# igd-geo/schwarzwald

Measured on AMD Instinct MI355X. Metric: Mpoints/s end-to-end tile (Morton+sort+sample), higher is better.
Workload: dtype u64 keys / f64 positions

## Files before the change

schwarzwald_amd/csrc/swz_api.hip:

```cpp
#include <algorithm>
#include <cstring>

#include "swz_device.h"
#include "swz_internal.h"

int swz_ctx::get(const char* name, size_t bytes, void** out) {
  swz::DevBuf& b = bufs[name];
  if (bytes == 0) bytes = 16;
  if (b.cap < bytes) {
    const size_t old_cap = b.cap;
    if (b.ptr) {
      SWZ_HIP(this, hipStreamSynchronize(stream));
      free_buf(b);
    }
    size_t want = bytes + bytes / 16;
    const size_t minimal = (want + 255) & ~size_t(255);
    if (old_cap) {
      if (strncmp(name, "tl_", 3) == 0 || strncmp(name, "tiler_store", 11) == 0) want = std::max(want, 2 * old_cap);
      else want = std::max(want, std::min(2 * old_cap, bytes + (size_t(1) << 30)));
    }
    want = (want + 255) & ~size_t(255);
    hipError_t e = hipMalloc(&b.ptr, want);
    if (const char* fa = opt("SWZ_FAIL_ALLOC")) {
      const size_t fl = strlen(fa);
      const bool hit = fl && fa[fl - 1] == '*' ? strncmp(fa, name, fl - 1) == 0 : strcmp(fa, name) == 0;
      if (e == hipSuccess && hit) {
        (void)hipFree(b.ptr);
        b.ptr = nullptr;
        e = hipErrorOutOfMemory;
      }
    }
    if (e == hipErrorOutOfMemory) {
      (void)hipGetLastError();
      SWZ_HIP(this, hipStreamSynchronize(stream));
      for (auto& kv : bufs) {
        const std::string& nm = kv.first;
        const bool level_scratch = nm.compare(0, 3, "md_") == 0 || nm.compare(0, 3, "sp_") == 0 || nm.compare(0, 3, "pm_") == 0;
        const bool shared_root = md_shard_root_published && nm.size() >= 3 && nm.compare(nm.size() - 3, 3, "_sr") == 0;
        const bool tiler_scratch = tiler_scratch_dead && nm.compare(0, 3, "tl_") == 0;
        if ((level_scratch || tiler_scratch) && !shared_root && kv.second.ptr && kv.second.epoch < scratch_epoch && &kv.second != &b)
          free_buf(kv.second);
      }
      e = hipMalloc(&b.ptr, want);
      if (e == hipErrorOutOfMemory && want > minimal) {
        (void)hipGetLastError();
        want = minimal;
        e = hipMalloc(&b.ptr, want);
      }
    }
    if (e != hipSuccess) {
      b.ptr = nullptr;
      std::vector<std::pair<size_t, std::string>> held;
      size_t total = 0;
      for (const auto& kv : bufs) {
        if (kv.second.host) continue;
        total += kv.second.cap;
        if (kv.second.cap) held.emplace_back(kv.second.cap, kv.first);
      }
      std::sort(held.rbegin(), held.rend());
      size_t free_b = 0, total_b = 0;
      (void)hipMemGetInfo(&free_b, &total_b);
      std::string top;
      for (size_t i = 0; i < held.size() && i < 14; ++i)
        top += " " + held[i].second + "=" + std::to_string(held[i].first >> 20) + "M";
      return fail(SWZ_ERR_HIP, std::string("hipMalloc(") + name + ", " + std::to_string(want) + " bytes): " + hipGetErrorString(e) +
                                 "; workspace holds " + std::to_string(total >> 20) + " MiB, device free " +
                                 std::to_string(free_b >> 20) + " of " + std::to_string(total_b >> 20) + " MiB; largest:" + top);
    }
    b.cap = want;
    if (const char* e = opt("SWZ_POISON")) {
      const char* only = opt("SWZ_POISON_ONLY");
      if (!only || strstr(name, only)) SWZ_HIP(this, hipMemsetAsync(b.ptr, atoi(e), want, stream));
    }
  }
  b.epoch = scratch_epoch;
  *out = b.ptr;
  return SWZ_OK;
}

void swz_ctx::release_all() {
  if (stream) (void)hipStreamSynchronize(stream);
  for (auto& kv : bufs) free_buf(kv.second);
  bufs.clear();
}

void swz_ctx::free_buf(swz::DevBuf& b) {
  if (b.ptr && b.ptr == sbi_clean_ptr) sbi_clean_ptr = nullptr;
  if (b.ptr) (void)(b.host ? hipHostFree(b.ptr) : hipFree(b.ptr));
  b.ptr = nullptr;
  b.cap = 0;
  b.host = false;
}

uint64_t swz_ctx::held_bytes() const {
  uint64_t s = 0;
  for (const auto& kv : bufs)
    if (!kv.second.host) s += kv.second.cap;
  return s;
}

uint64_t swz_ctx::held_host_bytes() const {
  uint64_t s = 0;
  for (const auto& kv : bufs)
    if (kv.second.host) s += kv.second.cap;
  return s;
}

hipEvent_t swz_ctx::take_event() {
  if (!event_pool.empty()) {
    hipEvent_t e = event_pool.back();
    event_pool.pop_back();
    return e;
  }
  hipEvent_t e = nullptr;
  (void)hipEventCreate(&e);
  return e;
}

void swz_ctx::prof_begin(const char*) {
  if (!profile) return;
  cur_e0_ = take_event();
  (void)hipEventRecord(cur_e0_, stream);
}

void swz_ctx::prof_end(const char* name, uint64_t launches, uint64_t bytes) {
  if (!profile || !cur_e0_) return;
  hipEvent_t e1 = take_event();
  (void)hipEventRecord(e1, stream);
  pending.push_back({name, cur_e0_, e1, launches, bytes});
  cur_e0_ = nullptr;
}

void swz_ctx::prof_collect() {
  for (auto& p : pending) {
    float ms = 0.f;
    if (hipEventSynchronize(p.e1) == hipSuccess && hipEventElapsedTime(&ms, p.e0, p.e1) == hipSuccess) {
      swz::KernelStat& k = kstats[p.name];
      k.launches += p.launches;
      k.total_ms += ms;
      k.bytes += p.bytes;
    }
    event_pool.push_back(p.e0);
    event_pool.push_back(p.e1);
  }
  pending.clear();
}

int swz::read_u32(swz_ctx* c, const uint32_t* d, uint32_t* h) {
  SWZ_HIP(c, hipMemcpyAsync(h, d, 4, hipMemcpyDeviceToHost, c->stream));
  SWZ_HIP(c, hipStreamSynchronize(c->stream));
  return SWZ_OK;
}

int swz::check_params(swz_ctx* c, const swz_tile_params* p) {
  if (!p) return c->fail(SWZ_ERR_BAD_ARG, "params must not be NULL");
  if (p->sampler < SWZ_RANDOM_GRID || p->sampler > SWZ_MIN_DISTANCE_FAST) return c->fail(SWZ_ERR_BAD_ARG, "unknown sampler");
  if (p->sampler == SWZ_MIN_DISTANCE_FAST && (p->flags & SWZ_FLAG_MIN_DISTANCE_PROPERTY))
    return c->fail(SWZ_ERR_BAD_ARG, "SWZ_FLAG_MIN_DISTANCE_PROPERTY with MIN_DISTANCE_FAST: the property mode's order is not defined for "
                                    "a sampler that offers only every n-th point of a node");
  if (p->strategy != SWZ_ACCURATE && p->strategy != SWZ_FAST) return c->fail(SWZ_ERR_BAD_ARG, "unknown strategy");
  if (!(p->spacing_at_root > 0.f)) return c->fail(SWZ_ERR_BAD_ARG, "spacing_at_root must be > 0");
  if (p->strategy == SWZ_FAST && p->fast_concurrency == 0)
    return c->fail(SWZ_ERR_BAD_ARG, "FAST needs fast_concurrency >= 1");
  return SWZ_OK;
}

const char* swz::sharded_sampler_refusal(int sampler) {
  if (sampler != SWZ_MIN_DISTANCE_FAST) return nullptr;
  return "MIN_DISTANCE_FAST cannot be sharded: the root offers every fourth point of ITS Morton-ordered range, counted across the "
         "shards' octants, and a shard does not know how many points the lower shards hold in front of its own";
}

static std::string g_create_error;

namespace {

int upload(swz_ctx* c, void* dst, const void* src, size_t bytes) {
  if (bytes == 0) return SWZ_OK;
  SWZ_HIP(c, hipMemcpyAsync(dst, src, bytes, hipMemcpyHostToDevice, c->stream));
  return SWZ_OK;
}
int download(swz_ctx* c, void* dst, const void* src, size_t bytes) {
  if (bytes == 0) return SWZ_OK;
  SWZ_HIP(c, hipMemcpyAsync(dst, src, bytes, hipMemcpyDeviceToHost, c->stream));
  return SWZ_OK;
}
int sync(swz_ctx* c) {
  SWZ_HIP(c, hipStreamSynchronize(c->stream));
  c->prof_collect();
  return SWZ_OK;
}
int check_n(swz_ctx* c, uint64_t n) {
  if (n > 0xFFFF0000ull) return c->fail(SWZ_ERR_TOO_MANY_POINTS, "more than 2^32-65536 points in one batch");
  return SWZ_OK;
}
int check_bounds(swz_ctx* c, const double mn[3], const double mx[3]) {
  if (!mn || !mx) return c->fail(SWZ_ERR_BAD_ARG, "bounds must not be NULL");
  for (int a = 0; a < 3; ++a)
    if (!(mx[a] > mn[a])) return c->fail(SWZ_ERR_BAD_ARG, "bounds must have positive extent on every axis");
  return SWZ_OK;
}

}

extern "C" {

int swz_abi_version(void) { return SWZ_ABI_VERSION; }

int swz_create(swz_ctx** ctx_out, int device) {
  if (!ctx_out) return SWZ_ERR_BAD_ARG;
  *ctx_out = nullptr;
  int count = 0;
  hipError_t e = hipGetDeviceCount(&count);
  if (e != hipSuccess || count <= 0) {
    g_create_error = std::string("swz_create: no usable HIP device (") +
                     (e != hipSuccess ? hipGetErrorString(e) : "device count is 0") +
                     "); this library has no CPU fallback";
    return SWZ_ERR_HIP;
  }
  if (device < 0 || device >= count) {
    g_create_error = "swz_create: device ordinal out of range";
    return SWZ_ERR_BAD_ARG;
  }
  e = hipSetDevice(device);
  if (e != hipSuccess) {
    g_create_error = std::string("swz_create: hipSetDevice: ") + hipGetErrorString(e);
    return SWZ_ERR_HIP;
  }
  swz_ctx* c = new swz_ctx();
  c->device = device;
  e = hipStreamCreateWithFlags(&c->own_stream, hipStreamNonBlocking);
  if (e != hipSuccess) {
    g_create_error = std::string("swz_create: hipStreamCreate: ") + hipGetErrorString(e);
    delete c;
    return SWZ_ERR_HIP;
  }
  c->stream = c->own_stream;
  extern char** environ;
  for (char** e = environ; e && *e; ++e) {
    if (std::strncmp(*e, "SWZ_", 4) != 0) continue;
    const char* eq = std::strchr(*e, '=');
    if (eq) c->options[std::string(*e, (size_t)(eq - *e))] = std::string(eq + 1);
  }
  *ctx_out = c;
  return SWZ_OK;
}

int swz_set_option(swz_ctx* c, const char* name, const char* value) {
  if (!c || !name) return SWZ_ERR_BAD_ARG;
  if (value) c->options[name] = value; else c->options.erase(name);
  return SWZ_OK;
}

int swz_destroy(swz_ctx* c) {
  if (!c) return SWZ_OK;
  (void)hipSetDevice(c->device);
  if (c->nodes_tiler) {
    (void)swz_tiler_destroy(c->nodes_tiler);
    c->nodes_tiler = nullptr;
  }
  swz::shard_free(c);
  c->release_all();
  c->prof_collect();
  for (hipEvent_t e : c->event_pool) (void)hipEventDestroy(e);
  for (hipStream_t st : c->aux_streams) (void)hipStreamDestroy(st);
  if (c->own_stream) (void)hipStreamDestroy(c->own_stream);
  delete c;
  return SWZ_OK;
}

const char* swz_last_error(const swz_ctx* c) { return c ? c->err.c_str() : g_create_error.c_str(); }

int swz_set_stream(swz_ctx* c, void* hip_stream) {
  if (!c) return SWZ_ERR_BAD_ARG;
  SWZ_HIP(c, hipStreamSynchronize(c->stream));
  c->stream = hip_stream == SWZ_OWN_STREAM ? c->own_stream : reinterpret_cast<hipStream_t>(hip_stream);
  return SWZ_OK;
}

int swz_release_workspace(swz_ctx* c) {
  if (!c) return SWZ_ERR_BAD_ARG;
  SWZ_HIP(c, hipSetDevice(c->device));
  if (c->tiler_active) return c->fail(SWZ_ERR_BAD_ARG, "swz_release_workspace: a tiler of this context keeps its node store in the workspace");
  swz::shard_free(c);
  c->release_all();
  return SWZ_OK;
}

uint64_t swz_workspace_bytes(const swz_ctx* c) { return c ? c->held_bytes() : 0; }

int swz_host_alloc_pinned(uint64_t bytes, void** out) {
  if (!out) return SWZ_ERR_BAD_ARG;
  *out = nullptr;
  return hipHostMalloc(out, bytes ? bytes : 1, hipHostMallocDefault) == hipSuccess ? SWZ_OK : SWZ_ERR_HIP;
}
int swz_host_free_pinned(void* p) { return (!p || hipHostFree(p) == hipSuccess) ? SWZ_OK : SWZ_ERR_HIP; }

int swz_device_alloc(uint64_t bytes, void** d_out) {
  if (!d_out) return SWZ_ERR_BAD_ARG;
  *d_out = nullptr;
  return hipMalloc(d_out, bytes ? bytes : 1) == hipSuccess ? SWZ_OK : SWZ_ERR_HIP;
}
int swz_device_alloc_on(swz_ctx* c, uint64_t bytes, void** d_out) {
  if (!c || !d_out) return SWZ_ERR_BAD_ARG;
  *d_out = nullptr;
  SWZ_HIP(c, hipSetDevice(c->device));
  SWZ_HIP(c, hipMalloc(d_out, bytes ? bytes : 1));
  return SWZ_OK;
}
int swz_device_free(void* d_ptr) { return (!d_ptr || hipFree(d_ptr) == hipSuccess) ? SWZ_OK : SWZ_ERR_HIP; }
static bool is_mapped_host_memory(const void* p) {
  hipPointerAttribute_t at{};
  if (hipPointerGetAttributes(&at, p) != hipSuccess) {
    (void)hipGetLastError();
    return false;
  }
  return at.type == hipMemoryTypeHost;
}
int swz_copy_to_host(swz_ctx* c, void* dst_host, const void* d_src, uint64_t bytes) {
  if (!c) return SWZ_ERR_BAD_ARG;
  SWZ_HIP(c, hipSetDevice(c->device));
  if (bytes && is_mapped_host_memory(d_src)) {
    SWZ_HIP(c, hipStreamSynchronize(c->stream));
    std::memcpy(dst_host, d_src, bytes);
    return SWZ_OK;
  }
  if (bytes) SWZ_HIP(c, hipMemcpyAsync(dst_host, d_src, bytes, hipMemcpyDeviceToHost, c->stream));
  SWZ_HIP(c, hipStreamSynchronize(c->stream));
  return SWZ_OK;
}
int swz_copy_to_device(swz_ctx* c, void* d_dst, const void* src_host, uint64_t bytes) {
  if (!c) return SWZ_ERR_BAD_ARG;
  SWZ_HIP(c, hipSetDevice(c->device));
  if (bytes && is_mapped_host_memory(d_dst)) {
    SWZ_HIP(c, hipStreamSynchronize(c->stream));
    std::memcpy(d_dst, src_host, bytes);
    return SWZ_OK;
  }
  if (bytes) SWZ_HIP(c, hipMemcpyAsync(d_dst, src_host, bytes, hipMemcpyHostToDevice, c->stream));
  SWZ_HIP(c, hipStreamSynchronize(c->stream));
  return SWZ_OK;
}

int swz_profile_enable(swz_ctx* c, int enabled) {
  if (!c) return SWZ_ERR_BAD_ARG;
  c->profile = enabled != 0;
  return SWZ_OK;
}
int swz_profile_reset(swz_ctx* c) {
  if (!c) return SWZ_ERR_BAD_ARG;
  SWZ_TRY(sync(c));
  c->kstats.clear();
  return SWZ_OK;
}
int swz_profile_get(swz_ctx* c, swz_kernel_stat* out, uint32_t max_stats, uint32_t* num_out) {
  if (!c || !num_out) return SWZ_ERR_BAD_ARG;
  SWZ_TRY(sync(c));
  uint32_t k = 0;
  for (const auto& kv : c->kstats) {
    if (k < max_stats && out) {
      std::memset(&out[k], 0, sizeof(out[k]));
      std::strncpy(out[k].name, kv.first.c_str(), sizeof(out[k].name) - 1);
      out[k].launches = kv.second.launches;
      out[k].total_ms = kv.second.total_ms;
      out[k].algorithmic_bytes = kv.second.bytes;
    }
    ++k;
  }
  *num_out = k;
  return SWZ_OK;
}

int swz_morton_encode_device(swz_ctx* c, double* d_xyz, uint64_t n, const double bmin[3], const double bmax[3],
                             uint64_t* d_keys_out) {
  if (!c) return SWZ_ERR_BAD_ARG;
  SWZ_HIP(c, hipSetDevice(c->device));
  SWZ_TRY(check_n(c, n));
  SWZ_TRY(check_bounds(c, bmin, bmax));
  if (n && (!d_xyz || !d_keys_out)) return c->fail(SWZ_ERR_BAD_ARG, "swz_morton_encode_device: NULL buffer");
  SWZ_TRY(swz::encode_device(c, d_xyz, (uint32_t)n, bmin, bmax, d_keys_out));
  return sync(c);
}

int swz_morton_encode(swz_ctx* c, double* xyz, uint64_t n, const double bmin[3], const double bmax[3],
                      uint64_t* keys_out) {
  if (!c) return SWZ_ERR_BAD_ARG;
  SWZ_HIP(c, hipSetDevice(c->device));
  SWZ_TRY(check_n(c, n));
  SWZ_TRY(check_bounds(c, bmin, bmax));
  if (n == 0) return SWZ_OK;
  if (!xyz || !keys_out) return c->fail(SWZ_ERR_BAD_ARG, "swz_morton_encode: NULL buffer");
  double* d_xyz = nullptr;
  uint64_t* d_keys = nullptr;
  SWZ_TRY(c->get("h_xyz", (size_t)n * 3, &d_xyz));
  SWZ_TRY(c->get("h_keys", (size_t)n, &d_keys));
  SWZ_TRY(upload(c, d_xyz, xyz, (size_t)n * 24));
  SWZ_TRY(swz::encode_device(c, d_xyz, (uint32_t)n, bmin, bmax, d_keys));
  SWZ_TRY(download(c, keys_out, d_keys, (size_t)n * 8));
  SWZ_TRY(download(c, xyz, d_xyz, (size_t)n * 24));
  return sync(c);
}

int swz_sort_by_key_device(swz_ctx* c, const uint64_t* d_keys, uint64_t n, uint32_t* d_perm_out,
                           uint64_t* d_keys_sorted_out) {
  if (!c) return SWZ_ERR_BAD_ARG;
  SWZ_HIP(c, hipSetDevice(c->device));
  SWZ_TRY(check_n(c, n));
  if (n == 0) return SWZ_OK;
  if (!d_keys || !d_perm_out) return c->fail(SWZ_ERR_BAD_ARG, "swz_sort_by_key_device: NULL buffer");
  uint64_t *kin = nullptr, *kout = d_keys_sorted_out;
  uint32_t* vtmp = nullptr;
  SWZ_TRY(c->get("sort_keys_b", (size_t)n, &kin));
  SWZ_TRY(c->get("sort_vals_b", (size_t)n, &vtmp));
  if (!kout) SWZ_TRY(c->get("sort_keys_a", (size_t)n, &kout));
  SWZ_HIP(c, hipMemcpyAsync(kin, d_keys, (size_t)n * 8, hipMemcpyDeviceToDevice, c->stream));
  SWZ_TRY(swz::radix_sort_pairs(c, kin, vtmp, kout, d_perm_out, (uint32_t)n, true));
  return sync(c);
}

int swz_sort_by_key(swz_ctx* c, const uint64_t* keys, uint64_t n, uint32_t* perm_out, uint64_t* keys_sorted_out) {
  if (!c) return SWZ_ERR_BAD_ARG;
  SWZ_HIP(c, hipSetDevice(c->device));
  SWZ_TRY(check_n(c, n));
  if (n == 0) return SWZ_OK;
  if (!keys || !perm_out) return c->fail(SWZ_ERR_BAD_ARG, "swz_sort_by_key: NULL buffer");
  uint64_t *ka = nullptr, *kb = nullptr;
  uint32_t *va = nullptr, *vb = nullptr;
  SWZ_TRY(c->get("sort_keys_a", (size_t)n, &ka));
  SWZ_TRY(c->get("sort_keys_b", (size_t)n, &kb));
  SWZ_TRY(c->get("sort_vals_a", (size_t)n, &va));
  SWZ_TRY(c->get("sort_vals_b", (size_t)n, &vb));
  SWZ_TRY(upload(c, kb, keys, (size_t)n * 8));
  SWZ_TRY(swz::radix_sort_pairs(c, kb, vb, ka, va, (uint32_t)n, true));
  SWZ_TRY(download(c, perm_out, va, (size_t)n * 4));
  if (keys_sorted_out) SWZ_TRY(download(c, keys_sorted_out, ka, (size_t)n * 8));
  return sync(c);
}

int swz_generate_uniform_device(swz_ctx* c, uint64_t seed, uint64_t first_point, uint64_t n, double* d_xyz_out) {
  if (!c) return SWZ_ERR_BAD_ARG;
  SWZ_HIP(c, hipSetDevice(c->device));
  if (n && !d_xyz_out) return c->fail(SWZ_ERR_BAD_ARG, "swz_generate_uniform_device: NULL buffer");
  SWZ_TRY(swz::generate_uniform_device(c, seed, first_point, n, d_xyz_out));
  return sync(c);
}

int swz_tile_device(swz_ctx* c, double* d_xyz, uint64_t n, const double bmin[3], const double bmax[3],
                    const swz_tile_params* params, uint64_t* d_keys_out, uint32_t* d_perm_out, int8_t* d_level_out,
                    uint32_t* d_dup_mask_out, swz_tile_stats* stats) {
  if (!c) return SWZ_ERR_BAD_ARG;
  SWZ_HIP(c, hipSetDevice(c->device));
  if (c->opt("SWZ_SYNC_ENTRY")) SWZ_HIP(c, hipDeviceSynchronize());
  SWZ_TRY(check_n(c, n));
  SWZ_TRY(check_bounds(c, bmin, bmax));
  SWZ_TRY(swz::check_params(c, params));
  if (stats) std::memset(stats, 0, sizeof(*stats));
  if (stats) {
    stats->max_level = -1;
    stats->fast_start_levels = -1;
  }
  if (n == 0) return SWZ_OK;
  if (!d_xyz || !d_keys_out || !d_perm_out || !d_level_out)
    return c->fail(SWZ_ERR_BAD_ARG, "swz_tile_device: NULL buffer");
  swz::TileDeviceOut out{d_keys_out, d_perm_out, d_level_out, d_dup_mask_out};
  int st = swz::tile_device(c, d_xyz, (uint32_t)n, bmin, bmax, *params, out, stats);
  int st2 = sync(c);
  return st != SWZ_OK ? st : st2;
}

int swz_tile(swz_ctx* c, double* xyz, uint64_t n, const double bmin[3], const double bmax[3],
             const swz_tile_params* params, uint64_t* keys_out, uint32_t* perm_out, int8_t* level_out,
             uint32_t* dup_mask_out, swz_tile_stats* stats) {
  if (!c) return SWZ_ERR_BAD_ARG;
  SWZ_HIP(c, hipSetDevice(c->device));
  SWZ_TRY(check_n(c, n));
  SWZ_TRY(check_bounds(c, bmin, bmax));
  SWZ_TRY(swz::check_params(c, params));
  if (stats) {
    std::memset(stats, 0, sizeof(*stats));
    stats->max_level = -1;
    stats->fast_start_levels = -1;
  }
  if (n == 0) return SWZ_OK;
  if (!xyz || !keys_out || !perm_out || !level_out) return c->fail(SWZ_ERR_BAD_ARG, "swz_tile: NULL buffer");
  double* d_xyz = nullptr;
  uint64_t* d_keys = nullptr;
  uint32_t *d_perm = nullptr, *d_dup = nullptr;
  int8_t* d_level = nullptr;
  SWZ_TRY(c->get("h_xyz", (size_t)n * 3, &d_xyz));
  SWZ_TRY(c->get("h_keys", (size_t)n, &d_keys));
  SWZ_TRY(c->get("h_perm", (size_t)n, &d_perm));
  SWZ_TRY(c->get("h_level", (size_t)n, &d_level));
  if (dup_mask_out) SWZ_TRY(c->get("h_dup", (size_t)n, &d_dup));
  SWZ_TRY(upload(c, d_xyz, xyz, (size_t)n * 24));
  swz::TileDeviceOut out{d_keys, d_perm, d_level, d_dup};
  int st = swz::tile_device(c, d_xyz, (uint32_t)n, bmin, bmax, *params, out, stats);
  if (st != SWZ_OK) {
    (void)sync(c);
    return st;
  }
  SWZ_TRY(download(c, keys_out, d_keys, (size_t)n * 8));
  SWZ_TRY(download(c, perm_out, d_perm, (size_t)n * 4));
  SWZ_TRY(download(c, level_out, d_level, (size_t)n));
  if (dup_mask_out) SWZ_TRY(download(c, dup_mask_out, d_dup, (size_t)n * 4));
  SWZ_TRY(download(c, xyz, d_xyz, (size_t)n * 24));
  return sync(c);
}

int swz_partition_by_octant_device(swz_ctx* c, const uint64_t* d_keys, uint64_t n, uint32_t* d_perm_out,
                                   uint64_t counts_out[8]) {
  if (!c || !counts_out) return SWZ_ERR_BAD_ARG;
  SWZ_HIP(c, hipSetDevice(c->device));
  SWZ_TRY(check_n(c, n));
  for (int o = 0; o < 8; ++o) counts_out[o] = 0;
  if (n == 0) return SWZ_OK;
  if (!d_keys || !d_perm_out) return c->fail(SWZ_ERR_BAD_ARG, "swz_partition_by_octant_device: NULL buffer");
  SWZ_TRY(swz::partition_top_digit(c, d_keys, (uint32_t)n, d_perm_out, counts_out));
  return sync(c);
}

int swz_shard_presort_device(swz_ctx* c, const double* d_xyz_local, uint64_t n, const double bmin[3],
                             const double bmax[3], const swz_tile_params* params, uint64_t ghost_capacity) {
  if (!c) return SWZ_ERR_BAD_ARG;
  SWZ_HIP(c, hipSetDevice(c->device));
  SWZ_TRY(check_n(c, n + ghost_capacity));
  SWZ_TRY(check_bounds(c, bmin, bmax));
  SWZ_TRY(swz::check_params(c, params));
  if (const char* why = swz::sharded_sampler_refusal(params->sampler)) return c->fail(SWZ_ERR_BAD_ARG, why);
  if (n && !d_xyz_local) return c->fail(SWZ_ERR_BAD_ARG, "swz_shard_presort_device: NULL buffer");
  if (n == 0) return SWZ_OK;
  int st = swz::shard_presort_device(c, d_xyz_local, (uint32_t)n, bmin, bmax, *params, (uint32_t)ghost_capacity);
  int st2 = sync(c);
  return st != SWZ_OK ? st : st2;
}

int swz_shard_begin_device(swz_ctx* c, const double* d_xyz_local, uint64_t n, const double bmin[3],
                           const double bmax[3], const swz_tile_params* params, const swz_shard_info* shard,
                           uint64_t* num_root_taken_out) {
  if (!c) return SWZ_ERR_BAD_ARG;
  SWZ_HIP(c, hipSetDevice(c->device));
  if (!shard) return c->fail(SWZ_ERR_BAD_ARG, "shard info must not be NULL");
  SWZ_TRY(check_n(c, n + shard->num_ghosts));
  SWZ_TRY(check_bounds(c, bmin, bmax));
  SWZ_TRY(swz::check_params(c, params));
  if (const char* why = swz::sharded_sampler_refusal(params->sampler)) return c->fail(SWZ_ERR_BAD_ARG, why);
  if ((n && !d_xyz_local) || (shard->num_ghosts && !shard->d_ghost_xyz))
    return c->fail(SWZ_ERR_BAD_ARG, "swz_shard_begin_device: NULL buffer");
  if (num_root_taken_out) *num_root_taken_out = 0;
  if (n == 0) {
    return swz::shard_begin_empty(c);
  }
  int st = swz::shard_begin_device(c, d_xyz_local, (uint32_t)n, bmin, bmax, *params, shard->global_points,
                                   shard->d_ghost_xyz, (uint32_t)shard->num_ghosts, num_root_taken_out);
  int st2 = sync(c);
  return st != SWZ_OK ? st : st2;
}

int swz_shard_root_taken_device(swz_ctx* c, double* d_xyz_out) {
  if (!c) return SWZ_ERR_BAD_ARG;
  SWZ_HIP(c, hipSetDevice(c->device));
  SWZ_TRY(swz::shard_root_taken_device(c, d_xyz_out));
  return sync(c);
}

int swz_shard_finish_device(swz_ctx* c, uint64_t* d_keys_out, uint32_t* d_perm_out, int8_t* d_level_out,
                            swz_tile_stats* stats) {
  if (!c) return SWZ_ERR_BAD_ARG;
  SWZ_HIP(c, hipSetDevice(c->device));
  if (stats) {
    std::memset(stats, 0, sizeof(*stats));
    stats->max_level = -1;
    stats->fast_start_levels = -1;
  }
  int st = swz::shard_finish_device(c, d_keys_out, d_perm_out, d_level_out, stats);
  int st2 = sync(c);
  return st != SWZ_OK ? st : st2;
}

int swz_shard_fast_begin_device(swz_ctx* c, const double* d_xyz_local, uint64_t n, const double bmin[3], const double bmax[3],
                                const swz_tile_params* params, uint32_t* prefix_counts_out) {
  if (!c) return SWZ_ERR_BAD_ARG;
  SWZ_HIP(c, hipSetDevice(c->device));
  SWZ_TRY(check_n(c, n));
  SWZ_TRY(check_bounds(c, bmin, bmax));
  SWZ_TRY(swz::check_params(c, params));
  if (const char* why = swz::sharded_sampler_refusal(params->sampler)) return c->fail(SWZ_ERR_BAD_ARG, why);
  if ((n && !d_xyz_local) || !prefix_counts_out) return c->fail(SWZ_ERR_BAD_ARG, "swz_shard_fast_begin_device: NULL buffer");
  int st = swz::shard_fast_begin_device(c, d_xyz_local, (uint32_t)n, bmin, bmax, *params, prefix_counts_out);
  int st2 = sync(c);
  return st != SWZ_OK ? st : st2;
}
int swz_shard_fast_run(swz_ctx* c, int32_t start_level, uint64_t* num_root_candidates_out) {
  if (!c || !num_root_candidates_out) return SWZ_ERR_BAD_ARG;
  SWZ_HIP(c, hipSetDevice(c->device));
  int st = swz::shard_fast_run_device(c, start_level, num_root_candidates_out);
  int st2 = sync(c);
  return st != SWZ_OK ? st : st2;
}
int swz_shard_fast_root_candidates_device(swz_ctx* c, uint64_t* d_keys_out, double* d_xyz_out) {
  if (!c) return SWZ_ERR_BAD_ARG;
  SWZ_HIP(c, hipSetDevice(c->device));
  SWZ_TRY(swz::shard_fast_root_candidates_device(c, d_keys_out, d_xyz_out));
  return sync(c);
}
int swz_shard_fast_set_root_device(swz_ctx* c, const uint8_t* d_taken) {
  if (!c) return SWZ_ERR_BAD_ARG;
  SWZ_HIP(c, hipSetDevice(c->device));
  SWZ_TRY(swz::shard_fast_set_root_device(c, d_taken));
  return sync(c);
}
int swz_shard_fast_finish_device(swz_ctx* c, uint64_t* d_keys_out, uint32_t* d_perm_out, int8_t* d_level_out, uint32_t* d_dup_out,
                                 swz_tile_stats* stats) {
  if (!c) return SWZ_ERR_BAD_ARG;
  SWZ_HIP(c, hipSetDevice(c->device));
  if (stats) {
    std::memset(stats, 0, sizeof(*stats));
    stats->max_level = -1;
    stats->fast_start_levels = -1;
  }
  int st = swz::shard_fast_finish_device(c, d_keys_out, d_perm_out, d_level_out, d_dup_out, stats);
  int st2 = sync(c);
  return st != SWZ_OK ? st : st2;
}

int swz_sample_points(swz_ctx* c, int sampler, uint64_t max_points_per_node, const uint64_t* keys,
                      const uint32_t* idx, uint64_t n, const double* xyz, uint64_t num_points, uint64_t node_key,
                      int32_t node_level, const double root_min[3], const double root_max[3], float spacing_at_root,
                      int behaviour, uint8_t* taken_out, uint64_t* num_taken_out) {
  if (!c) return SWZ_ERR_BAD_ARG;
  SWZ_HIP(c, hipSetDevice(c->device));
  SWZ_TRY(check_n(c, n));
  SWZ_TRY(check_n(c, num_points));
  SWZ_TRY(check_bounds(c, root_min, root_max));
  if (sampler < SWZ_RANDOM_GRID || sampler > SWZ_MIN_DISTANCE_FAST) return c->fail(SWZ_ERR_BAD_ARG, "unknown sampler");
  if (node_level < -1 || node_level > 20) return c->fail(SWZ_ERR_BAD_ARG, "node_level out of range");
  if (num_taken_out) *num_taken_out = 0;
  if (n == 0) return SWZ_OK;
  if (!keys || !idx || !xyz || !taken_out) return c->fail(SWZ_ERR_BAD_ARG, "swz_sample_points: NULL buffer");
  double* d_xyz = nullptr;
  uint64_t* d_keys = nullptr;
  uint32_t* d_idx = nullptr;
  uint8_t* d_taken = nullptr;
  SWZ_TRY(c->get("h_xyz", (size_t)num_points * 3, &d_xyz));
  SWZ_TRY(c->get("h_keys", (size_t)n, &d_keys));
  SWZ_TRY(c->get("h_perm", (size_t)n, &d_idx));
  SWZ_TRY(c->get("h_taken", (size_t)n, &d_taken));
  SWZ_TRY(upload(c, d_xyz, xyz, (size_t)num_points * 24));
  SWZ_TRY(upload(c, d_keys, keys, (size_t)n * 8));
  SWZ_TRY(upload(c, d_idx, idx, (size_t)n * 4));
  int st = swz::sample_points_device(c, sampler, max_points_per_node, d_keys, d_idx, (uint32_t)n, d_xyz, node_key,
                                     node_level, root_min, root_max, spacing_at_root, behaviour, d_taken,
                                     num_taken_out);
  if (st != SWZ_OK) {
    (void)sync(c);
    return st;
  }
  SWZ_TRY(download(c, taken_out, d_taken, (size_t)n));
  return sync(c);
}

int swz_sample_points_device(swz_ctx* c, int sampler, uint64_t max_points_per_node, const uint64_t* d_keys, const uint32_t* d_idx,
                             uint64_t n, const double* d_xyz, uint64_t num_points, uint64_t node_key, int32_t node_level,
                             const double root_min[3], const double root_max[3], float spacing_at_root, int behaviour,
                             uint8_t* d_taken_out, uint64_t* num_taken_out) {
  if (!c) return SWZ_ERR_BAD_ARG;
  SWZ_HIP(c, hipSetDevice(c->device));
  SWZ_TRY(check_n(c, n));
  SWZ_TRY(check_n(c, num_points));
  SWZ_TRY(check_bounds(c, root_min, root_max));
  if (sampler < SWZ_RANDOM_GRID || sampler > SWZ_MIN_DISTANCE_FAST) return c->fail(SWZ_ERR_BAD_ARG, "unknown sampler");
  if (node_level < -1 || node_level > 20) return c->fail(SWZ_ERR_BAD_ARG, "node_level out of range");
  if (num_taken_out) *num_taken_out = 0;
  if (n == 0) return SWZ_OK;
  if (!d_keys || !d_idx || !d_xyz || !d_taken_out) return c->fail(SWZ_ERR_BAD_ARG, "swz_sample_points_device: NULL buffer");
  int st = swz::sample_points_device(c, sampler, max_points_per_node, d_keys, d_idx, (uint32_t)n, d_xyz, node_key, node_level, root_min,
                                     root_max, spacing_at_root, behaviour, d_taken_out, num_taken_out);
  int st2 = sync(c);
  return st != SWZ_OK ? st : st2;
}

int swz_build_node_lists(swz_ctx* c, const uint64_t* keys_sorted, const int8_t* level, uint64_t n,
                         uint32_t* order_out, uint64_t max_nodes, int8_t* node_level_out, uint64_t* node_key_out,
                         uint64_t* node_offset_out, uint64_t* node_count_out, uint64_t* num_nodes_out) {
  if (!c || !num_nodes_out) return SWZ_ERR_BAD_ARG;
  *num_nodes_out = 0;
  if (n == 0) return SWZ_OK;
  if (!keys_sorted || !level || !order_out) return c->fail(SWZ_ERR_BAD_ARG, "swz_build_node_lists: NULL buffer");
  uint64_t hist[23] = {0};
  for (uint64_t i = 0; i < n; ++i) {
    const int l = level[i];
    if (l < -1 || l > 20) return c->fail(SWZ_ERR_BAD_ARG, "level out of range");
    hist[l + 2]++;
  }
  for (int l = 1; l < 23; ++l) hist[l] += hist[l - 1];
  for (uint64_t i = 0; i < n; ++i) order_out[hist[level[i] + 1]++] = (uint32_t)i;
  uint64_t nn = 0;
  uint64_t i = 0;
  while (i < n) {
    const uint64_t p = order_out[i];
    const int l = level[p];
    const uint32_t sh = (l < 0) ? 63u : swz::level_shift(l);
    const uint64_t prefix = keys_sorted[p] >> sh;
    uint64_t j = i + 1;
    while (j < n && level[order_out[j]] == l && (keys_sorted[order_out[j]] >> sh) == prefix) ++j;
    if (nn < max_nodes && node_level_out && node_key_out && node_offset_out && node_count_out) {
      node_level_out[nn] = (int8_t)l;
      node_key_out[nn] = (l < 0) ? 0 : (prefix << sh);
      node_offset_out[nn] = i;
      node_count_out[nn] = j - i;
    }
    ++nn;
    i = j;
  }
  *num_nodes_out = nn;
  if (nn > max_nodes) return c->fail(SWZ_ERR_BAD_ARG, "max_nodes too small");
  return SWZ_OK;
}

}
```

schwarzwald_amd/csrc/swz_internal.h:

```cpp
#pragma once

#include <hip/hip_runtime.h>
#include <stdint.h>

#include <map>
#include <cstdio>
#include <cstdlib>
#include <string>
#include <vector>

#include "../../include/swz_gpu.h"

namespace swz {

constexpr uint32_t MAX_LEVELS = 21;

struct DevBuf {
  void* ptr = nullptr;
  size_t cap = 0;
  uint64_t epoch = 0;
  bool host = false;
};

struct KernelStat {
  uint64_t launches = 0;
  double total_ms = 0.0;
  uint64_t bytes = 0;
};

struct PendingEvent {
  std::string name;
  hipEvent_t e0, e1;
  uint64_t launches;
  uint64_t bytes;
};

}

struct swz_ctx {
  int device = 0;
  hipStream_t own_stream = nullptr;
  hipStream_t stream = nullptr;
  std::string err;
  std::map<std::string, swz::DevBuf> bufs;
  bool profile = false;
  std::map<std::string, swz::KernelStat> kstats;
  std::vector<swz::PendingEvent> pending;
  std::vector<hipEvent_t> event_pool;
  std::vector<hipStream_t> aux_streams;

  int fail(int code, const std::string& msg) {
    err = msg;
    return code;
  }
  int hip_fail(hipError_t e, const char* what, const char* file, int line) {
    err = std::string(what) + ": " + hipGetErrorString(e) + " (" + file + ":" + std::to_string(line) + ")";
    return SWZ_ERR_HIP;
  }

  uint64_t scratch_epoch = 1;
  void next_scratch_epoch() { ++scratch_epoch; }
  int get(const char* name, size_t bytes, void** out);
  template <typename T>
  int get(const char* name, size_t count, T** out) {
    return get(name, count * sizeof(T), reinterpret_cast<void**>(out));
  }
  void release_all();
  void free_buf(swz::DevBuf& b);
  uint64_t held_bytes() const;
  uint64_t held_host_bytes() const;

  hipEvent_t take_event();
  void prof_begin(const char* name);
  void prof_end(const char* name, uint64_t launches, uint64_t bytes);
  void prof_collect();
  hipEvent_t cur_e0_ = nullptr;
  void* shard = nullptr;
  const void* md_shard_root = nullptr;
  bool md_shard_root_published = false;
  const void* sbi_clean_ptr = nullptr;
  size_t sbi_clean_bytes = 0;
  bool tiler_active = false;
  swz_tiler* nodes_tiler = nullptr;
  bool tiler_scratch_dead = false;
  std::map<std::string, std::string> options;
  const char* opt(const char* name) const {
    const auto it = options.find(name);
    return it == options.end() ? nullptr : it->second.c_str();
  }
  long opt_int(const char* name, long def) const {
    const char* v = opt(name);
    return v ? (long)atoll(v) : def;
  }
  double opt_num(const char* name, double def) const {
    const char* v = opt(name);
    return v ? atof(v) : def;
  }
  bool opt_on(const char* name, bool def) const {
    const char* v = opt(name);
    return v ? atoi(v) != 0 : def;
  }
};

#define SWZ_HIP(ctx, expr)                                                \
  do {                                                                    \
    hipError_t _e = (expr);                                               \
    if (_e != hipSuccess) return (ctx)->hip_fail(_e, #expr, __FILE__, __LINE__); \
  } while (0)

#define SWZ_TRY(expr)            \
  do {                           \
    int _s = (expr);             \
    if (_s != SWZ_OK) return _s; \
  } while (0)

#define SWZ_LAUNCH_CHECK(ctx) SWZ_HIP(ctx, hipGetLastError())

namespace swz {

inline uint32_t div_up(uint64_t a, uint64_t b) { return (uint32_t)((a + b - 1) / b); }

struct ProfScope {
  swz_ctx* c;
  const char* name;
  uint64_t launches, bytes;
  ProfScope(swz_ctx* ctx, const char* n, uint64_t b, uint64_t l = 1) : c(ctx), name(n), launches(l), bytes(b) {
    c->prof_begin(name);
  }
  ~ProfScope() { c->prof_end(name, launches, bytes); }
};

#define SWZ_STAGE(ctx, what)                                                              \
  do {                                                                                    \
    if ((ctx)->opt("SWZ_TRACE")) {                                                            \
      const hipError_t _e = hipStreamSynchronize((ctx)->stream);                          \
      fprintf(stderr, "[swz trace] %s:%d %s -> %s\n", __FILE__, __LINE__, what, hipGetErrorString(_e)); \
      fflush(stderr);                                                                     \
    }                                                                                     \
  } while (0)

inline hipError_t memset_large(void* p, int value, size_t bytes, hipStream_t stream) {
  const size_t piece = size_t(1) << 30;
  for (size_t at = 0; at < bytes; at += piece) {
    const hipError_t e = hipMemsetAsync(static_cast<char*>(p) + at, value, bytes - at < piece ? bytes - at : piece, stream);
    if (e != hipSuccess) return e;
  }
  return hipSuccess;
}

int read_u32(swz_ctx* c, const uint32_t* d, uint32_t* h);

int encode_device(swz_ctx* c, double* d_xyz, uint32_t n, const double bmin[3], const double bmax[3],
                  uint64_t* d_keys);
int generate_uniform_device(swz_ctx* c, uint64_t seed, uint64_t first, uint64_t n, double* d_xyz);
int check_params(swz_ctx* c, const swz_tile_params* p);
const char* sharded_sampler_refusal(int sampler);

int radix_sort_pairs(swz_ctx* c, uint64_t* d_keys_in, uint32_t* d_vals_tmp, uint64_t* d_keys_out,
                     uint32_t* d_vals_out, uint32_t n, bool vals_identity);

int scan_exclusive_u32(swz_ctx* c, const uint32_t* d_in, uint32_t* d_out, uint64_t n, uint32_t* d_total,
                       const char* tag);

int gather_positions(swz_ctx* c, const double* d_xyz, const uint32_t* d_perm, uint32_t n, double* d_x,
                     double* d_y, double* d_z);

struct TileDeviceOut {
  uint64_t* keys;
  uint32_t* perm;
  int8_t* level;
  uint32_t* dup;
};

int tile_device(swz_ctx* c, double* d_xyz, uint32_t n, const double bmin[3], const double bmax[3],
                const swz_tile_params& p, const TileDeviceOut& out, swz_tile_stats* stats);

int shard_begin_device(swz_ctx* c, const double* d_xyz_local, uint32_t n, const double bmin[3],
                       const double bmax[3], const swz_tile_params& p, uint64_t global_points,
                       const double* d_ghost_xyz, uint32_t ghosts, uint64_t* num_root_taken);
int shard_presort_device(swz_ctx* c, const double* d_xyz_local, uint32_t n, const double bmin[3], const double bmax[3],
                         const swz_tile_params& p, uint32_t ghost_capacity);
int shard_root_taken_device(swz_ctx* c, double* d_xyz_out);
int shard_finish_device(swz_ctx* c, uint64_t* d_keys_out, uint32_t* d_perm_out, int8_t* d_level_out,
                        swz_tile_stats* stats);
int shard_begin_empty(swz_ctx* c);
void shard_free(swz_ctx* c);
int shard_fast_begin_device(swz_ctx* c, const double* d_xyz_local, uint32_t n, const double bmin[3], const double bmax[3],
                            const swz_tile_params& p, uint32_t* counts_host);
int shard_fast_run_device(swz_ctx* c, int start_level, uint64_t* num_root_candidates);
int shard_fast_root_candidates_device(swz_ctx* c, uint64_t* d_keys_out, double* d_xyz_out);
int shard_fast_set_root_device(swz_ctx* c, const uint8_t* d_taken);
int shard_fast_finish_device(swz_ctx* c, uint64_t* d_keys_out, uint32_t* d_perm_out, int8_t* d_level_out, uint32_t* d_dup_out,
                             swz_tile_stats* stats);
int partition_top_digit(swz_ctx* c, const uint64_t* d_keys, uint32_t n, uint32_t* d_perm_out, uint64_t octants[8]);
int partition_by_top_byte(swz_ctx* c, const uint64_t* d_keys, uint32_t n, uint32_t* d_perm_out, uint32_t starts[256]);

int sample_points_device(swz_ctx* c, int sampler, uint64_t max_points, const uint64_t* d_keys,
                         const uint32_t* d_idx, uint32_t n, const double* d_xyz, uint64_t node_key,
                         int32_t node_level, const double rmin[3], const double rmax[3], float spacing,
                         int behaviour, uint8_t* d_taken, uint64_t* num_taken);

}
```

schwarzwald_amd/csrc/swz_level.h:

```cpp
#pragma once
#include "swz_device.h"
#include "swz_internal.h"

namespace swz {

enum : uint8_t { MODE_TAKE_ALL = 0, MODE_SAMPLE = 1 };

inline bool greedy_sampler(int sampler) { return sampler == SWZ_MIN_DISTANCE || sampler == SWZ_MIN_DISTANCE_FAST; }

enum {
  CTR_NUM_NODES = 0,
  CTR_SAMPLE_NODES = 1,
  CTR_SAMPLE_POINTS = 2,
  CTR_ERROR = 3,
  CTR_REMAINING = 4,
  CTR_NUM_CELLS = 5,
  CTR_DONE_CELLS = 6,
  CTR_Q0 = 8,
  CTR_DBG_TIME = 20,
  CTR_DBG_TMAX = 21,
  CTR_DBG_HIST = 22,
  CTR_COUNT = 40
};

struct ActiveSet {
  const uint64_t* akey = nullptr;
  const uint32_t* aidx = nullptr;
  uint32_t m = 0;
  const uint64_t* ckey = nullptr;
  uint32_t nc = 0;
  uint32_t old_lo = 0, old_hi = 0;
  const uint64_t* new_key = nullptr;
  uint32_t new_m = 0;
  const uint64_t* child_nkey = nullptr;
  uint32_t child_nn = 0;
  const uint64_t* parent_prefix = nullptr;
  uint32_t parents = 0;
};

struct SortedPoints {
  const double* X = nullptr;
  const double* Y = nullptr;
  const double* Z = nullptr;
  const double* xyz = nullptr;
  const uint32_t* perm = nullptr;
  const double* ghost_xyz = nullptr;
  uint32_t ghosts = 0;
};
__host__ __device__ inline const double* sorted_point_xyz(const double* xyz, const uint32_t* perm, const double* ghost_xyz, uint32_t ghosts,
                                                          uint32_t s) {
  return (s < ghosts ? ghost_xyz : xyz) + (size_t)perm[s] * 3;
}
__device__ __forceinline__ void store_sorted_point(const SortedPoints& sp, uint32_t i, double* __restrict__ out_xyz, uint64_t o) {
  if (sp.X) {
    out_xyz[3 * o] = sp.X[i];
    out_xyz[3 * o + 1] = sp.Y[i];
    out_xyz[3 * o + 2] = sp.Z[i];
  } else {
    const double* p = sorted_point_xyz(sp.xyz, sp.perm, sp.ghost_xyz, sp.ghosts, i);
    out_xyz[3 * o] = p[0];
    out_xyz[3 * o + 1] = p[1];
    out_xyz[3 * o + 2] = p[2];
  }
}

struct LevelPlan {
  int level = -1;
  uint32_t node_shift = 63;
  int sampler = 0;
  uint64_t max_points = 0;
  bool force_sample = false;
  bool terminal = false;
  bool reroot = false;
  bool md_property = false;
  Box root;
  int cand = -1;
  double spacing_node = 0.0;
  uint32_t jitter_start = 0;
  double sq_spacing = 0.0;
  int cell_levels_geo = 0;
};

struct LevelBuffers {
  uint32_t* flags = nullptr;
  uint32_t* nid = nullptr;
  uint32_t* nstart = nullptr;
  uint8_t* nmode = nullptr;
  uint8_t* taken = nullptr;
  uint32_t* counters = nullptr;
};

struct LevelResult {
  uint32_t remaining = 0;
  uint32_t num_nodes = 0;
  uint32_t md_rounds = 0;
  const uint64_t* node_prefix = nullptr;
};

LevelPlan make_plan(int level, int sampler, uint64_t max_points, float spacing_at_root, uint32_t max_depth,
                    const double bmin[3], const double bmax[3], bool force_sample, bool tiler_rules);
int alloc_level_buffers(swz_ctx* c, uint32_t m, LevelBuffers* lb);
int required_depth_host(int sampler, int node_level, double root_extent_x, float root_max_spacing);
int level_step(swz_ctx* c, const LevelPlan& plan, const ActiveSet& as, const SortedPoints& sp, const LevelBuffers& lb,
               int8_t* level_out, uint64_t* okey, uint32_t* oidx, LevelResult* res);
const char* level_error_message(int code);
int fast_start_level(swz_ctx* c, const uint64_t* d_keys_sorted, uint32_t n, uint32_t concurrency, int* start_level);
int fast_prefix_counts(swz_ctx* c, const uint64_t* d_keys_sorted, uint32_t n, uint32_t* counts_host);
int fast_start_level_from_counts(const uint64_t* counts, uint32_t concurrency);

int random_grid_level(swz_ctx* c, const LevelPlan& plan, const ActiveSet& as, const LevelBuffers& lb);
int grid_level(swz_ctx* c, const LevelPlan& plan, const ActiveSet& as, const SortedPoints& sp, const LevelBuffers& lb);
bool grid_level_uses_keys(const swz_ctx* c, const LevelPlan& plan, const SortedPoints& sp);
int min_distance_level(swz_ctx* c, const LevelPlan& plan, const ActiveSet& as, const SortedPoints& sp,
                       const LevelBuffers& lb, uint32_t num_nodes, uint32_t sample_nodes,
                       uint32_t sample_points, uint32_t* rounds_out);
int min_distance_fast_level(swz_ctx* c, const LevelPlan& plan, const ActiveSet& as, const SortedPoints& sp, const LevelBuffers& lb,
                            uint32_t stride, uint32_t num_nodes, uint32_t sample_nodes, uint32_t* rounds_out);

}
```

schwarzwald_amd/csrc/swz_level.hip:

```cpp
#include <algorithm>
#include <cmath>

#include "swz_md.h"
#include "swz_scan.h"

namespace swz {

struct NodeHeadF {
  const uint64_t* akey;
  uint32_t nsh;
  __device__ uint32_t operator()(uint32_t i) const {
    return (i == 0) ? 1u : (uint32_t)((akey[i] >> nsh) != (akey[i - 1] >> nsh));
  }
};
struct NodeAssignG {
  uint32_t* nid;
  uint32_t* nstart;
  uint32_t m;
  __device__ void operator()(uint32_t i, uint32_t excl, uint32_t head) const {
    const uint32_t id = excl + head - 1u;
    nid[i] = id;
    if (head) nstart[id] = i;
    if (i == m - 1) nstart[id + 1] = m;
  }
};
__global__ __launch_bounds__(256) void node_child_bounds_kernel(const uint64_t* __restrict__ akey, uint32_t m, uint32_t nsh,
                                                                const uint64_t* __restrict__ pprefix, uint32_t parents,
                                                                uint32_t* __restrict__ cb) {
  const uint32_t t = blockIdx.x * 256 + threadIdx.x;
  const uint32_t j = t >> 4, o = t & 15u;
  if (j >= parents || o > 8u) return;
  const uint64_t target = (pprefix[j] >> nsh) + o;
  uint32_t lo = 0, hi = m;
  while (lo < hi) {
    const uint32_t mid = lo + (hi - lo) / 2;
    if ((akey[mid] >> nsh) < target) lo = mid + 1; else hi = mid;
  }
  cb[j * 9u + o] = lo;
}
struct ChildExistsF {
  const uint32_t* cb;
  uint32_t parents, m;
  uint32_t* counters;
  __device__ uint32_t operator()(uint32_t e) const {
    const uint32_t j = e >> 3, o = e & 7u;
    if (o == 0) {
      const uint32_t b = cb[j * 9u], en = cb[j * 9u + 8u];
      const bool ok = (j == 0 ? b == 0u : b == cb[(j - 1u) * 9u + 8u]) && (j + 1u < parents || en == m);
      if (!ok) atomicMax(&counters[CTR_ERROR], (uint32_t)SWZ_ERR_INTERNAL);
    }
    return cb[j * 9u + o + 1u] > cb[j * 9u + o] ? 1u : 0u;
  }
};
struct ChildStartG {
  const uint32_t* cb;
  uint32_t* nstart;
  __device__ void operator()(uint32_t e, uint32_t excl, uint32_t exists) const {
    if (!exists) return;
    const uint32_t j = e >> 3, o = e & 7u;
    nstart[excl] = cb[j * 9u + o];
    nstart[excl + 1u] = cb[j * 9u + o + 1u];
  }
};
constexpr uint32_t NF_TILE = 1024;
__global__ __launch_bounds__(256) void node_fill_kernel(const uint32_t* __restrict__ nstart, const uint32_t* __restrict__ counters,
                                                        uint32_t m, uint32_t* __restrict__ nid, int lazy) {
  __shared__ uint32_t s_lo, s_hi;
  __shared__ uint32_t ss[NF_TILE + 1];
  const uint32_t nn = counters[CTR_NUM_NODES];
  if (lazy && counters[CTR_SAMPLE_NODES] == nn) return;
  if (counters[CTR_ERROR] != 0u || nn == 0u) return;
  const uint32_t tid = threadIdx.x;
  const uint32_t i0 = blockIdx.x * NF_TILE;
  const uint32_t last = (m - i0) > NF_TILE ? i0 + NF_TILE - 1u : m - 1u;
  auto node_of = [&](uint32_t i) {
    uint32_t lo = 0, hi = nn;
    while (lo < hi) {
      const uint32_t mid = lo + (hi - lo) / 2;
      if (nstart[mid] <= i) lo = mid + 1; else hi = mid;
    }
    return lo - 1u;
  };
  if (tid < 2) {
    const uint32_t r = node_of(tid ? last : i0);
    if (tid) s_hi = r; else s_lo = r;
  }
  __syncthreads();
  const uint32_t lo = s_lo, span = min(s_hi - s_lo + 1u, (uint32_t)NF_TILE);
  for (uint32_t k = tid; k <= span; k += 256u) ss[k] = (lo + k < nn) ? nstart[lo + k] : 0xFFFFFFFFu;
  __syncthreads();
  const uint32_t i = i0 + tid * 4u;
  if (i >= m) return;
  uint32_t a = 0, b = span;
  while (a < b) {
    const uint32_t mid = a + (b - a) / 2;
    if (ss[mid] <= i) a = mid + 1; else b = mid;
  }
  uint32_t k = a - 1u;
  uint32_t v[4];
#pragma unroll
  for (uint32_t q = 0; q < 4u; ++q) {
    while (k + 1u <= span && ss[k + 1u] <= i + q) ++k;
    v[q] = lo + k;
  }
  if (i + 4u <= m) {
    *reinterpret_cast<uint4*>(nid + i) = make_uint4(v[0], v[1], v[2], v[3]);
  } else {
    for (uint32_t q = 0; i + q < m; ++q) nid[i + q] = v[q];
  }
}
__global__ __launch_bounds__(256) void node_prefix_kernel(const uint32_t* __restrict__ nstart, const uint64_t* __restrict__ akey,
                                                          uint32_t nsh, uint32_t nn, uint64_t* __restrict__ out) {
  const uint32_t j = blockIdx.x * 256 + threadIdx.x;
  if (j < nn) out[j] = nsh >= 63u ? 0ull : ((akey[nstart[j]] >> nsh) << nsh);
}
__global__ void single_node_kernel(uint32_t* __restrict__ nstart, uint32_t* __restrict__ num_nodes, uint32_t m) {
  nstart[0] = 0;
  nstart[1] = m;
  *num_nodes = 1;
}
struct KeepF {
  const uint8_t* taken;
  __device__ uint32_t operator()(uint32_t i) const { return taken[i] ? 0u : 1u; }
};
template <>
struct FsCountsZeroBytes<KeepF> {
  static constexpr bool value = true;
};
struct CompactG {
  const uint64_t* akey;
  const uint32_t* aidx;
  int8_t level;
  int8_t* level_out;
  uint64_t* okey;
  uint32_t* oidx;
  __device__ void operator()(uint32_t i, uint32_t excl, uint32_t keep) const {
    const uint32_t p = aidx ? aidx[i] : i;
    if (keep) {
      okey[excl] = akey[i];
      oidx[excl] = p;
    } else {
      level_out[p] = level;
    }
  }
};

__global__ __launch_bounds__(256) void node_head_kernel(const uint64_t* __restrict__ akey, uint32_t m,
                                                        uint32_t nsh, uint32_t* __restrict__ flags) {
  const uint32_t i = blockIdx.x * 256 + threadIdx.x;
  if (i >= m) return;
  flags[i] = (i == 0) ? 1u : (uint32_t)((akey[i] >> nsh) != (akey[i - 1] >> nsh));
}

__global__ __launch_bounds__(256) void node_finish_kernel(const uint32_t* __restrict__ flags,
                                                          uint32_t* __restrict__ nid, uint32_t m,
                                                          uint32_t* __restrict__ nstart) {
  const uint32_t i = blockIdx.x * 256 + threadIdx.x;
  if (i >= m) return;
  const uint32_t f = flags[i];
  const uint32_t id = nid[i] + f - 1u;
  nid[i] = id;
  if (f) nstart[id] = i;
  if (i == m - 1) nstart[id + 1] = m;
}

__global__ __launch_bounds__(256) void node_mode_kernel(const uint32_t* __restrict__ nstart,
                                                        uint8_t* __restrict__ nmode, uint32_t* __restrict__ counters,
                                                        uint64_t max_points, int force_sample, int terminal,
                                                        int reroot, const uint64_t* __restrict__ akey, uint32_t nsh,
                                                        const uint64_t* __restrict__ ckey, uint32_t nc) {
  const uint32_t nnodes = counters[CTR_NUM_NODES];
  for (uint32_t j = blockIdx.x * 256 + threadIdx.x; j < nnodes; j += gridDim.x * 256u) {
    const uint32_t cnt = nstart[j + 1] - nstart[j];
    bool cached = false;
    if (nc) {
      const uint64_t prefix = akey[nstart[j]] >> nsh;
      uint32_t lo = 0, hi = nc;
      while (lo < hi) {
        const uint32_t mid = lo + (hi - lo) / 2;
        if ((ckey[mid] >> nsh) < prefix) lo = mid + 1; else hi = mid;
      }
      cached = lo < nc && (ckey[lo] >> nsh) == prefix;
    }
    const bool sample = !terminal && (force_sample || cached || (uint64_t)cnt > max_points);
    nmode[j] = sample ? MODE_SAMPLE : MODE_TAKE_ALL;
    if (sample) {
      if (reroot) atomicMax(&counters[CTR_ERROR], (uint32_t)SWZ_ERR_REROOT_UNSUPPORTED);
      atomicAdd(&counters[CTR_SAMPLE_NODES], 1u);
      atomicAdd(&counters[CTR_SAMPLE_POINTS], cnt);
    }
  }
}

__global__ __launch_bounds__(256) void take_all_kernel(uint32_t m, const uint32_t* __restrict__ nid,
                                                       const uint8_t* __restrict__ nmode,
                                                       uint8_t* __restrict__ taken) {
  const uint32_t i = blockIdx.x * 256 + threadIdx.x;
  if (i >= m) return;
  if (nmode[nid[i]] == MODE_TAKE_ALL) taken[i] = 1;
}

static int candidate_level_host(double root_extent_x, float spacing_at_root, int node_level) {
  const auto spacing_at_this_node = spacing_at_root / std::pow(2, node_level + 1);
  return std::max(-1, (int)std::floor(std::log2f(root_extent_x / spacing_at_this_node)) - 1);
}
static int node_level_to_sample_from_host(double root_extent_x, float root_max_spacing, int node_level) {
  const auto spacing_at_target_node = root_max_spacing / std::pow(2, node_level + 1);
  const float target_spacing = (float)spacing_at_target_node;
  return std::max(-1, (int)std::floor(std::log2f(root_extent_x / target_spacing)) - 1);
}
static uint32_t prev_pow2_host(uint32_t x) {
  x = x | (x >> 1);
  x = x | (x >> 2);
  x = x | (x >> 4);
  x = x | (x >> 8);
  x = x | (x >> 16);
  return x - (x >> 1);
}
int required_depth_host(int sampler, int node_level, double root_extent_x, float root_max_spacing) {
  switch (sampler) {
    case SWZ_RANDOM_GRID:
    case SWZ_GRID_CENTER:
      return node_level_to_sample_from_host(root_extent_x, root_max_spacing, node_level);
    case SWZ_MIN_DISTANCE:
    case SWZ_MIN_DISTANCE_FAST:
      return node_level;
    default: {
      const auto spacing_at_this_node = root_max_spacing / std::pow(2, node_level + 1);
      const auto perfect_cell_count = (root_extent_x / std::pow(2, node_level + 1)) / spacing_at_this_node;
      const double clamped = perfect_cell_count >= 4294967295.0 ? 4294967295.0 : perfect_cell_count;
      const auto actual_cell_count = prev_pow2_host(static_cast<uint32_t>(clamped));
      const uint32_t levels = static_cast<uint32_t>(std::log2(actual_cell_count));
      return static_cast<int32_t>(static_cast<uint32_t>(node_level + levels));
    }
  }
}

}
extern "C" int32_t swz_required_morton_index_depth(int sampler, int32_t node_level, const double root_min[3],
                                                   const double root_max[3], float spacing_at_root) {
  if (!root_min || !root_max) return INT32_MIN;
  return swz::required_depth_host(sampler, node_level, root_max[0] - root_min[0], spacing_at_root);
}
namespace swz {

LevelPlan make_plan(int level, int sampler, uint64_t max_points, float spacing_at_root, uint32_t max_depth,
                           const double bmin[3], const double bmax[3], bool force_sample, bool tiler_rules) {
  LevelPlan p;
  p.level = level;
  p.node_shift = level < 0 ? 63u : level_shift(level);
  p.sampler = sampler;
  p.max_points = max_points;
  p.force_sample = force_sample;
  p.root = Box{bmin[0], bmin[1], bmin[2], bmax[0], bmax[1], bmax[2]};
  const double ext_x = bmax[0] - bmin[0];
  if (tiler_rules) {
    const int req = required_depth_host(sampler, level, ext_x, spacing_at_root);
    const bool deeper = req > level;
    const int max_level = (int)std::min<uint32_t>(MAX_LEVELS - 1, max_depth);
    if (!deeper) {
      p.terminal = req >= max_level;
    } else {
      p.terminal = level >= max_level;
      p.reroot = !p.terminal && req >= (int)MAX_LEVELS;
    }
  }
  p.cand = candidate_level_host(ext_x, spacing_at_root, level);
  p.spacing_node = spacing_at_root / std::pow(2, level + 1);
  p.jitter_start = (3u * static_cast<uint32_t>(level + 1)) % 16u;
  const float sf = static_cast<float>(p.spacing_node);
  const float sq = sf * sf;
  p.sq_spacing = (double)sq;
  double min_ext = std::min(bmax[0] - bmin[0], std::min(bmax[1] - bmin[1], bmax[2] - bmin[2]));
  const double need = (double)spacing_at_root * (1.0 + 0x1.0p-20);
  int mg = 0;
  while (mg < 20 && min_ext / 2 >= need) {
    min_ext /= 2;
    ++mg;
  }
  p.cell_levels_geo = std::min(mg, 20 - level);
  return p;
}

bool level_decides_on_keys(const swz_ctx* c, const LevelPlan& plan, const SortedPoints& sp) {
  if (plan.sampler == SWZ_RANDOM_GRID) return true;
  if (greedy_sampler(plan.sampler)) return min_distance_level_uses_keys(c, plan, sp);
  return grid_level_uses_keys(c, plan, sp);
}

const char* level_error_message(int code) {
  switch (code) {
    case SWZ_ERR_JITTER_GRID_TOO_SMALL: return "Grids smaller than 16x16 are not supported currently!";
    case SWZ_ERR_JITTER_NODE_TOO_DEEP: return "node is too small to be sampled with JITTERED";
    case SWZ_ERR_REROOT_UNSUPPORTED: return "a node needs Morton re-rooting, which this call's per-point outputs cannot express: use swz_tile_nodes_begin_device / _end_device (one batch as node files) or a swz_tiler";
    case SWZ_ERR_INTERNAL: return "level segmentation inconsistent, or a MIN_DISTANCE sweep / a peer shard failed";
    default: return "a kernel of the level raised an error";
  }
}

int level_step(swz_ctx* c, const LevelPlan& plan, const ActiveSet& as, const SortedPoints& sp,
                      const LevelBuffers& lb, int8_t* level_out, uint64_t* okey, uint32_t* oidx,
                      LevelResult* res) {
  const uint32_t m = as.m;
  const uint32_t nb = div_up(m, 256);
  SWZ_HIP(c, hipMemsetAsync(lb.counters, 0, CTR_COUNT * sizeof(uint32_t), c->stream));
  {
    ProfScope ps(c, "level_nodes", (uint64_t)m * 8ull, 3);
    bool fill_after_modes = false;
    if (plan.node_shift >= 63u && m > 0) {
      const bool sampled_for_sure = !plan.terminal && (plan.force_sample || (uint64_t)m > plan.max_points);
      if (greedy_sampler(plan.sampler) || !sampled_for_sure)
        SWZ_HIP(c, hipMemsetAsync(lb.nid, 0, (size_t)m * sizeof(uint32_t), c->stream));
      hipLaunchKernelGGL(single_node_kernel, dim3(1), dim3(1), 0, c->stream, lb.nstart, lb.counters + CTR_NUM_NODES, m);
      SWZ_LAUNCH_CHECK(c);
    } else if (as.parent_prefix && as.parents && m > 0 && !c->opt("SWZ_LEVEL_NODES_SCAN")) {
      uint32_t* cb = nullptr;
      SWZ_TRY(c->get("lvl_child_bounds", (size_t)as.parents * 9u, &cb));
      hipLaunchKernelGGL(node_child_bounds_kernel, dim3(div_up(as.parents * 16u, 256u)), dim3(256), 0, c->stream, as.akey, m,
                         plan.node_shift, as.parent_prefix, as.parents, cb);
      SWZ_LAUNCH_CHECK(c);
      SWZ_TRY(fused_scan(c, ChildExistsF{cb, as.parents, m, lb.counters}, ChildStartG{cb, lb.nstart}, as.parents * 8u,
                         lb.counters + CTR_NUM_NODES, "lvl"));
      fill_after_modes = true;
    } else {
      SWZ_TRY(fused_scan(c, NodeHeadF{as.akey, plan.node_shift}, NodeAssignG{lb.nid, lb.nstart, m}, m,
                         lb.counters + CTR_NUM_NODES, "lvl"));
    }
    hipLaunchKernelGGL(node_mode_kernel, dim3(std::min(nb, 2048u)), dim3(256), 0, c->stream, lb.nstart, lb.nmode, lb.counters,
                       plan.max_points, plan.force_sample ? 1 : 0, plan.terminal ? 1 : 0, plan.reroot ? 1 : 0, as.akey,
                       plan.node_shift, as.ckey, as.nc);
    SWZ_LAUNCH_CHECK(c);
    if (fill_after_modes) {
      hipLaunchKernelGGL(node_fill_kernel, dim3(div_up(m, NF_TILE)), dim3(256), 0, c->stream, lb.nstart, lb.counters, m, lb.nid,
                         greedy_sampler(plan.sampler) ? 0 : 1);
      SWZ_LAUNCH_CHECK(c);
    }
  }

  if (plan.sampler == SWZ_RANDOM_GRID) {
    SWZ_TRY(random_grid_level(c, plan, as, lb));
  } else if (plan.sampler == SWZ_GRID_CENTER || plan.sampler == SWZ_JITTERED) {
    SWZ_TRY(grid_level(c, plan, as, sp, lb));
  } else if (plan.sampler == SWZ_MIN_DISTANCE_FAST && plan.cand < 0) {
    SWZ_TRY(random_grid_level(c, plan, as, lb));
  } else {
    SWZ_HIP(c, hipMemsetAsync(lb.taken, 0, m, c->stream));
    uint32_t h[CTR_COUNT];
    SWZ_HIP(c, hipMemcpyAsync(h, lb.counters, sizeof(h), hipMemcpyDeviceToHost, c->stream));
    SWZ_HIP(c, hipStreamSynchronize(c->stream));
    if (h[CTR_ERROR]) return c->fail((int)h[CTR_ERROR], level_error_message((int)h[CTR_ERROR]));
    if (h[CTR_SAMPLE_NODES] < h[CTR_NUM_NODES]) {
      hipLaunchKernelGGL(take_all_kernel, dim3(nb), dim3(256), 0, c->stream, m, lb.nid, lb.nmode, lb.taken);
      SWZ_LAUNCH_CHECK(c);
    }
    const uint32_t stride = plan.sampler == SWZ_MIN_DISTANCE_FAST ? (uint32_t)swz_min_distance_fast_stride(plan.level) : 1u;
    if (h[CTR_SAMPLE_NODES] > 0 && stride > 1u) {
      SWZ_TRY(min_distance_fast_level(c, plan, as, sp, lb, stride, h[CTR_NUM_NODES], h[CTR_SAMPLE_NODES], &res->md_rounds));
    } else if (h[CTR_SAMPLE_NODES] > 0) {
      SWZ_TRY(min_distance_level(c, plan, as, sp, lb, h[CTR_NUM_NODES], h[CTR_SAMPLE_NODES], h[CTR_SAMPLE_POINTS],
                                 &res->md_rounds));
    }
  }

  if (okey) {
    ProfScope ps(c, "level_compact", (uint64_t)m * 14ull, 2);
    SWZ_TRY(fused_scan(c, KeepF{lb.taken}, CompactG{as.akey, as.aidx, (int8_t)plan.level, level_out, okey, oidx}, m,
                       lb.counters + CTR_REMAINING, "lvl"));
  }
  uint32_t h[CTR_COUNT];
  SWZ_HIP(c, hipMemcpyAsync(h, lb.counters, sizeof(h), hipMemcpyDeviceToHost, c->stream));
  SWZ_HIP(c, hipStreamSynchronize(c->stream));
  c->prof_collect();
  if (h[CTR_ERROR]) {
    const int code = (int)h[CTR_ERROR];
    return c->fail(code, level_error_message(code));
  }
  res->remaining = h[CTR_REMAINING];
  res->num_nodes = h[CTR_NUM_NODES];
  res->node_prefix = nullptr;
  if (okey && res->remaining && res->num_nodes) {
    uint64_t* np = nullptr;
    SWZ_TRY(c->get((plan.level & 1) ? "lvl_node_prefix_1" : "lvl_node_prefix_0", (size_t)res->num_nodes, &np));
    hipLaunchKernelGGL(node_prefix_kernel, dim3(div_up(res->num_nodes, 256)), dim3(256), 0, c->stream, lb.nstart, as.akey,
                       plan.node_shift, res->num_nodes, np);
    SWZ_LAUNCH_CHECK(c);
    res->node_prefix = np;
  }
  return SWZ_OK;
}

int alloc_level_buffers(swz_ctx* c, uint32_t m, LevelBuffers* lb) {
  SWZ_TRY(c->get("lvl_flags", (size_t)m, &lb->flags));
  SWZ_TRY(c->get("lvl_nid", (size_t)m, &lb->nid));
  SWZ_TRY(c->get("lvl_nstart", (size_t)m + 1, &lb->nstart));
  SWZ_TRY(c->get("lvl_nmode", (size_t)m, &lb->nmode));
  SWZ_TRY(c->get("lvl_taken", (size_t)m, &lb->taken));
  SWZ_TRY(c->get("lvl_counters", (size_t)CTR_COUNT, &lb->counters));
  return SWZ_OK;
}

}
```

schwarzwald_amd/csrc/swz_md.h:

```cpp
#pragma once
#include "swz_level.h"

namespace swz {

struct MdPeerView {
  const uint4* rec = nullptr;
  const uint64_t* qpos = nullptr;
  const uint8_t* state = nullptr;
  const float4* ovf = nullptr;
  const uint32_t* gridmap = nullptr;
  const uint32_t* round_word = nullptr;
  const uint32_t* perm = nullptr;
  const double* xyz = nullptr;
  const uint32_t* aidx = nullptr;
  uint32_t ncells = 0, rg = 0, cell_shift = 0;
  uint32_t npoints = 0;
  int status = 0;
  int entered = 0;
};
struct MdShardRoot {
  int shard = 0, shards = 1;
  MdPeerView* views = nullptr;
  void (*barrier)(void*) = nullptr;
  void* barrier_arg = nullptr;
};

struct KeyMetric {
  bool ok = false;
  double T = 0.0;
  float f_lo = 0.f;
  float f_hi = 0.f;
};
KeyMetric key_metric(const swz_ctx* c, const LevelPlan& plan, const SortedPoints& sp);
int key_point_ids(swz_ctx* c, const ActiveSet& as, const SortedPoints& sp, const uint32_t** ids);
bool min_distance_level_uses_keys(const swz_ctx* c, const LevelPlan& plan, const SortedPoints& sp);
bool level_decides_on_keys(const swz_ctx* c, const LevelPlan& plan, const SortedPoints& sp);
struct MdLevel {
  const LevelPlan& plan;
  const ActiveSet& as;
  const SortedPoints& sp;
  const LevelBuffers& lb;
  uint32_t num_nodes, sample_nodes, sample_points;
  bool all_sampled;
  const uint32_t* snode_of = nullptr;
  KeyMetric km;
  uint32_t occupied[12] = {0};
  bool sampled_hist = false;
  double pop[4] = {0, 0, 0, 0};
  bool have_pop = false;
};
int md_clamp_cell_levels(uint32_t sample_nodes, int cl);
int md_count_cells_exact(swz_ctx* c, const MdLevel& L, uint32_t occupied[12]);
int md_active_positions(swz_ctx* c, const MdLevel& L, size_t per_point, const double** X, const double** Y, const double** Z);

int min_distance_keys_level(swz_ctx* c, const MdLevel& L, int cl, uint32_t* rounds_out, bool* used,
                            const MdShardRoot* shard_root = nullptr);
int min_distance_block_level(swz_ctx* c, const MdLevel& L, bool* done);
int min_distance_sparse_level(swz_ctx* c, const MdLevel& L, int cl, uint32_t* rounds_out, bool* used);
int min_distance_rounds_level(swz_ctx* c, const MdLevel& L, uint32_t* rounds_out, bool* used);
int min_distance_sweep_level(swz_ctx* c, const MdLevel& L, int cl, uint32_t* rounds_out);
int min_distance_phases_level(swz_ctx* c, const MdLevel& L, int cl, uint32_t* phases_out);

}
```

schwarzwald_amd/csrc/swz_md.hip:

```cpp
#include <algorithm>
#include <cmath>

#include "swz_md.h"
#include "swz_scan.h"

namespace swz {

__global__ __launch_bounds__(256) void md_node_flag_kernel(const uint8_t* __restrict__ nmode, uint32_t nnodes,
                                                           uint32_t* __restrict__ out) {
  const uint32_t j = blockIdx.x * 256 + threadIdx.x;
  if (j < nnodes) out[j] = nmode[j] == MODE_SAMPLE ? 1u : 0u;
}

__global__ __launch_bounds__(256) void md_cell_hist_kernel(const uint64_t* __restrict__ akey, const uint32_t* __restrict__ nid,
                                                           const uint8_t* __restrict__ nmode, uint32_t m, uint32_t node_shift,
                                                           uint32_t cl_geo, uint32_t skip, uint32_t* __restrict__ hist) {
  __shared__ uint32_t lh[16];
  if (threadIdx.x < 16) lh[threadIdx.x] = 0;
  __syncthreads();
  uint32_t mine = 0;
  for (uint64_t i0 = (uint64_t)blockIdx.x * skip * 256u; i0 < m; i0 += (uint64_t)gridDim.x * skip * 256u) {
    const uint32_t i = (uint32_t)i0 + threadIdx.x;
    uint32_t bin = 0xFFu;
    if (i0 + threadIdx.x < m && nmode[nid[i]] == MODE_SAMPLE) {
      if (i == 0 || nid[i - 1] != nid[i]) {
        bin = 0;
      } else if (cl_geo) {
        const uint64_t diff = ((akey[i] ^ akey[i - 1]) >> (node_shift - 3u * cl_geo)) & ((1ull << (3u * cl_geo)) - 1ull);
        if (diff) bin = cl_geo - (uint32_t)(63 - __clzll((unsigned long long)diff)) / 3u;
      }
    }
    for (uint32_t b = 0; b <= cl_geo; ++b) {
      const uint32_t cnt = (uint32_t)__popcll(__ballot(bin == b));
      if (lane_id() == b) mine += cnt;
    }
  }
  if (lane_id() <= cl_geo && mine) atomicAdd(&lh[lane_id()], mine);
  __syncthreads();
  if (threadIdx.x < 16 && lh[threadIdx.x]) atomicAdd(&hist[threadIdx.x], lh[threadIdx.x]);
}

constexpr uint32_t MD_POP_SAMPLES = 1u << 16;
__global__ __launch_bounds__(256) void md_cell_pop_kernel(const uint64_t* __restrict__ akey, const uint32_t* __restrict__ nid,
                                                          const uint8_t* __restrict__ nmode, uint32_t m, uint32_t node_shift,
                                                          uint32_t cl_geo, unsigned long long* __restrict__ out) {
  const uint32_t t = blockIdx.x * 256 + threadIdx.x;
  if (t >= MD_POP_SAMPLES) return;
  const uint32_t i = (uint32_t)(((uint64_t)t * m) / MD_POP_SAMPLES);
  if (i >= m || nmode[nid[i]] != MODE_SAMPLE) return;
  const uint64_t key = akey[i];
  for (uint32_t k = 0; k <= 3u && k <= cl_geo; ++k) {
    const uint32_t sh = node_shift - 3u * (cl_geo - k);
    const uint64_t pre = key >> sh;
    uint32_t lo = 0, hi = i;
    while (lo < hi) {
      const uint32_t mid = lo + (hi - lo) / 2u;
      if ((akey[mid] >> sh) < pre) lo = mid + 1u; else hi = mid;
    }
    const uint32_t first = lo;
    lo = i;
    hi = m;
    while (lo < hi) {
      const uint32_t mid = lo + (hi - lo) / 2u;
      if ((akey[mid] >> sh) <= pre) lo = mid + 1u; else hi = mid;
    }
    atomicAdd(&out[k], (unsigned long long)(lo - first));
  }
  atomicAdd(&out[4], 1ull);
}

__global__ __launch_bounds__(256) void md_gather_active_kernel(const uint32_t* __restrict__ aidx, uint32_t m,
                                                               const double* __restrict__ X,
                                                               const double* __restrict__ Y,
                                                               const double* __restrict__ Z, double* __restrict__ ax,
                                                               double* __restrict__ ay, double* __restrict__ az) {
  const uint32_t i = blockIdx.x * 256 + threadIdx.x;
  if (i >= m) return;
  const uint32_t s = aidx[i];
  ax[i] = X[s];
  ay[i] = Y[s];
  az[i] = Z[s];
}

__global__ __launch_bounds__(256) void pm_clear_taken_kernel(const uint32_t* __restrict__ nid, const uint8_t* __restrict__ nmode,
                                                             uint32_t m, uint8_t* __restrict__ taken) {
  const uint32_t i = blockIdx.x * 256 + threadIdx.x;
  if (i < m && nmode[nid[i]] == MODE_SAMPLE) taken[i] = 0;
}

int md_clamp_cell_levels(uint32_t sample_nodes, int cl) {
  while (cl > 0 && (double)sample_nodes * std::pow(8.0, cl) > 2147483648.0) --cl;
  return cl;
}

static int count_cells(swz_ctx* c, const MdLevel& L, uint32_t skip, uint32_t occupied[12]) {
  const uint32_t m = L.as.m;
  uint32_t* d_hist = nullptr;
  SWZ_TRY(c->get("md_hist", (size_t)16, &d_hist));
  SWZ_HIP(c, hipMemsetAsync(d_hist, 0, 64, c->stream));
  const uint32_t tiles = div_up(m, 256);
  const uint32_t sampled_tiles = div_up(tiles, skip);
  hipLaunchKernelGGL(md_cell_hist_kernel, dim3(std::min<uint32_t>(sampled_tiles, 4096u)), dim3(256), 0, c->stream, L.as.akey,
                     L.lb.nid, L.lb.nmode, m, L.plan.node_shift, (uint32_t)L.plan.cell_levels_geo, skip, d_hist);
  SWZ_LAUNCH_CHECK(c);
  SWZ_STAGE(c, "md cell hist");
  uint32_t h[16];
  SWZ_HIP(c, hipMemcpyAsync(h, d_hist, 64, hipMemcpyDeviceToHost, c->stream));
  SWZ_HIP(c, hipStreamSynchronize(c->stream));
  const double scale = skip == 1 ? 1.0 : (double)m / (double)std::min<uint64_t>(m, (uint64_t)sampled_tiles * 256u);
  double run = 0;
  for (int b = 0; b < 12; ++b) {
    run += h[b];
    occupied[b] = (uint32_t)std::min<double>(run * scale, (double)m);
  }
  return SWZ_OK;
}
int md_count_cells_exact(swz_ctx* c, const MdLevel& L, uint32_t occupied[12]) { return count_cells(c, L, 1u, occupied); }

static int md_populations(swz_ctx* c, MdLevel& L) {
  if (L.have_pop) return SWZ_OK;
  unsigned long long* d_pop = nullptr;
  SWZ_TRY(c->get("md_pop", (size_t)8, &d_pop));
  SWZ_HIP(c, hipMemsetAsync(d_pop, 0, 64, c->stream));
  hipLaunchKernelGGL(md_cell_pop_kernel, dim3(MD_POP_SAMPLES / 256), dim3(256), 0, c->stream, L.as.akey, L.lb.nid, L.lb.nmode, L.as.m,
                     L.plan.node_shift, (uint32_t)L.plan.cell_levels_geo, d_pop);
  SWZ_LAUNCH_CHECK(c);
  SWZ_STAGE(c, "md cell pop");
  unsigned long long h[5];
  SWZ_HIP(c, hipMemcpyAsync(h, d_pop, 40, hipMemcpyDeviceToHost, c->stream));
  SWZ_HIP(c, hipStreamSynchronize(c->stream));
  for (int k = 0; k < 4; ++k) L.pop[k] = h[4] ? (double)h[k] / (double)h[4] : 1e30;
  L.have_pop = true;
  return SWZ_OK;
}

static int survey(swz_ctx* c, MdLevel& L) {
  const uint32_t skip = std::max(1u, L.as.m >> 23);
  L.sampled_hist = skip > 1u;
  SWZ_TRY(count_cells(c, L, skip, L.occupied));
  if (!L.plan.md_property) SWZ_TRY(md_populations(c, L));
  uint32_t* snode = nullptr;
  SWZ_TRY(c->get("md_snode", (size_t)L.num_nodes, &snode));
  hipLaunchKernelGGL(md_node_flag_kernel, dim3(div_up(L.num_nodes, 256)), dim3(256), 0, c->stream, L.lb.nmode, L.num_nodes, snode);
  SWZ_LAUNCH_CHECK(c);
  SWZ_TRY(scan_exclusive_u32(c, snode, snode, L.num_nodes, nullptr, "mdn"));
  L.snode_of = snode;
  L.km = key_metric(c, L.plan, L.sp);
  return SWZ_OK;
}

int md_active_positions(swz_ctx* c, const MdLevel& L, size_t per_point, const double** X, const double** Y, const double** Z) {
  *X = L.sp.X;
  *Y = L.sp.Y;
  *Z = L.sp.Z;
  if (!L.as.aidx) return SWZ_OK;
  const uint32_t m = L.as.m;
  double* ax = nullptr;
  SWZ_TRY(c->get("md_pos", (size_t)m * per_point, &ax));
  hipLaunchKernelGGL(md_gather_active_kernel, dim3(div_up(m, 256)), dim3(256), 0, c->stream, L.as.aidx, m, L.sp.X, L.sp.Y, L.sp.Z, ax,
                     ax + m, ax + 2 * (size_t)m);
  SWZ_LAUNCH_CHECK(c);
  *X = ax;
  *Y = ax + m;
  *Z = ax + 2 * (size_t)m;
  return SWZ_OK;
}

static int sweep_cell_levels(const swz_ctx* c, const MdLevel& L) {
  const LevelPlan& plan = L.plan;
  int cl = plan.cell_levels_geo;
  const double avg = (double)L.sample_points / (double)L.sample_nodes;
  const double per_cell = 8.0;
  const double max_pop = 160.0;
  while (cl > 0 && plan.cell_levels_geo - cl < 3 && (double)L.sample_points / (double)std::max(1u, L.occupied[cl]) < per_cell &&
         L.pop[plan.cell_levels_geo - cl + 1] <= max_pop)
    --cl;
  cl = md_clamp_cell_levels(L.sample_nodes, cl);
  if (const long coarsen = c->opt_int("SWZ_MD_COARSEN", 0))
    if (avg / std::pow(8.0, cl) >= c->opt_num("SWZ_MD_COARSEN_MIN", 32.0)) cl = std::max(0, cl - (int)coarsen);
  return cl;
}

static int phases_cell_levels(swz_ctx* c, MdLevel& L, int* cl_out) {
  const LevelPlan& plan = L.plan;
  const double node_ext = (plan.root.maxx - plan.root.minx) / std::pow(2.0, plan.level + 1);
  const double r0 = node_ext / std::pow(2.0, plan.cell_levels_geo) / plan.spacing_node;
  int cl = plan.cell_levels_geo;
  if (cl > 0 && (double)L.sample_points / (double)std::max(1u, L.occupied[cl]) < 24.0 && 0.75 * 8.0 * r0 * r0 * r0 <= 48.0) {
    SWZ_TRY(md_populations(c, L));
    if (L.pop[1] <= 1024.0) --cl;
  }
  *cl_out = md_clamp_cell_levels(L.sample_nodes, cl);
  return SWZ_OK;
}

int min_distance_level(swz_ctx* c, const LevelPlan& plan, const ActiveSet& as, const SortedPoints& sp, const LevelBuffers& lb,
                       uint32_t num_nodes, uint32_t sample_nodes, uint32_t sample_points, uint32_t* rounds_out) {
  c->next_scratch_epoch();
  MdLevel L{plan, as, sp, lb, num_nodes, sample_nodes, sample_points, sample_nodes == num_nodes};
  SWZ_TRY(survey(c, L));
  bool used = false;

  if (c->md_shard_root && plan.level == -1) {
    SWZ_TRY(min_distance_keys_level(c, L, plan.cell_levels_geo, rounds_out, &used, static_cast<const MdShardRoot*>(c->md_shard_root)));
    if (!used) return c->fail(SWZ_ERR_INTERNAL, "MIN_DISTANCE root of a sharded batch: the joint sweep needs a level that can be decided on keys");
    return SWZ_OK;
  }

  const int cl_sparse = md_clamp_cell_levels(sample_nodes, plan.cell_levels_geo);
  const bool sparse = (double)sample_points / (double)std::max(1u, L.occupied[cl_sparse]) < c->opt_num("SWZ_MD_SPARSE_LIMIT", 2.0);
  if (sparse && !(sp.ghosts && plan.level == -1 && !sp.X)) {
    SWZ_TRY(min_distance_block_level(c, L, &used));
    if (used) {
      if (rounds_out) *rounds_out += 1;
      return SWZ_OK;
    }
    SWZ_TRY(min_distance_sparse_level(c, L, cl_sparse, rounds_out, &used));
    if (used) return SWZ_OK;
    if (plan.md_property) {
      hipLaunchKernelGGL(pm_clear_taken_kernel, dim3(div_up(as.m, 256)), dim3(256), 0, c->stream, lb.nid, lb.nmode, as.m, lb.taken);
      SWZ_LAUNCH_CHECK(c);
    }
  }

  if (plan.md_property && L.km.ok) {
    SWZ_TRY(min_distance_rounds_level(c, L, rounds_out, &used));
    if (used) return SWZ_OK;
  }

  int cl = 0;
  if (!plan.md_property || !sp.X) {
    SWZ_TRY(md_populations(c, L));
    cl = sweep_cell_levels(c, L);
    SWZ_TRY(min_distance_keys_level(c, L, cl, rounds_out, &used));
    if (used) return SWZ_OK;
  }

  if (!sp.X) return c->fail(SWZ_ERR_INTERNAL, "MIN_DISTANCE: this level needs the positions in Morton order and they were not gathered");
  if (!plan.md_property) return min_distance_sweep_level(c, L, cl, rounds_out);
  SWZ_TRY(phases_cell_levels(c, L, &cl));
  return min_distance_phases_level(c, L, cl, rounds_out);
}

}
```

schwarzwald_amd/csrc/swz_mdkeys.hip:

```cpp
#include <algorithm>
#include <chrono>
#include <cmath>
#include <cstdio>
#include <cstdlib>
#include <cstring>
#include <string>
#include <vector>

#include "swz_md.h"
#include "swz_scan.h"

namespace swz {

constexpr uint32_t QNONE = 0xFFFFFFFFu;
constexpr unsigned long long QEMPTY = ~0ull;
constexpr uint32_t MQ_WOKEN = 0x80000000u;
constexpr int MQ_LIST_CAP = 128;
constexpr int MQ_FRESH_CAP = 32;
#ifndef MQ_MINW4
#define MQ_MINW4 4
#endif
#ifndef MQ_MINW1
#define MQ_MINW1 6
#endif
constexpr uint32_t MQ_FIRST_ROUND = 2;
constexpr uint32_t MQ_ROUND_DONE = 0xFFFFFFF0u;
constexpr uint32_t MQ_ROUND_FAILED = 0xFFFFFFF1u;

enum : uint8_t { QS_OPEN = 0, QS_TAKEN = 1, QS_DEAD = 2 };

KeyMetric key_metric(const swz_ctx* c, const LevelPlan& plan, const SortedPoints& sp) {
  KeyMetric k;
  if (!sp.xyz || !sp.perm) return k;
  if (!c->opt_on("SWZ_MD_KEYS", true)) return k;
  const double ex = plan.root.maxx - plan.root.minx, ey = plan.root.maxy - plan.root.miny, ez = plan.root.maxz - plan.root.minz;
  if (!(ex > 0.0) || ex != ey || ey != ez) return k;
  const double cell = ex / 2097152.0;
  const double T = std::sqrt(plan.sq_spacing) / cell;
  const double tmin = c->opt_num("SWZ_MD_KEYS_MIN_CELLS", 64.0);
  if (!(T >= tmin) || !(T < 4.0e6)) return k;
  double band = 1.75 + T * 0x1.0p-20;
  band += c->opt_num("SWZ_MD_KEYS_BAND", 0.0);
  const double lo = T - band, hi = T + band;
  float f_lo = 0.f;
  if (lo > 0.0) {
    f_lo = (float)(lo * lo);
    while ((double)f_lo > lo * lo) f_lo = std::nextafterf(f_lo, 0.f);
    f_lo = std::nextafterf(f_lo, 0.f);
  }
  float f_hi = (float)(hi * hi);
  while ((double)f_hi < hi * hi) f_hi = std::nextafterf(f_hi, INFINITY);
  f_hi = std::nextafterf(f_hi, INFINITY);
  k.T = T;
  k.f_lo = f_lo;
  k.f_hi = f_hi;
  k.ok = true;
  return k;
}

__global__ __launch_bounds__(256) void mq_point_ids_kernel(const uint32_t* __restrict__ aidx, const uint32_t* __restrict__ perm, uint32_t m,
                                                           uint32_t ghosts, uint32_t* __restrict__ ids) {
  const uint32_t i = blockIdx.x * 256 + threadIdx.x;
  if (i >= m) return;
  const uint32_t s = aidx ? aidx[i] : i;
  ids[i] = s < ghosts ? perm[s] : ghosts + perm[s];
}
int key_point_ids(swz_ctx* c, const ActiveSet& as, const SortedPoints& sp, const uint32_t** ids) {
  if (!as.aidx && !sp.ghosts) {
    *ids = sp.perm;
    return SWZ_OK;
  }
  uint32_t* d = nullptr;
  SWZ_TRY(c->get("md_qids", (size_t)as.m, &d));
  hipLaunchKernelGGL(mq_point_ids_kernel, dim3(div_up(as.m, 256)), dim3(256), 0, c->stream, as.aidx, sp.perm, as.m, sp.ghosts, d);
  SWZ_LAUNCH_CHECK(c);
  *ids = d;
  return SWZ_OK;
}

constexpr uint32_t MQ_PEER_SHIFT = 28;
constexpr uint32_t MQ_ID_MASK = (1u << MQ_PEER_SHIFT) - 1u;
struct MqPeers {
  const uint4* rec[8];
  const uint64_t* qpos[8];
  const uint8_t* state[8];
  const float4* ovf[8];
  const uint32_t* gridmap[8];
  const uint32_t* round_word[8];
  const uint32_t* perm[8];
  const double* xyz[8];
  const uint32_t* aidx[8];
  uint32_t shard, shards;
};

struct MqArgs {
  const uint64_t* akey;
  const uint32_t* aidx;
  uint32_t m;
  const uint32_t* nid;
  const uint8_t* nmode;
  const uint32_t* nstart;
  const double* xyz;
  const uint32_t* perm;
  const double* gxyz;
  uint32_t ng;
  uint8_t* taken;
  uint32_t* counters;
  uint64_t* qpos;
  uint8_t* state;
  uint32_t direct;
  uint32_t cpn_shift;
  uint2* cinfo;
  uint32_t* crel;
  uint32_t* csnode;
  uint32_t* gridmap;
  uint32_t* qnbr;
  uint4* rec;
  float4* ovf;
  unsigned long long* slot;
  uint4* qst;
  uint32_t* queue[2];
  uint32_t* qctr;
  uint32_t* qtotal;
  uint32_t* qhead;
  uint32_t nseg, nseg_shift, segcap;
  const uint32_t* snode_of;
  uint32_t cell_shift;
  uint64_t cells_per_node;
  uint32_t cell_bits;
  uint32_t cell_levels;
  uint32_t rg, rg2_shift;
  float f_lo, f_hi;
  double sq_spacing;
  uint32_t patient;
  float lazy_frac;
  uint32_t all_sampled;
  uint32_t group, groups;
  uint32_t no_dead_test;
  uint32_t stats;
  uint32_t chain;
  uint32_t dense_min;
  uint8_t* dirty;
  uint32_t* bulk_round;
  const uint32_t* dlist;
  uint32_t* round_word;
  MqPeers peers;
};

__device__ __forceinline__ uint32_t uni(uint32_t v) { return (uint32_t)__builtin_amdgcn_readfirstlane((int)v); }
__device__ __forceinline__ uint32_t qb_u32(uint32_t v, int src) { return (uint32_t)__builtin_amdgcn_readlane((int)v, src); }
__device__ __forceinline__ float qb_f32(float v, int src) {
  return __int_as_float(__builtin_amdgcn_readlane(__float_as_int(v), src));
}
__device__ __forceinline__ unsigned long long qb_u64(unsigned long long v, int src) {
  const uint32_t lo = qb_u32((uint32_t)v, src), hi = qb_u32((uint32_t)(v >> 32), src);
  return ((unsigned long long)hi << 32) | lo;
}
template <typename Op>
__device__ __forceinline__ uint32_t mq_wave_scan(uint32_t v, Op op, uint32_t identity) {
  v = op(v, (uint32_t)__builtin_amdgcn_update_dpp((int)identity, (int)v, 0x111, 0xF, 0xF, false));
  v = op(v, (uint32_t)__builtin_amdgcn_update_dpp((int)identity, (int)v, 0x112, 0xF, 0xF, false));
  v = op(v, (uint32_t)__builtin_amdgcn_update_dpp((int)identity, (int)v, 0x114, 0xF, 0xF, false));
  v = op(v, (uint32_t)__builtin_amdgcn_update_dpp((int)identity, (int)v, 0x118, 0xF, 0xF, false));
  v = op(v, (uint32_t)__builtin_amdgcn_update_dpp((int)identity, (int)v, 0x142, 0xA, 0xF, false));
  v = op(v, (uint32_t)__builtin_amdgcn_update_dpp((int)identity, (int)v, 0x143, 0xC, 0xF, false));
  return v;
}
struct MqAdd {
  __device__ uint32_t operator()(uint32_t a, uint32_t b) const { return a + b; }
};
struct MqMax {
  __device__ uint32_t operator()(uint32_t a, uint32_t b) const { return a > b ? a : b; }
};
struct MqMin {
  __device__ uint32_t operator()(uint32_t a, uint32_t b) const { return a < b ? a : b; }
};

__device__ __forceinline__ uint64_t mq_pack(uint64_t key) {
  uint32_t x, y, z;
  key_coords_u32(key, x, y, z);
  return (uint64_t)x | ((uint64_t)y << 21) | ((uint64_t)z << 42);
}
__device__ __forceinline__ void mq_unpack(uint64_t v, float& x, float& y, float& z) {
  const uint32_t lo = (uint32_t)v, hi = (uint32_t)(v >> 32);
  x = (float)(lo & 0x1FFFFFu);
  y = (float)(((lo >> 21) | (hi << 11)) & 0x1FFFFFu);
  z = (float)(hi >> 10);
}
__device__ __forceinline__ float mq_d2(float ax, float ay, float az, float bx, float by, float bz) {
  const float dx = ax - bx, dy = ay - by, dz = az - bz;
  return __builtin_fmaf(dz, dz, __builtin_fmaf(dy, dy, dx * dx));
}
__device__ __forceinline__ bool mq_exact_near(const MqArgs& a, uint32_t i, uint32_t j) {
  const double* p = sorted_point_xyz(a.xyz, a.perm, a.gxyz, a.ng, a.aidx ? a.aidx[i] : i);
  const double* q = sorted_point_xyz(a.xyz, a.perm, a.gxyz, a.ng, a.aidx ? a.aidx[j] : j);
  return sq_dist(p[0], p[1], p[2], q[0], q[1], q[2]) < a.sq_spacing;
}

#ifdef SWZ_MQ_STATS
#define MQ_T(var) const uint64_t var = wall_clock64()
#define MQ_TACC(idx, t0, t1) do { if (l == 0 && (c & 31u) == 0u) atomicAdd(&a.counters[CTR_DBG_HIST + 8 + (idx)], (uint32_t)((t1) - (t0))); } while (0)
#else
#define MQ_T(var) do { } while (0)
#define MQ_TACC(idx, t0, t1) do { } while (0)
#endif
#define MQ_STAT(idx) do { if (a.stats && l == 0) atomicAdd(&a.counters[CTR_DBG_HIST + (idx)], 1u); } while (0)

__device__ __forceinline__ uint4 mq_ld_sys(const uint4* p) {
  const unsigned long long* q = reinterpret_cast<const unsigned long long*>(p);
  const unsigned long long lo = __hip_atomic_load(q, __ATOMIC_RELAXED, __HIP_MEMORY_SCOPE_SYSTEM);
  const unsigned long long hi = __hip_atomic_load(q + 1, __ATOMIC_RELAXED, __HIP_MEMORY_SCOPE_SYSTEM);
  return make_uint4((uint32_t)lo, (uint32_t)(lo >> 32), (uint32_t)hi, (uint32_t)(hi >> 32));
}
__device__ __forceinline__ uint4 mq_ld_agent(const uint4* p) {
  const unsigned long long* q = reinterpret_cast<const unsigned long long*>(p);
  const unsigned long long lo = __hip_atomic_load(q, __ATOMIC_RELAXED, __HIP_MEMORY_SCOPE_AGENT);
  const unsigned long long hi = __hip_atomic_load(q + 1, __ATOMIC_RELAXED, __HIP_MEMORY_SCOPE_AGENT);
  return make_uint4((uint32_t)lo, (uint32_t)(lo >> 32), (uint32_t)hi, (uint32_t)(hi >> 32));
}
__device__ __forceinline__ uint32_t mq_ld_sys(const uint32_t* p) { return __hip_atomic_load(p, __ATOMIC_RELAXED, __HIP_MEMORY_SCOPE_SYSTEM); }

__device__ __forceinline__ bool mq_exact_near_peer(const MqArgs& a, uint32_t i, uint32_t j, uint32_t tag) {
  const double* p = sorted_point_xyz(a.xyz, a.perm, a.gxyz, a.ng, a.aidx ? a.aidx[i] : i);
  const double* q = tag ? a.peers.xyz[tag - 1u] + (size_t)a.peers.perm[tag - 1u][a.peers.aidx[tag - 1u] ? a.peers.aidx[tag - 1u][j] : j] * 3
                        : sorted_point_xyz(a.xyz, a.perm, a.gxyz, a.ng, a.aidx ? a.aidx[j] : j);
  return sq_dist(p[0], p[1], p[2], q[0], q[1], q[2]) < a.sq_spacing;
}

struct MqLds {
  uint4* stage;
  float4* list;
  float4* fresh;
  uint8_t* tag;
  uint32_t* trust;
  uint32_t* sid;
};
constexpr uint32_t MQ_CHAIN = 8;
__host__ __device__ constexpr uint32_t mq_staged(bool peers) { return peers ? 27u : 20u; }
static inline size_t mq_lds_bytes(uint32_t rg, bool peers) {
  return (size_t)(mq_staged(peers) * 2u * rg + MQ_LIST_CAP + MQ_FRESH_CAP) * 16u + MQ_LIST_CAP + MQ_CHAIN * 4u + 128u;
}

__device__ __forceinline__ bool mq_is_head(const MqArgs& a, uint32_t i) {
  if (!a.all_sampled && a.nmode[a.nid[i]] != MODE_SAMPLE) return false;
  return i == 0 || ((a.akey[i] >> a.cell_shift) != (a.akey[i - 1] >> a.cell_shift));
}

__global__ __launch_bounds__(256) void mq_pack_kernel(const uint64_t* __restrict__ akey, uint32_t m, uint64_t* __restrict__ qpos,
                                                      uint8_t* __restrict__ state) {
  const uint32_t i = blockIdx.x * 256 + threadIdx.x;
  if (i >= m) return;
  qpos[i] = mq_pack(akey[i]);
  state[i] = QS_OPEN;
}

struct MqHeadF {
  MqArgs a;
  __device__ uint32_t operator()(uint32_t i) const { return mq_is_head(a, i) ? 1u : 0u; }
};
struct MqCellBuildG {
  MqArgs a;
  __device__ void operator()(uint32_t i, uint32_t c, uint32_t head) const {
    const uint64_t key = a.akey[i];
    a.qpos[i] = mq_pack(key);
    a.state[i] = QS_OPEN;
    if (!head) return;
    a.cinfo[c].x = i;
    a.crel[c] = (uint32_t)((key >> a.cell_shift) & (a.cells_per_node - 1ull));
    a.csnode[c] = a.all_sampled ? a.nid[i] : a.snode_of[a.nid[i]];
  }
};

__global__ __launch_bounds__(256) void mq_direct_build_kernel(MqArgs a, uint32_t vec) {
  const uint64_t i0 = ((uint64_t)blockIdx.x * 256u + threadIdx.x) * 4u;
  if (i0 >= a.m) return;
  const uint32_t n = a.m - i0 < 4u ? (uint32_t)(a.m - i0) : 4u;
  uint64_t key[6];
  uint64_t q[4];
  if (vec && n == 4u) {
    const ulonglong2 v0 = *reinterpret_cast<const ulonglong2*>(a.akey + i0), v1 = *reinterpret_cast<const ulonglong2*>(a.akey + i0 + 2);
    key[1] = v0.x, key[2] = v0.y, key[3] = v1.x, key[4] = v1.y;
  } else {
#pragma unroll
    for (uint32_t j = 0; j < 4u; ++j) key[1 + j] = j < n ? a.akey[i0 + j] : 0ull;
  }
  key[0] = i0 ? a.akey[i0 - 1u] : 0ull;
  key[5] = i0 + 4u < a.m ? a.akey[i0 + 4u] : 0ull;
#pragma unroll
  for (int j = 0; j < 4; ++j) q[j] = mq_pack(key[1 + j]);
  if (n == 4u) {
    ulonglong2 w0, w1;
    w0.x = q[0], w0.y = q[1], w1.x = q[2], w1.y = q[3];
    *reinterpret_cast<ulonglong2*>(a.qpos + i0) = w0;
    *reinterpret_cast<ulonglong2*>(a.qpos + i0 + 2) = w1;
    *reinterpret_cast<uint32_t*>(a.state + i0) = 0x01010101u * (uint32_t)QS_OPEN;
  } else {
    for (uint32_t j = 0; j < n; ++j) {
      a.qpos[i0 + j] = q[j];
      a.state[i0 + j] = QS_OPEN;
    }
  }
#pragma unroll
  for (uint32_t j = 0; j < 4u; ++j) {
    if (j >= n) break;
    const uint32_t i = (uint32_t)i0 + j;
    const uint64_t pre = key[1 + j] >> a.cell_shift;
    const bool first = i == 0u || (key[j] >> a.cell_shift) != pre;
    const bool last = i + 1u == a.m || (key[2 + j] >> a.cell_shift) != pre;
    if (!first && !last) continue;
    const uint32_t node = a.nid[i];
    if (!a.all_sampled && a.nmode[node] != MODE_SAMPLE) continue;
    const uint64_t g = ((uint64_t)(a.all_sampled ? node : a.snode_of[node]) << a.cpn_shift) | (pre & (a.cells_per_node - 1ull));
    if (first) a.cinfo[g].x = i;
    if (last) a.cinfo[g].y = i + 1u;
  }
}

__global__ __launch_bounds__(256) void mq_cell_end_kernel(MqArgs a, uint32_t ncells) {
  const uint32_t c = blockIdx.x * 256 + threadIdx.x;
  if (c >= ncells) return;
  const uint32_t s = a.cinfo[c].x;
  const uint32_t node_end = a.nstart[a.nid[s] + 1];
  const uint32_t next = (c + 1 < ncells) ? a.cinfo[c + 1].x : a.m;
  const uint32_t e = next < node_end ? next : node_end;
  a.cinfo[c].y = e;
  a.gridmap[(uint64_t)a.csnode[c] * a.cells_per_node + a.crel[c]] = c;
  uint4* r = a.rec + ((size_t)c << a.rg2_shift);
  r[0] = make_uint4(s, 0u, 0u, e);
  r[a.rg] = make_uint4(s, 0u, 1u, e);
  a.qst[c] = make_uint4(QNONE, 0u, 0u, 0u);
}

__device__ __forceinline__ void mq_wave_push(bool want, uint32_t value, uint32_t* qout, uint32_t* cout) {
  const uint64_t m = __ballot(want);
  if (!m) return;
  const int leader = __ffsll((unsigned long long)m) - 1;
  uint32_t base = 0;
  if ((int)lane_id() == leader) base = atomicAdd(cout, (uint32_t)__popcll(m));
  base = __shfl(base, leader, WAVE);
  if (want) qout[base + (uint32_t)__popcll(m & lanemask_lt())] = value;
}

struct MqStart {
  uint32_t* queue[8];
  uint32_t* qctr[8];
  uint32_t groups;
  uint32_t lazy;
};

__global__ __launch_bounds__(256) void mq_nbr_build_kernel(MqArgs a, uint32_t ncells, MqStart st) {
  for (uint64_t cbase = (uint64_t)blockIdx.x * 8u; cbase < ncells; cbase += (uint64_t)gridDim.x * 8u) {
    const uint32_t c = (uint32_t)cbase + threadIdx.x / 32u;
    const uint32_t k = threadIdx.x & 31u;
    const bool in_grid = c < ncells;
    bool in = in_grid;
    if (a.direct && in_grid) {
      const uint2 ci = a.cinfo[c];
      if (k < 2u) a.rec[((size_t)c << a.rg2_shift) + k * a.rg] = make_uint4(ci.x, 0u, k, ci.y);
      in = ci.x != ci.y;
    }
    uint32_t nb = QNONE;
    if (in && k == 13u) {
      nb = c;
    } else if (in && k < 27u) {
      const uint32_t rel = a.direct ? (c & (uint32_t)(a.cells_per_node - 1ull)) : a.crel[c];
      const uint32_t all = (uint32_t)(a.cells_per_node - 1ull);
      const uint32_t mz = all & 0x09249249u, my = mz << 1, mx = mz << 2;
      const uint32_t v[3] = {rel & mx, rel & my, rel & mz};
      const uint32_t mk[3] = {mx, my, mz};
      const uint32_t d[3] = {k / 9u, (k / 3u) % 3u, k % 3u};
      bool inside = true;
      uint32_t nrel = 0;
#pragma unroll
      for (int ax = 0; ax < 3; ++ax) {
        uint32_t w = v[ax];
        if (d[ax] == 0u) {
          inside &= w != 0u;
          w = (w - 1u) & mk[ax];
        } else if (d[ax] == 2u) {
          inside &= w != mk[ax];
          w = ((w | ~mk[ax]) + 1u) & mk[ax];
        }
        nrel |= w;
      }
      if (inside) {
        if (a.peers.shards > 1u) {
          const uint32_t owner = (nrel >> (3u * (a.cell_levels - 1u))) * a.peers.shards / 8u;
          if (owner == a.peers.shard) {
            nb = a.gridmap[nrel];
          } else if (owner < a.peers.shard && a.peers.gridmap[owner]) {
            const uint32_t id = a.peers.gridmap[owner][nrel];
            if (id != QNONE) nb = ((owner + 1u) << MQ_PEER_SHIFT) | id;
          }
        } else if (a.direct) {
          const uint32_t g = (c - rel) | nrel;
          const uint2 cn = a.cinfo[g];
          if (cn.x != cn.y) nb = g;
        } else {
          nb = a.gridmap[(uint64_t)a.csnode[c] * a.cells_per_node + nrel];
        }
      }
    }
    if (in) a.qnbr[(size_t)c * 32 + k] = nb;
    uint32_t best = 0;
    if (st.lazy && in && k < 27u && nb != QNONE && (a.peers.shards <= 1u || (nb >> MQ_PEER_SHIFT) == 0u) && nb < c) best = nb + 1u;
    if (st.lazy) {
#pragma unroll
      for (int off = 16; off >= 1; off >>= 1) best = max(best, (uint32_t)__shfl_xor((int)best, off, 32));
      if (in && best && nb + 1u == best) {
        const uint2 o = a.cinfo[best - 1u];
        const uint32_t bq = o.x + (uint32_t)((float)(o.y - 1u - o.x) * a.lazy_frac);
        a.slot[(size_t)(best - 1u) * 32 + (26u - k)] = (unsigned long long)bq;
        a.qst[c] = make_uint4(a.cinfo[c].x, k, bq, 0u);
      }
    }
    if (a.direct && in_grid && k == 2u && best == 0u) a.qst[c] = make_uint4(QNONE, 0u, 0u, 0u);
    const bool push = in && k == 13u && best == 0u;
    const uint32_t seg = (uint32_t)(cbase >> 3) & (a.nseg - 1u);
    if (st.groups == 1u) {
      mq_wave_push(push, c | MQ_WOKEN, st.queue[0] + (size_t)seg * a.segcap, st.qctr[0] + (size_t)seg * 32u);
    } else {
      const uint32_t g = push ? (a.direct ? c >> a.cpn_shift : a.csnode[c]) % st.groups : 0u;
      for (uint32_t gg = 0; gg < st.groups; ++gg)
        mq_wave_push(push && g == gg, c | MQ_WOKEN, st.queue[gg] + (size_t)seg * a.segcap, st.qctr[gg] + (size_t)seg * 32u);
    }
  }
}

template <int SU>
__device__ __forceinline__ uint32_t mq_scan(const MqArgs& a, const uint64_t* __restrict__ qpos, const uint8_t* __restrict__ state,
                                            const MqLds& lds, uint32_t live_wn, uint32_t qs, uint32_t qe, float cx, float cy, float cz) {
  const uint32_t l = lane_id();
  for (uint32_t q0 = qs; q0 < qe; q0 += (uint32_t)SU * WAVE) {
    uint64_t v[SU];
    uint8_t s[SU];
#pragma unroll
    for (int u = 0; u < SU; ++u) {
      const uint32_t q = q0 + (uint32_t)u * WAVE + l;
      const bool inb = q < qe;
      v[u] = inb ? qpos[q] : 0ull;
      s[u] = inb ? state[q] : (uint8_t)QS_DEAD;
    }
#pragma unroll
    for (int u = 0; u < SU; ++u) {
      float x, y, z;
      mq_unpack(v[u], x, y, z);
      bool hit = s[u] != QS_DEAD && mq_d2(x, y, z, cx, cy, cz) < a.f_hi;
      uint64_t hb = __ballot(hit);
      if (hb && live_wn) {
        if (hit) {
          for (uint32_t i = 0; i < live_wn; ++i) {
            const float4 e = lds.list[i];
            if (mq_d2(x, y, z, e.x, e.y, e.z) < a.f_lo) {
              hit = false;
              break;
            }
          }
        }
        hb = __ballot(hit);
      }
      if (hb) return q0 + (uint32_t)u * WAVE + (uint32_t)__ffsll((unsigned long long)hb) - 1u;
    }
  }
  return QNONE;
}

__device__ __forceinline__ uint32_t mq_first_open(const uint8_t* __restrict__ state, uint32_t q0, uint32_t qe) {
  const uint32_t l = lane_id();
  while (q0 < qe) {
    const uint32_t base = q0 & ~15u;
    const uint32_t at = base + l * 16u;
    uint4 sb = make_uint4(0x02020202u, 0x02020202u, 0x02020202u, 0x02020202u);
    if (at < qe) sb = *reinterpret_cast<const uint4*>(state + at);
    const uint32_t w[4] = {sb.x, sb.y, sb.z, sb.w};
    uint32_t first = 16u;
#pragma unroll
    for (int q = 3; q >= 0; --q)
#pragma unroll
      for (int bt = 3; bt >= 0; --bt) {
        const uint32_t idx = at + (uint32_t)q * 4u + (uint32_t)bt;
        if (((w[q] >> (8 * bt)) & 0xFFu) != (uint32_t)QS_DEAD && idx >= q0 && idx < qe) first = (uint32_t)q * 4u + (uint32_t)bt;
      }
    const uint64_t hit = __ballot(first < 16u);
    if (hit) {
      const int hl = __ffsll((unsigned long long)hit) - 1;
      return base + (uint32_t)hl * 16u + qb_u32(first, hl);
    }
    q0 = base + 1024u;
  }
  return qe;
}

template <int SU>
__device__ __forceinline__ uint32_t mq_scan_dense(const MqArgs& a, const uint64_t* __restrict__ qpos, const uint8_t* __restrict__ state,
                                                  const MqLds& lds, uint32_t live_wn, uint32_t qs, uint32_t qe, float cx, float cy, float cz) {
  for (uint32_t q0 = mq_first_open(state, qs, qe); q0 < qe;) {
    const uint32_t wend = (qe - q0) > (uint32_t)SU * WAVE ? q0 + (uint32_t)SU * WAVE : qe;
    const uint32_t hq = mq_scan<SU>(a, qpos, state, lds, live_wn, q0, wend, cx, cy, cz);
    if (hq != QNONE) return hq;
    q0 = mq_first_open(state, wend, qe);
  }
  return QNONE;
}

enum : uint32_t { QO_FINISHED = 0, QO_STALLED = 1, QO_YIELD = 2 };

template <int U, bool PEERS>
__device__ void mq_activate(const MqArgs& a, uint32_t round, uint32_t qentry, const MqLds& lds, uint32_t* qout, uint32_t* cout, uint32_t seg0,
                            uint32_t ntrust, bool may_chain, uint32_t& chain_next) {
  chain_next = QNONE;
  const uint32_t l = lane_id();
  const bool woken = (qentry & MQ_WOKEN) != 0u;
  const uint32_t c = qentry & ~MQ_WOKEN;
  const uint32_t rg = a.rg, rg2s = a.rg2_shift, cap = rg - 1u;
  const float f_lo = a.f_lo, f_hi = a.f_hi;

  MQ_T(t_begin);
  const uint32_t nbv = a.qnbr[(size_t)c * 32 + (l & 31u)];
  const unsigned long long myslot = a.slot[(size_t)c * 32 + (l & 31u)];
  const uint2 ci = a.cinfo[c];
  const uint4 st = a.qst[c];
  uint4* myrec = a.rec + ((size_t)c << rg2s);
  const uint4 h0 = myrec[0], h1 = myrec[rg];
  const uint32_t sbuf = h1.z > h0.z ? 1u : 0u;
  const uint32_t e = ci.y, P = sbuf ? h1.x : h0.x, CNT = sbuf ? h1.y : h0.y;
  if (P >= e) return;
  const bool nb_have = nbv != QNONE;
  const uint32_t nb_peer = (PEERS && nb_have) ? (nbv >> MQ_PEER_SHIFT) : 0u;
  const uint32_t nb_id = PEERS ? (nbv & MQ_ID_MASK) : nbv;
  auto push_again = [&](uint32_t entry) {
    uint32_t base = 0, seg = (seg0 + c * 0x9E3779B1u + (c >> 7)) & (a.nseg - 1u);
    if (l == 0) {
      uint32_t tries = 0;
      for (; tries < a.nseg; ++tries) {
        base = atomicAdd(cout + (size_t)seg * 32u, 1u);
        if (base + 1u <= a.segcap) break;
        seg = (seg + 1u) & (a.nseg - 1u);
      }
      if (tries == a.nseg) atomicMax(&a.counters[CTR_ERROR], (uint32_t)SWZ_ERR_INTERNAL);
      else qout[(size_t)seg * a.segcap + base] = entry;
    }
  };
  bool claimed = woken;

  if (!woken) {
    if (st.x == QNONE || st.w == round) return;
    const uint32_t bk = uni(st.y);
    const uint32_t Bv = qb_u32(nbv, (int)bk);
    const uint32_t Bp = PEERS ? (Bv >> MQ_PEER_SHIFT) : 0u, B = PEERS ? (Bv & MQ_ID_MASK) : Bv;
    if (PEERS && Bp) {
      const uint32_t rb = mq_ld_sys(a.peers.round_word[Bp - 1u]);
      if (rb == MQ_ROUND_FAILED) {
        if (l == 0) atomicMax(&a.counters[CTR_ERROR], (uint32_t)SWZ_ERR_INTERNAL);
        return;
      }
      const uint4* brec = a.peers.rec[Bp - 1u] + ((size_t)B << rg2s);
      const uint4 b0 = mq_ld_sys(brec), b1 = mq_ld_sys(brec + rg);
      const uint32_t ra = mq_ld_sys(a.peers.round_word[Bp - 1u]);
      const bool use1 = b1.z < rb && (b0.z >= rb || b1.z > b0.z);
      const uint4 hb = use1 ? b1 : b0;
      const bool seen = ra == rb && (use1 || b0.z < rb);
      if (!seen || !(hb.x > st.z || hb.x >= hb.w)) {
        push_again(c);
        return;
      }
      claimed = true;
    } else {
    const uint4* brec = a.rec + ((size_t)B << rg2s);
    const uint4 b0 = brec[0], b1 = brec[rg];
    const bool use1 = b1.z < round && (b0.z >= round || b1.z > b0.z);
    const uint4 hb = use1 ? b1 : b0;
    const bool passed = hb.x > st.z || hb.x >= hb.w;
    if (!passed) {
      MQ_STAT(1);
      return;
    }
    const unsigned long long expect = ((unsigned long long)st.w << 32) | st.z;
    unsigned long long old = expect;
    if (l == 0) old = atomicCAS(&a.slot[(size_t)B * 32 + (26u - bk)], expect, QEMPTY);
    old = qb_u64(old, 0);
    if (old != expect) {
      MQ_STAT(2);
      return;
    }
    claimed = true;
    }
  }

  MQ_STAT(0);
  MQ_T(t_rt1);
  MQ_TACC(0, t_begin, t_rt1);
  uint64_t pv[U];
  uint8_t ps[U];
#pragma unroll
  for (int u = 0; u < U; ++u) {
    const uint32_t p = P + (uint32_t)u * WAVE + l;
    const bool inb = p < e;
    pv[u] = inb ? a.qpos[p] : 0ull;
    ps[u] = inb ? a.state[p] : (uint8_t)QS_DEAD;
  }
  const bool valid = l < 27u && nb_have && (nb_peer != 0u || nb_id <= c);
  const uint32_t vmask = (uint32_t)__ballot(valid);
  const uint32_t srank = (uint32_t)__popc(vmask & ((1u << (l & 31u)) - 1u));
  const uint32_t rank13 = (uint32_t)__popc(vmask & ((1u << 13) - 1u));
  if (valid) lds.sid[srank] = nbv;
  __builtin_amdgcn_wave_barrier();
  uint32_t r_before = round;
  if (PEERS && nb_peer && l < 27u) r_before = mq_ld_sys(a.peers.round_word[nb_peer - 1u]);
  {
    const uint32_t ngran = (uint32_t)__popc(vmask) << rg2s;
    constexpr int NT = (int)(mq_staged(PEERS) * 16u + WAVE - 1u) / (int)WAVE;
    uint4 tmp[NT];
#pragma unroll
    for (int j = 0; j < NT; ++j) {
      const uint32_t g = (uint32_t)j * WAVE + l;
      tmp[j] = make_uint4(0u, 0u, 0u, 0u);
      if (g < ngran) {
        const uint32_t nb = lds.sid[g >> rg2s], part = g & ((1u << rg2s) - 1u);
        if (PEERS) {
          const uint32_t np = nb >> MQ_PEER_SHIFT, ni = nb & MQ_ID_MASK;
          if (np) tmp[j] = mq_ld_sys(a.peers.rec[np - 1u] + ((size_t)ni << rg2s) + part);
          else tmp[j] = ntrust ? mq_ld_agent(a.rec + ((size_t)ni << rg2s) + part) : a.rec[((size_t)ni << rg2s) + part];
        } else {
          tmp[j] = ntrust ? mq_ld_agent(a.rec + ((size_t)nb << rg2s) + part) : a.rec[((size_t)nb << rg2s) + part];
        }
      }
    }
#pragma unroll
    for (int j = 0; j < NT; ++j) {
      const uint32_t g = (uint32_t)j * WAVE + l;
      if (g < ngran) lds.stage[g] = tmp[j];
    }
  }
  __builtin_amdgcn_wave_barrier();
  if (PEERS) {
    bool late = false;
    if (nb_peer && l < 27u) late = mq_ld_sys(a.peers.round_word[nb_peer - 1u]) != r_before;
    if (__ballot(PEERS && nb_peer && l < 27u && r_before == MQ_ROUND_FAILED)) {
      if (l == 0) atomicMax(&a.counters[CTR_ERROR], (uint32_t)SWZ_ERR_INTERNAL);
      return;
    }
    if (__ballot(late)) {
      push_again(claimed ? (c | MQ_WOKEN) : c);
      return;
    }
  }

  MQ_T(t_rt2);
  MQ_TACC(1, t_rt1, t_rt2);
  const bool earlier = valid && l != 13u;
  uint32_t n_pos = 0, n_cnt = 0, n_end = 0, pick = 0;
  if (valid) {
    const uint4 a0 = lds.stage[srank << rg2s], a1 = lds.stage[(srank << rg2s) + rg];
    uint32_t rr = (PEERS && nb_peer) ? r_before : round;
    if (ntrust && !(PEERS && nb_peer)) {
      bool mine = false;
      for (uint32_t j = 0; j < ntrust; ++j) mine |= lds.trust[j] == nb_id;
      if (mine) rr = round + 1u;
    }
    pick = (a1.z < rr && (a0.z >= rr || a1.z > a0.z)) ? 1u : 0u;
    const uint4 hd = pick ? a1 : a0;
    n_pos = hd.x;
    n_cnt = hd.y;
    n_end = hd.w;
  }
  const uint32_t my_last = sbuf ? h1.z : h0.z;
  const bool k_new = valid && l != 13u && (nb_peer != 0u || (pick ? lds.stage[(srank << rg2s) + rg].z : lds.stage[srank << rg2s].z) >= my_last);
  const uint32_t incl_new = mq_wave_scan(k_new ? n_cnt : 0u, MqAdd{}, 0u);
  const uint32_t incl_old = mq_wave_scan(k_new ? 0u : n_cnt, MqAdd{}, 0u);
  const uint32_t Tnew = qb_u32(incl_new, WAVE - 1);
  const uint32_t T = Tnew + qb_u32(incl_old, WAVE - 1);
  const uint32_t off = k_new ? incl_new - n_cnt : Tnew + incl_old - n_cnt;
  const uint32_t maxcnt = qb_u32(mq_wave_scan(n_cnt, MqMax{}, 0u), WAVE - 1);
  const uint32_t tested = (st.x != QNONE && my_last >= MQ_FIRST_ROUND) ? st.x : P;
  auto fill = [&](uint32_t base) -> uint32_t {
    __builtin_amdgcn_wave_barrier();
    for (uint32_t j = 0; j < maxcnt && j < cap; ++j) {
      const uint32_t ti = off + j;
      if (j < n_cnt && ti >= base && ti < base + (uint32_t)MQ_LIST_CAP) {
        *reinterpret_cast<uint4*>(&lds.list[ti - base]) = lds.stage[(srank << rg2s) + pick * rg + 1u + j];
        if (PEERS) lds.tag[ti - base] = (uint8_t)nb_peer;
      }
    }
    const float4* ovf = a.ovf;
    if (PEERS) {
      if (nb_peer) ovf = a.peers.ovf[(nb_peer - 1u) & 7u];
    }
    for (uint32_t j0 = cap; j0 < maxcnt; j0 += 2u) {
      const uint32_t ja = j0, jb = j0 + 1u, ta = off + ja, tb = off + jb;
      const bool ma = ja < n_cnt && ta >= base && ta < base + (uint32_t)MQ_LIST_CAP;
      const bool mb = jb < n_cnt && tb >= base && tb < base + (uint32_t)MQ_LIST_CAP;
      uint4 sa = make_uint4(0u, 0u, 0u, 0u), sb = sa;
      if (PEERS && nb_peer) {
        if (ma) sa = mq_ld_sys(reinterpret_cast<const uint4*>(ovf + (n_end - 1u - (ja - cap))));
        if (mb) sb = mq_ld_sys(reinterpret_cast<const uint4*>(ovf + (n_end - 1u - (jb - cap))));
      } else if (ntrust) {
        if (ma) sa = mq_ld_agent(reinterpret_cast<const uint4*>(ovf + (n_end - 1u - (ja - cap))));
        if (mb) sb = mq_ld_agent(reinterpret_cast<const uint4*>(ovf + (n_end - 1u - (jb - cap))));
      } else {
        if (ma) sa = *reinterpret_cast<const uint4*>(ovf + (n_end - 1u - (ja - cap)));
        if (mb) sb = *reinterpret_cast<const uint4*>(ovf + (n_end - 1u - (jb - cap)));
      }
      if (ma) *reinterpret_cast<uint4*>(&lds.list[ta - base]) = sa;
      if (mb) *reinterpret_cast<uint4*>(&lds.list[tb - base]) = sb;
      if (PEERS) {
        if (ma) lds.tag[ta - base] = (uint8_t)nb_peer;
        if (mb) lds.tag[tb - base] = (uint8_t)nb_peer;
      }
    }
    __builtin_amdgcn_wave_barrier();
    return (T - base) < (uint32_t)MQ_LIST_CAP ? (T - base) : (uint32_t)MQ_LIST_CAP;
  };
  const uint32_t wn0 = T ? fill(0u) : 0u;
  uint32_t resident = 0;
  const uint32_t live_wn = (T <= (uint32_t)MQ_LIST_CAP && !a.no_dead_test) ? wn0 : 0u;

  MQ_T(t_fill);
  MQ_TACC(2, t_rt2, t_fill);
  uint32_t fresh = 0;
  uint32_t out_pos = e, out_status = QO_FINISHED, b_k = 0, b_q = 0;
  uint32_t tested_now = P;
  const uint32_t S = 1u << a.cell_bits;

  for (uint32_t W0 = P; W0 < e; W0 += (uint32_t)U * WAVE) {
    float fx[U], fy[U], fz[U];
    uint32_t alive = 0;
    if (W0 != P) {
      while (W0 < e) {
        const uint32_t base = W0 & ~15u;
        const uint32_t at = base + l * 16u;
        uint4 sb = make_uint4(0x02020202u, 0x02020202u, 0x02020202u, 0x02020202u);
        if (at < e) sb = *reinterpret_cast<const uint4*>(a.state + at);
        const uint32_t w[4] = {sb.x, sb.y, sb.z, sb.w};
        uint32_t first = 16u;
#pragma unroll
        for (int q = 3; q >= 0; --q)
#pragma unroll
          for (int bt = 3; bt >= 0; --bt) {
            const uint32_t idx = at + (uint32_t)q * 4u + (uint32_t)bt;
            if (((w[q] >> (8 * bt)) & 0xFFu) == (uint32_t)QS_OPEN && idx >= W0 && idx < e) first = (uint32_t)q * 4u + (uint32_t)bt;
          }
        const uint64_t hit = __ballot(first < 16u);
        if (hit) {
          const int hl = __ffsll((unsigned long long)hit) - 1;
          W0 = base + (uint32_t)hl * 16u + qb_u32(first, hl);
          break;
        }
        W0 = base + 1024u;
      }
      if (W0 >= e) break;
#pragma unroll
      for (int u = 0; u < U; ++u) {
        const uint32_t p = W0 + (uint32_t)u * WAVE + l;
        const bool inb = p < e;
        pv[u] = inb ? a.qpos[p] : 0ull;
        ps[u] = inb ? a.state[p] : (uint8_t)QS_DEAD;
      }
    }
#pragma unroll
    for (int u = 0; u < U; ++u) {
      mq_unpack(pv[u], fx[u], fy[u], fz[u]);
      alive |= (ps[u] == QS_OPEN ? 1u : 0u) << u;
    }
    tested_now = W0 + (uint32_t)U * WAVE;
    if (!__ballot(alive != 0u)) continue;

    {
      float bx0 = 0.f, bx1 = 0.f, by0 = 0.f, by1 = 0.f, bz0 = 0.f, bz1 = 0.f;
      if (U == 1) {
        const bool al = alive & 1u;
        const uint32_t hi_id = 0xFFFFFFFFu;
        bx0 = __uint_as_float(qb_u32(mq_wave_scan(al ? __float_as_uint(fx[0]) : hi_id, MqMin{}, hi_id), WAVE - 1));
        by0 = __uint_as_float(qb_u32(mq_wave_scan(al ? __float_as_uint(fy[0]) : hi_id, MqMin{}, hi_id), WAVE - 1));
        bz0 = __uint_as_float(qb_u32(mq_wave_scan(al ? __float_as_uint(fz[0]) : hi_id, MqMin{}, hi_id), WAVE - 1));
        bx1 = __uint_as_float(qb_u32(mq_wave_scan(al ? __float_as_uint(fx[0]) : 0u, MqMax{}, 0u), WAVE - 1));
        by1 = __uint_as_float(qb_u32(mq_wave_scan(al ? __float_as_uint(fy[0]) : 0u, MqMax{}, 0u), WAVE - 1));
        bz1 = __uint_as_float(qb_u32(mq_wave_scan(al ? __float_as_uint(fz[0]) : 0u, MqMax{}, 0u), WAVE - 1));
      }
      uint32_t oldc = 0;
#pragma unroll
      for (int u = 0; u < U; ++u)
        if (W0 + (uint32_t)(u + 1) * WAVE <= tested) oldc |= 1u << u;
      uint32_t nearb = 0;
      for (uint32_t base = 0;; base += (uint32_t)MQ_LIST_CAP) {
        const bool last = base >= T;
        uint32_t wn = fresh;
        if (!last) {
          if (oldc == (1u << U) - 1u && base >= Tnew) {
            base = T;
            continue;
          }
          if (resident != base) {
            (void)fill(base);
            resident = base;
          }
          wn = (T - base) < (uint32_t)MQ_LIST_CAP ? (T - base) : (uint32_t)MQ_LIST_CAP;
        }
        const float4* lst = last ? lds.fresh : lds.list;
        float dmin[U];
#pragma unroll
        for (int u = 0; u < U; ++u) dmin[u] = __builtin_inff();
        if (U == 1) {
          const uint32_t lim = (last || !(oldc & 1u)) ? wn : (Tnew > base ? ((Tnew - base) < wn ? (Tnew - base) : wn) : 0u);
          for (uint32_t b0 = 0; b0 < lim; b0 += WAVE) {
            bool rel = false;
            if (b0 + l < lim) {
              const float4 en = lst[b0 + l];
              const float gx = fmaxf(fmaxf(bx0 - en.x, en.x - bx1), 0.f);
              const float gy = fmaxf(fmaxf(by0 - en.y, en.y - by1), 0.f);
              const float gz = fmaxf(fmaxf(bz0 - en.z, en.z - bz1), 0.f);
              rel = __builtin_fmaf(gz, gz, __builtin_fmaf(gy, gy, gx * gx)) < f_hi;
            }
            uint64_t rm = __ballot(rel);
            while (rm) {
              const int bit = __ffsll((unsigned long long)rm) - 1;
              rm &= rm - 1ull;
              const float4 en = lst[b0 + (uint32_t)bit];
              dmin[0] = fminf(dmin[0], mq_d2(fx[0], fy[0], fz[0], en.x, en.y, en.z));
            }
          }
        } else {
          const uint32_t nnew = last ? wn : (Tnew > base ? ((Tnew - base) < wn ? (Tnew - base) : wn) : 0u);
          const uint32_t lim = oldc == (1u << U) - 1u ? nnew : wn;
          for (uint32_t i = 0; i < lim; ++i) {
            const float4 en = lst[i];
#pragma unroll
            for (int u = 0; u < U; ++u) dmin[u] = fminf(dmin[u], mq_d2(fx[u], fy[u], fz[u], en.x, en.y, en.z));
          }
        }
        uint32_t pend = 0;
#pragma unroll
        for (int u = 0; u < U; ++u) {
          nearb |= (dmin[u] < f_lo ? 1u : 0u) << u;
          pend |= (dmin[u] >= f_lo && dmin[u] < f_hi ? 1u : 0u) << u;
        }
        pend &= alive & ~nearb;
        if (__ballot(pend != 0u)) {
          for (uint32_t i = 0; i < wn; ++i) {
            const float4 en = lst[i];
#pragma unroll
            for (int u = 0; u < U; ++u) {
              if ((pend >> u) & 1u) {
                const float d2 = mq_d2(fx[u], fy[u], fz[u], en.x, en.y, en.z);
                if (d2 >= f_lo && d2 < f_hi &&
                    ((PEERS && !last) ? mq_exact_near_peer(a, W0 + (uint32_t)u * WAVE + l, __float_as_uint(en.w), lds.tag[i])
                                      : mq_exact_near(a, W0 + (uint32_t)u * WAVE + l, __float_as_uint(en.w)))) {
                  nearb |= 1u << u;
                  pend &= ~(1u << u);
                }
              }
            }
          }
        }
        if (last) break;
      }
      const uint32_t died = alive & nearb;
#pragma unroll
      for (int u = 0; u < U; ++u)
        if ((died >> u) & 1u) a.state[W0 + (uint32_t)u * WAVE + l] = QS_DEAD;
      alive &= ~nearb;
    }

    MQ_T(t_r);
    MQ_TACC(3, t_fill, t_r);
    bool stop = false;
    for (;;) {
      int cu = -1;
      uint64_t bm = 0;
#pragma unroll
      for (int u = 0; u < U; ++u) {
        const uint64_t b = __ballot((alive >> u) & 1u);
        if (cu < 0 && b) {
          cu = u;
          bm = b;
        }
      }
      if (cu < 0) break;
      const int j = __ffsll((unsigned long long)bm) - 1;
      const uint32_t cand = W0 + (uint32_t)cu * WAVE + (uint32_t)j;
      float cx = 0.f, cy = 0.f, cz = 0.f;
#pragma unroll
      for (int u = 0; u < U; ++u) {
        if (u == cu) {
          cx = qb_f32(fx[u], j);
          cy = qb_f32(fy[u], j);
          cz = qb_f32(fz[u], j);
        }
      }
      uint32_t need;
      {
        const uint32_t lx = (uint32_t)cx & (S - 1u), ly = (uint32_t)cy & (S - 1u), lz = (uint32_t)cz & (S - 1u);
        const uint32_t dxk = l / 9u, dyk = (l / 3u) % 3u, dzk = l % 3u;
        const float gx = dxk == 0u ? (float)lx : (dxk == 2u ? (float)(S - 1u - lx) : 0.f);
        const float gy = dyk == 0u ? (float)ly : (dyk == 2u ? (float)(S - 1u - ly) : 0.f);
        const float gz = dzk == 0u ? (float)lz : (dzk == 2u ? (float)(S - 1u - lz) : 0.f);
        const float gap2 = __builtin_fmaf(gz, gz, __builtin_fmaf(gy, gy, gx * gx));
        need = (uint32_t)__ballot(earlier && n_pos < n_end && gap2 < f_hi);
      }
      bool blocked = false;
      while (need && !blocked) {
        const int k = __ffs((int)need) - 1;
        need &= need - 1u;
        const uint32_t qs = qb_u32(n_pos, k), qe = qb_u32(n_end, k);
        MQ_STAT(4);
        const uint32_t kp = PEERS ? qb_u32(nb_peer, k) : 0u;
        uint32_t hq;
        if (U > 1 && a.dense_min && !kp && qe - qs >= a.dense_min)
          hq = mq_scan_dense<4>(a, a.qpos, a.state, lds, live_wn, qs, qe, cx, cy, cz);
        else
          hq = mq_scan<(U > 1 ? 4 : 1)>(a, kp ? a.peers.qpos[kp - 1u] : a.qpos, kp ? a.peers.state[kp - 1u] : a.state, lds, live_wn, qs, qe,
                                        cx, cy, cz);
        if (hq != QNONE) {
          blocked = true;
          b_k = (uint32_t)k;
          b_q = a.patient ? qe - 1u : hq;
        }
      }
      if (blocked) {
        MQ_STAT(3);
        out_pos = cand;
        out_status = QO_STALLED;
        stop = true;
        break;
      }
      if ((int)l == j) {
        a.taken[cand] = 1;
        a.state[cand] = QS_TAKEN;
        alive &= ~(1u << cu);
      }
      if (l == 0) lds.fresh[fresh] = make_float4(cx, cy, cz, __uint_as_float(cand));
      ++fresh;
#pragma unroll
      for (int u = 0; u < U; ++u) {
        if ((alive >> u) & 1u) {
          const float d2 = mq_d2(fx[u], fy[u], fz[u], cx, cy, cz);
          bool nr = d2 < f_lo;
          if (!nr && d2 < f_hi) nr = mq_exact_near(a, W0 + (uint32_t)u * WAVE + l, cand);
          if (nr) {
            a.state[W0 + (uint32_t)u * WAVE + l] = QS_DEAD;
            alive &= ~(1u << u);
          }
        }
      }
      __builtin_amdgcn_wave_barrier();
      if (fresh == (uint32_t)MQ_FRESH_CAP) {
        uint32_t next = W0 + (uint32_t)U * WAVE;
#pragma unroll
        for (int u = U - 1; u >= 0; --u) {
          const uint64_t b = __ballot((alive >> u) & 1u);
          if (b) next = W0 + (uint32_t)u * WAVE + (uint32_t)__ffsll((unsigned long long)b) - 1u;
        }
        if (next < e) {
          out_pos = next;
          out_status = QO_YIELD;
          stop = true;
        }
        break;
      }
    }
    if (stop) break;
    if ((fresh == (uint32_t)MQ_FRESH_CAP || (U > 1 && fresh && a.dense_min && e - ci.x >= a.dense_min)) &&
        W0 + (uint32_t)U * WAVE < e) {
      out_pos = W0 + (uint32_t)U * WAVE;
      out_status = QO_YIELD;
      break;
    }
  }

  MQ_T(t_cand);
  MQ_TACC(4, t_fill, t_cand);
  const uint32_t wb = sbuf ^ 1u;
  const uint32_t ncnt = CNT + fresh;
  __builtin_amdgcn_wave_barrier();
  for (uint32_t j = l; j < ncnt && j < cap; j += WAVE) {
    uint4 src;
    if (j < CNT) src = lds.stage[(rank13 << rg2s) + sbuf * rg + 1u + j];
    else src = *reinterpret_cast<const uint4*>(&lds.fresh[j - CNT]);
    myrec[wb * rg + 1u + j] = src;
  }
  for (uint32_t jj = l; jj < fresh; jj += WAVE) {
    const uint32_t j = CNT + jj;
    if (j >= cap) a.ovf[e - 1u - (j - cap)] = lds.fresh[jj];
  }
  const bool fin = out_pos >= e;
  if (l == 0) {
    myrec[wb * rg] = make_uint4(fin ? e : out_pos, ncnt, round, e);
    a.qst[c] = out_status == QO_STALLED ? make_uint4(tested_now, b_k, b_q, round) : make_uint4(QNONE, 0u, 0u, 0u);
  }
  if (U > 1 && a.dirty && fresh && l < 27u && nb_have && nb_peer == 0u) a.dirty[nb_id] = 1;
  bool won = false;
  if (l < 27u && nb_have && nb_peer == 0u && nb_id > c && myslot != QEMPTY && (uint32_t)(myslot >> 32) != round &&
      (fin || (uint32_t)myslot < out_pos)) {
    won = atomicCAS(&a.slot[(size_t)c * 32 + l], myslot, QEMPTY) == myslot;
  }
  if (out_status == QO_STALLED && l == 0) {
    const uint32_t Bv = qb_u32(nbv, (int)uni(b_k));
    if (!(PEERS && (Bv >> MQ_PEER_SHIFT))) a.slot[(size_t)(PEERS ? (Bv & MQ_ID_MASK) : Bv) * 32 + (26u - b_k)] = ((unsigned long long)round << 32) | b_q;
  }
  uint64_t wm = __ballot(won);
  if (may_chain && wm) {
    const int first = __ffsll((unsigned long long)wm) - 1;
    chain_next = qb_u32(nb_id, first);
    wm &= wm - 1ull;
    if ((int)l == first) won = false;
  }
  const uint32_t self = fin ? 0u : 1u;
  const uint32_t total = (uint32_t)__popcll(wm) + self;
  if (total) {
    uint32_t base = 0, seg = (seg0 + c * 0x9E3779B1u + (c >> 7)) & (a.nseg - 1u);
    if (l == 0) {
      uint32_t tries = 0;
      for (; tries < a.nseg; ++tries) {
        base = atomicAdd(cout + (size_t)seg * 32u, total);
        if (base + total <= a.segcap) break;
        seg = (seg + 1u) & (a.nseg - 1u);
      }
      if (tries == a.nseg) {
        atomicMax(&a.counters[CTR_ERROR], (uint32_t)SWZ_ERR_INTERNAL);
        base = QNONE;
      }
    }
    base = qb_u32(base, 0);
    seg = qb_u32(seg, 0);
    if (base != QNONE) {
      uint32_t* q = qout + (size_t)seg * a.segcap + base;
      if (won) q[(uint32_t)__popcll(wm & lanemask_lt())] = nb_id | MQ_WOKEN;
      if (self && l == 0) q[(uint32_t)__popcll(wm)] = out_status == QO_YIELD ? (c | MQ_WOKEN) : c;
    }
  }
  MQ_T(t_end);
  MQ_TACC(5, t_cand, t_end);
  MQ_TACC(6, t_begin, t_end);
#ifdef SWZ_MQ_STATS
  if (l == 0 && (c & 31u) == 0u) atomicAdd(&a.counters[CTR_DBG_HIST + 8 + 7], 1u);
#endif
}

template <int U, bool PEERS>
__global__ __launch_bounds__(WAVE, (U == 1 && !PEERS) ? MQ_MINW1 : ((U == 4 && !PEERS) ? MQ_MINW4 : 4)) void mq_sweep_kernel(MqArgs a, uint32_t round) {
  extern __shared__ uint4 mq_smem[];
  MqLds lds;
  lds.stage = mq_smem;
  lds.list = reinterpret_cast<float4*>(mq_smem + mq_staged(PEERS) * 2u * a.rg);
  lds.fresh = lds.list + MQ_LIST_CAP;
  lds.tag = reinterpret_cast<uint8_t*>(lds.fresh + MQ_FRESH_CAP);
  lds.trust = reinterpret_cast<uint32_t*>(lds.tag + MQ_LIST_CAP);
  lds.sid = lds.trust + MQ_CHAIN;
  const uint32_t r0 = round - MQ_FIRST_ROUND;
  const uint32_t ci = r0 % 3u, co = (r0 + 1u) % 3u, cz = (r0 + 2u) % 3u;
  if (blockIdx.x == 0) {
    const uint32_t l = lane_id();
    uint32_t mine = 0;
    for (uint32_t sg = l; sg < a.nseg; sg += WAVE) {
      a.qctr[((size_t)cz * a.nseg + sg) * 32u] = 0;
      a.qhead[((size_t)cz * a.nseg + sg) * 32u] = 0;
      const uint32_t n = a.qctr[((size_t)ci * a.nseg + sg) * 32u];
      mine += n < a.segcap ? n : a.segcap;
    }
    const uint32_t tot = qb_u32(mq_wave_scan(mine, MqAdd{}, 0u), WAVE - 1);
    if (l == 0) a.qtotal[ci] = tot;
  }
  const uint32_t seg = blockIdx.x & (a.nseg - 1u);
  uint32_t nq = a.qctr[((size_t)ci * a.nseg + seg) * 32u];
  nq = nq < a.segcap ? nq : a.segcap;
  const uint32_t* qin = a.queue[r0 & 1u] + (size_t)seg * a.segcap;
  uint32_t* qout = a.queue[(r0 + 1u) & 1u];
  uint32_t* cout = a.qctr + (size_t)co * a.nseg * 32u;
  uint32_t* head = a.qhead + ((size_t)ci * a.nseg + seg) * 32u;
  uint32_t i = blockIdx.x >> a.nseg_shift;
  const uint32_t wgs = gridDim.x >> a.nseg_shift;
  uint32_t entry = qin[i < a.segcap ? i : 0u];
  while (i < nq) {
    uint32_t next = 0;
    if (lane_id() == 0) next = atomicAdd(head, 1u);
    uint32_t cur = uni(entry), ntrust = 0;
    for (;;) {
      uint32_t woke = QNONE;
      mq_activate<U, PEERS>(a, round, cur, lds, qout, cout, seg, ntrust, ntrust + 1u < a.chain, woke);
      woke = uni(woke);
      if (woke == QNONE) break;
      if (lane_id() == 0) lds.trust[ntrust] = cur & ~MQ_WOKEN;
      ++ntrust;
      asm volatile("s_waitcnt vmcnt(0)" ::: "memory");
      __builtin_amdgcn_wave_barrier();
      cur = woke | MQ_WOKEN;
    }
    i = wgs + qb_u32(next, 0);
    if (i < nq) entry = qin[i];
  }
}

__global__ __launch_bounds__(256) void mq_dense_list_kernel(MqArgs a, uint32_t ncells, uint32_t* __restrict__ list, uint32_t* __restrict__ count) {
  const uint32_t c = blockIdx.x * 256 + threadIdx.x;
  if (c >= ncells) return;
  const uint2 ci = a.cinfo[c];
  if (ci.y - ci.x >= a.dense_min) list[atomicAdd(count, 1u)] = c;
}

constexpr uint32_t MQ_DENSE_LIST = 256;
__global__ __launch_bounds__(256) void mq_dense_reject_kernel(MqArgs a, uint32_t round) {
  __shared__ float4 lst[MQ_DENSE_LIST];
  __shared__ uint32_t cnt;
  const uint32_t c = a.dlist[blockIdx.x];
  if (!a.dirty[c]) return;
  const uint32_t tid = threadIdx.x;
  const uint32_t rg = a.rg, rg2s = a.rg2_shift, cap = rg - 1u;
  const uint4* myrec = a.rec + ((size_t)c << rg2s);
  const uint4 h0 = myrec[0], h1 = myrec[rg];
  const uint4 mine = h1.z > h0.z ? h1 : h0;
  const uint32_t P = mine.x, e = a.cinfo[c].y;
  const uint32_t since = a.bulk_round[c];
  if (tid == 0) cnt = 0;
  __syncthreads();
  if (tid == 0) {
    a.dirty[c] = 0;
    a.bulk_round[c] = round + 1u;
  }
  if (P >= e) return;
  if (tid < 27u) {
    const uint32_t nb = a.qnbr[(size_t)c * 32 + tid];
    if (nb != QNONE && nb <= c) {
      const uint4* r = a.rec + ((size_t)nb << rg2s);
      const uint4 a0 = r[0], a1 = r[rg];
      const uint32_t pick = a1.z > a0.z ? 1u : 0u;
      const uint4 hd = pick ? a1 : a0;
      if (hd.z >= since && hd.y) {
        const uint32_t at = atomicAdd(&cnt, hd.y);
        for (uint32_t j = 0; j < hd.y && at + j < MQ_DENSE_LIST; ++j) {
          uint4 en;
          if (j < cap) en = r[pick * rg + 1u + j];
          else en = *reinterpret_cast<const uint4*>(a.ovf + (hd.w - 1u - (j - cap)));
          lst[at + j] = make_float4(__uint_as_float(en.x), __uint_as_float(en.y), __uint_as_float(en.z), 0.f);
        }
      }
    }
  }
  __syncthreads();
  const uint32_t n = cnt < MQ_DENSE_LIST ? cnt : MQ_DENSE_LIST;
  if (!n) return;
  for (uint32_t p = P + tid; p < e; p += 256u) {
    if (a.state[p] != QS_OPEN) continue;
    float x, y, z;
    mq_unpack(a.qpos[p], x, y, z);
    bool dead = false;
    for (uint32_t i = 0; i < n && !dead; ++i) dead = mq_d2(x, y, z, lst[i].x, lst[i].y, lst[i].z) < a.f_lo;
    if (dead) a.state[p] = QS_DEAD;
  }
}

__global__ void mq_round_word_kernel(uint32_t* word, uint32_t value) {
  __hip_atomic_store(word, value, __ATOMIC_RELAXED, __HIP_MEMORY_SCOPE_SYSTEM);
}

__global__ __launch_bounds__(256) void mq_verify_kernel(MqArgs a, uint32_t ncells, uint32_t* __restrict__ open_cells) {
  const uint32_t c = blockIdx.x * 256 + threadIdx.x;
  bool open = false;
  if (c < ncells) {
    const uint4* r = a.rec + ((size_t)c << a.rg2_shift);
    const uint4 h0 = r[0], h1 = r[a.rg];
    const uint4 h = h1.z > h0.z ? h1 : h0;
    open = h.x < h.w;
  }
  const uint64_t bm = __ballot(open);
  if (bm && lane_id() == 0) atomicAdd(open_cells, (uint32_t)__popcll(bm));
}

bool min_distance_level_uses_keys(const swz_ctx* c, const LevelPlan& plan, const SortedPoints& sp) {
  return key_metric(c, plan, sp).ok;
}

int min_distance_keys_level(swz_ctx* c, const MdLevel& L, int cl, uint32_t* rounds_out, bool* used, const MdShardRoot* shard_root) {
  *used = false;
  const LevelPlan& plan = L.plan;
  const ActiveSet& as = L.as;
  const SortedPoints& sp = L.sp;
  const LevelBuffers& lb = L.lb;
  const KeyMetric& km = L.km;
  const uint32_t sample_nodes = L.sample_nodes, sample_points = L.sample_points;
  const double typical_pop = L.pop[std::min(3, plan.cell_levels_geo - cl)];
  const uint32_t est_cells = L.occupied[cl];
  if (!km.ok) return SWZ_OK;
  const bool sharded = shard_root != nullptr && shard_root->shards > 1;
  const std::string sfx = sharded ? "_sr" : "";
  const uint32_t m = as.m;
  MqArgs a{};
  a.akey = as.akey;
  a.aidx = as.aidx;
  a.m = m;
  a.nid = lb.nid;
  a.nmode = lb.nmode;
  a.nstart = lb.nstart;
  a.xyz = sp.xyz;
  a.perm = sp.perm;
  a.gxyz = sp.ghost_xyz;
  a.ng = sp.ghosts;
  a.taken = lb.taken;
  a.counters = lb.counters;
  a.snode_of = L.snode_of;
  a.cells_per_node = 1ull << (3 * cl);
  a.cpn_shift = 3u * (uint32_t)cl;
  a.cell_levels = (uint32_t)cl;
  a.peers.shards = sharded ? (uint32_t)shard_root->shards : 1u;
  a.peers.shard = sharded ? (uint32_t)shard_root->shard : 0u;
  a.cell_shift = plan.node_shift - 3u * (uint32_t)cl;
  a.cell_bits = a.cell_shift / 3u;
  a.f_lo = km.f_lo;
  a.f_hi = km.f_hi;
  a.sq_spacing = plan.sq_spacing;
  a.all_sampled = L.all_sampled ? 1u : 0u;
  a.no_dead_test = c->opt_on("SWZ_MD_NO_DEAD_TEST", false) ? 1u : 0u;
  a.stats = c->opt("SWZ_MD_STATS") ? 1u : 0u;
  a.chain = std::min<uint32_t>(MQ_CHAIN, (uint32_t)std::max(1L, c->opt_int("SWZ_MD_CHAIN", 2)));
  if (a.cell_bits > 21u) return SWZ_OK;

  ProfScope ps(c, "sample_min_distance", (uint64_t)sample_points * 33ull, 1);
  const double r_cell = std::ldexp(1.0, (int)a.cell_bits) / km.T;
  a.rg = (0.75 * r_cell * r_cell * r_cell <= 12.0) ? 4u : 8u;
  a.rg = c->opt_int("SWZ_MD_KEYS_RG", a.rg) >= 8 ? 8u : 4u;
  a.rg2_shift = a.rg == 4u ? 3u : 4u;
  const uint64_t grid_entries = (uint64_t)sample_nodes * a.cells_per_node;
  {
    const size_t per_cell = sizeof(uint2) + 32u * 4u + 2u * a.rg * sizeof(uint4) + 32u * 8u + sizeof(uint4) + 5u;
    uint64_t max_cells = 0x7FFFFFF0ull;
    if (const char* mc = c->opt("SWZ_MD_DIRECT_MAX_CELLS")) {
      max_cells = std::min<uint64_t>(max_cells, (uint64_t)std::max(0LL, atoll(mc)));
    } else {
      size_t free_b = 0, total_b = 0, held = 0;
      if (hipMemGetInfo(&free_b, &total_b) != hipSuccess) free_b = 0;
      for (const auto& kv : c->bufs)
        if (!kv.second.host && kv.first.compare(0, 4, "md_q") == 0) held += kv.second.cap;
      max_cells = std::min<uint64_t>(max_cells, (uint64_t)((double)(free_b + held) * 0.9 / (double)per_cell));
    }
    const double occupancy = (double)est_cells / (double)std::max<uint64_t>(1, grid_entries);
    bool direct = occupancy >= c->opt_num("SWZ_MD_DIRECT_MIN_OCCUPANCY", 0.5);
    if (const char* f = c->opt("SWZ_MD_DIRECT")) direct = atoi(f) != 0;
    a.direct = (direct && !sharded && grid_entries <= max_cells) ? 1u : 0u;
  }
  *used = true;
  uint32_t ncells = 0;
  uint32_t* d_cell_sums = nullptr;
  if (a.direct) {
    if (sample_points == 0) return SWZ_OK;
    ncells = (uint32_t)grid_entries;
  } else {
    SWZ_TRY(fused_scan_sums(c, MqHeadF{a}, m, lb.counters + CTR_NUM_CELLS, "mqc", &d_cell_sums));
    SWZ_HIP(c, hipMemcpyAsync(&ncells, lb.counters + CTR_NUM_CELLS, 4, hipMemcpyDeviceToHost, c->stream));
    SWZ_HIP(c, hipStreamSynchronize(c->stream));
    if (ncells == 0) return SWZ_OK;
    if (ncells >= 0x7FFFFFFFu) {
      *used = false;
      return SWZ_OK;
    }
  }
  const uint32_t occ_cells = a.direct ? std::max(1u, std::min<uint32_t>(est_cells, ncells)) : ncells;

  SWZ_TRY(c->get(("md_qpos" + sfx).c_str(), (size_t)m, &a.qpos));
  SWZ_TRY(c->get(("md_qstate" + sfx).c_str(), (size_t)m, &a.state));
  SWZ_TRY(c->get(("md_qovf" + sfx).c_str(), (size_t)m, &a.ovf));
  SWZ_TRY(c->get(("md_qcinfo" + sfx).c_str(), (size_t)ncells, &a.cinfo));
  if (!a.direct) {
    uint32_t* cellbuf = nullptr;
    SWZ_TRY(c->get(("md_qcells" + sfx).c_str(), (size_t)ncells * 2, &cellbuf));
    a.crel = cellbuf;
    a.csnode = cellbuf + ncells;
  }
  SWZ_TRY(c->get(("md_qnbr" + sfx).c_str(), (size_t)ncells * 32, &a.qnbr));
  SWZ_TRY(c->get(("md_qrec" + sfx).c_str(), (size_t)ncells * 2 * a.rg, &a.rec));
  SWZ_TRY(c->get(("md_qslot" + sfx).c_str(), (size_t)ncells * 32, &a.slot));
  SWZ_TRY(c->get(("md_qst" + sfx).c_str(), (size_t)ncells, &a.qst));
  SWZ_HIP(c, memset_large(a.slot, 0xFF, (size_t)ncells * 32 * sizeof(unsigned long long), c->stream));
  const uint32_t cb = div_up(ncells, 256);
  if (a.direct) {
    SWZ_HIP(c, memset_large(a.cinfo, 0, (size_t)ncells * sizeof(uint2), c->stream));
    hipLaunchKernelGGL(mq_direct_build_kernel, dim3(div_up(m, 1024)), dim3(256), 0, c->stream, a,
                       ((uintptr_t)a.akey & 15u) == 0 ? 1u : 0u);
    SWZ_LAUNCH_CHECK(c);
  } else {
    SWZ_TRY(c->get(("md_gridmap" + sfx).c_str(), (size_t)grid_entries, &a.gridmap));
    SWZ_HIP(c, memset_large(a.gridmap, 0xFF, (size_t)grid_entries * 4, c->stream));
    SWZ_TRY(fused_scan_apply(c, MqHeadF{a}, MqCellBuildG{a}, m, d_cell_sums));
    hipLaunchKernelGGL(mq_cell_end_kernel, dim3(cb), dim3(256), 0, c->stream, a, ncells);
    SWZ_LAUNCH_CHECK(c);
  }
  struct WordGuard {
    swz_ctx* c;
    uint32_t* word = nullptr;
    bool done = false;
    ~WordGuard() {
      if (word && !done) {
        hipLaunchKernelGGL(mq_round_word_kernel, dim3(1), dim3(1), 0, c->stream, word, MQ_ROUND_FAILED);
        (void)hipStreamSynchronize(c->stream);
      }
    }
  } word_guard{c};
  if (sharded) {
    MdPeerView& mine = shard_root->views[shard_root->shard];
    int my_status = SWZ_OK;
    if (cl < 1 || ncells >= (1u << MQ_PEER_SHIFT) || sample_nodes != 1) my_status = SWZ_ERR_INTERNAL;
    const uint32_t* aidx_sr = nullptr;
    if (as.aidx) {
      uint32_t* cp = nullptr;
      SWZ_TRY(c->get("md_qaidx_sr", (size_t)m, &cp));
      SWZ_HIP(c, hipMemcpyAsync(cp, as.aidx, (size_t)m * 4, hipMemcpyDeviceToDevice, c->stream));
      aidx_sr = cp;
    }
    SWZ_TRY(c->get("md_qround_sr", (size_t)32, &a.round_word));
    hipLaunchKernelGGL(mq_round_word_kernel, dim3(1), dim3(1), 0, c->stream, a.round_word, MQ_FIRST_ROUND);
    SWZ_LAUNCH_CHECK(c);
    SWZ_HIP(c, hipStreamSynchronize(c->stream));
    mine.rec = a.rec;
    mine.qpos = a.qpos;
    mine.state = a.state;
    mine.ovf = a.ovf;
    mine.gridmap = a.gridmap;
    mine.round_word = a.round_word;
    mine.perm = a.perm;
    mine.xyz = a.xyz;
    mine.aidx = aidx_sr;
    mine.ncells = ncells;
    mine.npoints = m;
    mine.rg = a.rg;
    mine.cell_shift = a.cell_shift;
    mine.status = my_status;
    mine.entered = 1;
    word_guard.word = a.round_word;
    shard_root->barrier(shard_root->barrier_arg);
    for (int p = 0; p < shard_root->shards; ++p) {
      const MdPeerView& v = shard_root->views[p];
      if (v.status != SWZ_OK || (v.ncells && (v.rg != a.rg || v.cell_shift != a.cell_shift)))
        return c->fail(SWZ_ERR_INTERNAL, "MIN_DISTANCE root of a sharded batch: shard " + std::to_string(p) +
                                           " cannot take part in the joint sweep (cell levels, cell count or record size differ)");
      if (p < shard_root->shard && v.ncells) {
        a.peers.rec[p] = v.rec;
        a.peers.qpos[p] = v.qpos;
        a.peers.state[p] = v.state;
        a.peers.ovf[p] = v.ovf;
        a.peers.gridmap[p] = v.gridmap;
        a.peers.round_word[p] = v.round_word;
        a.peers.perm[p] = v.perm;
        a.peers.xyz[p] = v.xyz;
        a.peers.aidx[p] = v.aidx;
      }
    }
  }
  const bool many_small = occ_cells >= (4u << 20) && (double)sample_points / (double)occ_cells <= 128.0;
  a.patient = (uint32_t)c->opt_int("SWZ_MD_PATIENT", many_small ? 1 : 0);
  const bool lazy = c->opt_on("SWZ_MD_LAZY", true);
  a.lazy_frac = (float)c->opt_num("SWZ_MD_LAZY_FRAC", many_small ? 0.5 : 0.0);
  const bool big_cells = c->opt_on("SWZ_MD_BIG", typical_pop > 256.0);
  uint32_t groups = 1;
  if (sample_nodes >= 2 && !big_cells) groups = 2;
  groups = (uint32_t)std::max(1L, std::min(8L, c->opt_int("SWZ_MD_GROUPS", groups)));
  groups = std::min(groups, sample_nodes);
  if (sharded) groups = 1;
  uint32_t ndense = 0;
  a.dense_min = 0;
  a.dirty = nullptr;
  if (big_cells && groups == 1 && !sharded) {
    const uint32_t dense_min = (uint32_t)std::max(0L, c->opt_int("SWZ_MD_DENSE_MIN", 4096));
    if (dense_min && m >= dense_min) {
      uint32_t* dl = nullptr;
      uint32_t* dcount = nullptr;
      SWZ_TRY(c->get("md_qdense", (size_t)(m / dense_min + 1u), &dl));
      SWZ_TRY(c->get("md_qdense_count", (size_t)4, &dcount));
      SWZ_HIP(c, hipMemsetAsync(dcount, 0, 4, c->stream));
      a.dense_min = dense_min;
      hipLaunchKernelGGL(mq_dense_list_kernel, dim3(cb), dim3(256), 0, c->stream, a, ncells, dl, dcount);
      SWZ_LAUNCH_CHECK(c);
      SWZ_HIP(c, hipMemcpyAsync(&ndense, dcount, 4, hipMemcpyDeviceToHost, c->stream));
      SWZ_HIP(c, hipStreamSynchronize(c->stream));
      if (ndense) {
        SWZ_TRY(c->get("md_qdirty", (size_t)ncells, &a.dirty));
        SWZ_TRY(c->get("md_qbulk", (size_t)ncells, &a.bulk_round));
        SWZ_HIP(c, hipMemsetAsync(a.dirty, 0, (size_t)ncells, c->stream));
        SWZ_HIP(c, hipMemsetAsync(a.bulk_round, 0, (size_t)ncells * 4, c->stream));
        a.dlist = dl;
      } else {
        a.dense_min = 0;
      }
    }
  }
  a.nseg_shift = 5;
  a.nseg = 1u << a.nseg_shift;
  a.segcap = (uint32_t)std::min<uint64_t>(0x7FFFFFF0ull, 2ull * ncells / a.nseg + 4096ull);
  std::vector<MqArgs> ga(groups, a);
  std::vector<hipStream_t> gs(groups, c->stream);
  for (uint32_t g = 0; g < groups; ++g) {
    ga[g].group = g;
    ga[g].groups = groups;
    const std::string tag = std::to_string(g);
    SWZ_TRY(c->get(("md_qqueue0_g" + tag).c_str(), (size_t)a.nseg * a.segcap, &ga[g].queue[0]));
    SWZ_TRY(c->get(("md_qqueue1_g" + tag).c_str(), (size_t)a.nseg * a.segcap, &ga[g].queue[1]));
    SWZ_TRY(c->get(("md_qctr_g" + tag).c_str(), (size_t)6 * a.nseg * 32 + 32, &ga[g].qctr));
    ga[g].qhead = ga[g].qctr + (size_t)3 * a.nseg * 32;
    ga[g].qtotal = ga[g].qctr + (size_t)6 * a.nseg * 32;
    SWZ_HIP(c, hipMemsetAsync(ga[g].qctr, 0, ((size_t)6 * a.nseg * 32 + 32) * sizeof(uint32_t), c->stream));
    if (g > 0) {
      SWZ_TRY(c->get(("md_counters_g" + tag).c_str(), (size_t)CTR_COUNT, &ga[g].counters));
      SWZ_HIP(c, hipMemsetAsync(ga[g].counters, 0, CTR_COUNT * sizeof(uint32_t), c->stream));
      while (c->aux_streams.size() < g) {
        hipStream_t stn = nullptr;
        SWZ_HIP(c, hipStreamCreateWithFlags(&stn, hipStreamNonBlocking));
        c->aux_streams.push_back(stn);
      }
      gs[g] = c->aux_streams[g - 1];
    }
  }
  {
    MqStart start{};
    start.groups = groups;
    start.lazy = lazy ? 1u : 0u;
    for (uint32_t g = 0; g < groups; ++g) {
      start.queue[g] = ga[g].queue[0];
      start.qctr[g] = ga[g].qctr;
    }
    hipLaunchKernelGGL(mq_nbr_build_kernel, dim3(std::min<uint32_t>(div_up(ncells, 8), 1u << 20)), dim3(256), 0, c->stream, ga[0], ncells, start);
    SWZ_LAUNCH_CHECK(c);
    SWZ_STAGE(c, "mq tables");
  }
  const bool dbg = c->opt("SWZ_DEBUG") != nullptr;
  if (dbg)
    fprintf(stderr, "[swz] MIN_DISTANCE level %d on keys: %u pts in %u nodes, %u cells%s (cell levels %d), spacing %.1f key cells, band "
                    "[%.0f, %.0f), records of %u, typical cell %.0f pts, lazy %d (%.2f) patient %u groups %u big %d dense cells %u\n",
            plan.level, sample_points, sample_nodes, ncells, a.direct ? " of the grid, numbered directly" : "", cl, km.T, (double)km.f_lo, (double)km.f_hi, a.rg - 1u, typical_pop, (int)lazy,
            (double)a.lazy_frac, a.patient, groups, (int)big_cells, ndense);
  hipEvent_t ev0 = nullptr, ev1 = nullptr;
  if (dbg) {
    ev0 = c->take_event();
    ev1 = c->take_event();
    (void)hipEventRecord(ev0, c->stream);
  }
  const size_t lds_bytes = mq_lds_bytes(a.rg, sharded);
  uint32_t sweep_grid = 0;
  {
    int dev = 0, cus = 0, per_cu = 0;
    (void)hipGetDevice(&dev);
    (void)hipDeviceGetAttribute(&cus, hipDeviceAttributeMultiprocessorCount, dev);
    const hipError_t oe = big_cells ? hipOccupancyMaxActiveBlocksPerMultiprocessor(&per_cu, mq_sweep_kernel<4, false>, WAVE, lds_bytes)
                                    : hipOccupancyMaxActiveBlocksPerMultiprocessor(&per_cu, mq_sweep_kernel<1, false>, WAVE, lds_bytes);
    if (oe != hipSuccess || per_cu < 1) per_cu = 8;
    if (cus < 1) cus = 256;
    uint32_t cap = (uint32_t)cus * (uint32_t)per_cu;
    if (const char* e = c->opt("SWZ_MD_GRID")) cap = (uint32_t)std::max(1, atoi(e)) * 4u;
    sweep_grid = std::max(a.nseg, (std::min<uint32_t>(cap / groups, ncells) + a.nseg - 1u) / a.nseg * a.nseg);
  }
  uint32_t batch = 32, batches_done = 0;
  const bool fixed_batch = c->opt("SWZ_MD_BATCH") != nullptr;
  if (fixed_batch) batch = std::max(1u, (uint32_t)c->opt_int("SWZ_MD_BATCH", 0));
  const auto wall0 = std::chrono::steady_clock::now();
  const double wall_limit = c->opt_num("SWZ_MD_TIME_LIMIT", 900.0);
  uint64_t max_rounds = 8ull * m + 1024;
  if (sharded) {
    uint64_t below = 0;
    for (int p = 0; p < shard_root->shard; ++p) below += shard_root->views[p].npoints;
    max_rounds += 64ull * below + 65536ull;
  }
  max_rounds = (uint64_t)c->opt_int("SWZ_MD_ROUND_LIMIT", (long)max_rounds);
  hipEvent_t fork = nullptr;
  if (groups > 1) {
    fork = c->take_event();
    SWZ_HIP(c, hipEventRecord(fork, c->stream));
    for (uint32_t g = 1; g < groups; ++g) SWZ_HIP(c, hipStreamWaitEvent(gs[g], fork, 0));
  }
  std::vector<uint32_t> gleft(groups, 1);
  uint32_t round = MQ_FIRST_ROUND;
  bool running = true;
  while (running) {
    for (uint32_t b = 0; b < batch; ++b, ++round) {
      for (uint32_t g = 0; g < groups; ++g) {
        if (sharded) {
          hipLaunchKernelGGL(mq_round_word_kernel, dim3(1), dim3(1), 0, gs[g], a.round_word, round);
          if (big_cells)
            hipLaunchKernelGGL((mq_sweep_kernel<4, true>), dim3(sweep_grid), dim3(WAVE), lds_bytes, gs[g], ga[g], round);
          else
            hipLaunchKernelGGL((mq_sweep_kernel<1, true>), dim3(sweep_grid), dim3(WAVE), lds_bytes, gs[g], ga[g], round);
        } else if (big_cells) {
          hipLaunchKernelGGL((mq_sweep_kernel<4, false>), dim3(sweep_grid), dim3(WAVE), lds_bytes, gs[g], ga[g], round);
          if (ndense) hipLaunchKernelGGL(mq_dense_reject_kernel, dim3(ndense), dim3(256), 0, gs[g], ga[g], round);
        } else {
          hipLaunchKernelGGL((mq_sweep_kernel<1, false>), dim3(sweep_grid), dim3(WAVE), lds_bytes, gs[g], ga[g], round);
        }
      }
    }
    SWZ_LAUNCH_CHECK(c);
    if (!fixed_batch && ++batches_done % 4u == 0u && batch < 128u) batch *= 2u;
    for (uint32_t g = 0; g < groups; ++g)
      SWZ_HIP(c, hipMemcpyAsync(&gleft[g], ga[g].qtotal + (round - 1u - MQ_FIRST_ROUND) % 3u, 4, hipMemcpyDeviceToHost, gs[g]));
    uint32_t peer_err = 0;
    if (sharded) SWZ_HIP(c, hipMemcpyAsync(&peer_err, ga[0].counters + CTR_ERROR, 4, hipMemcpyDeviceToHost, gs[0]));
    running = false;
    for (uint32_t g = 0; g < groups; ++g) {
      SWZ_HIP(c, hipStreamSynchronize(gs[g]));
      running |= gleft[g] != 0u;
    }
    if (peer_err) return c->fail(SWZ_ERR_INTERNAL, "MIN_DISTANCE root of a sharded batch: a lower shard's sweep failed (or a queue overflowed); this shard gives up as well");
    if (std::chrono::duration<double>(std::chrono::steady_clock::now() - wall0).count() > wall_limit) {
      char msg[200];
      snprintf(msg, sizeof(msg), "MIN_DISTANCE sweep on keys exceeded %.0f s: level %d, %u cells, %u rounds", wall_limit, plan.level,
               ncells, round);
      return c->fail(SWZ_ERR_INTERNAL, msg);
    }
    if (round > max_rounds) {
      char msg[160];
      snprintf(msg, sizeof(msg), "MIN_DISTANCE sweep on keys did not terminate: level %d, %u cells, %u rounds", plan.level, ncells, round);
      return c->fail(SWZ_ERR_INTERNAL, msg);
    }
  }
  if (fork) c->event_pool.push_back(fork);
  if (sharded) {
    hipLaunchKernelGGL(mq_round_word_kernel, dim3(1), dim3(1), 0, c->stream, a.round_word, MQ_ROUND_DONE);
    word_guard.done = true;
    SWZ_LAUNCH_CHECK(c);
  }
  {
    uint32_t* d_open = nullptr;
    SWZ_TRY(c->get("md_qopen", (size_t)4, &d_open));
    SWZ_HIP(c, hipMemsetAsync(d_open, 0, 4, c->stream));
    hipLaunchKernelGGL(mq_verify_kernel, dim3(cb), dim3(256), 0, c->stream, a, ncells, d_open);
    SWZ_LAUNCH_CHECK(c);
    uint32_t open_cells = 0, err = 0;
    SWZ_HIP(c, hipMemcpyAsync(&open_cells, d_open, 4, hipMemcpyDeviceToHost, c->stream));
    for (uint32_t g = 0; g < groups; ++g) {
      uint32_t eg = 0;
      SWZ_HIP(c, hipMemcpyAsync(&eg, ga[g].counters + CTR_ERROR, 4, hipMemcpyDeviceToHost, c->stream));
      SWZ_HIP(c, hipStreamSynchronize(c->stream));
      err |= eg;
    }
    if (open_cells || err) {
      char msg[200];
      snprintf(msg, sizeof(msg), "MIN_DISTANCE sweep on keys ended with %u of %u cells undecided at level %d after %u rounds (queue overflow: %s)",
               open_cells, ncells, plan.level, round - MQ_FIRST_ROUND, err ? "yes" : "no");
      return c->fail(SWZ_ERR_INTERNAL, msg);
    }
  }
  if (rounds_out) *rounds_out += round - MQ_FIRST_ROUND;
  if (dbg) {
    float ms = 0.f;
    (void)hipEventRecord(ev1, c->stream);
    (void)hipEventSynchronize(ev1);
    (void)hipEventElapsedTime(&ms, ev0, ev1);
    c->event_pool.push_back(ev0);
    c->event_pool.push_back(ev1);
    fprintf(stderr, "[swz] MIN_DISTANCE level %d on keys: sweep %.2f ms, %u rounds\n", plan.level, ms, round - MQ_FIRST_ROUND);
    for (uint32_t g = 0; g < groups; ++g) {
      uint32_t h[CTR_COUNT];
      SWZ_HIP(c, hipMemcpy(h, ga[g].counters, sizeof(h), hipMemcpyDeviceToHost));
      fprintf(stderr, "[swz]   group %u: %u full activations, %u confirms still asleep, %u confirms that lost the claim, %u stalls, %u scans\n", g,
              h[CTR_DBG_HIST], h[CTR_DBG_HIST + 1], h[CTR_DBG_HIST + 2], h[CTR_DBG_HIST + 3], h[CTR_DBG_HIST + 4]);
#ifdef SWZ_MQ_STATS
      {
        const double ns = std::max(1u, h[CTR_DBG_HIST + 15]) * 100.0;
        fprintf(stderr, "[swz]   timed %u full activations (us): first loads %.2f, records + window %.2f, list %.2f, first window (R) %.2f, "
                        "windows + candidates + scans %.2f, publish + wake %.2f, total %.2f\n", h[CTR_DBG_HIST + 15], h[CTR_DBG_HIST + 8] / ns,
                h[CTR_DBG_HIST + 9] / ns, h[CTR_DBG_HIST + 10] / ns, h[CTR_DBG_HIST + 11] / ns, h[CTR_DBG_HIST + 12] / ns, h[CTR_DBG_HIST + 13] / ns,
                h[CTR_DBG_HIST + 14] / ns);
      }
#endif
    }
  }
  return SWZ_OK;
}

}
```

schwarzwald_amd/csrc/swz_session.h:

```cpp
#pragma once
#include "swz_level.h"

namespace swz {

struct TileSession {
  uint32_t n = 0;
  double bmin[3] = {0, 0, 0}, bmax[3] = {0, 0, 0};
  swz_tile_params params{};
  uint64_t* keys = nullptr;
  uint32_t* perm = nullptr;
  int8_t* level = nullptr;
  uint32_t* dup = nullptr;
  const double* xyz_in = nullptr;
  SortedPoints sp;
  LevelBuffers lb;
  uint64_t* key_buf[2] = {nullptr, nullptr};
  uint32_t* idx_buf[2] = {nullptr, nullptr};
  int which = 0;
  ActiveSet as;
  int next_level = -1;
  uint64_t visited = 0, nodes = 0;
  uint32_t rounds = 0, nlevels = 0;
  int max_level = -1;
  int fast_start = -1;
  uint32_t ghosts = 0;
  uint32_t front = 0;
};

int session_prepare(swz_ctx* c, TileSession& t, double* d_xyz, uint32_t n, const double bmin[3], const double bmax[3],
                    const swz_tile_params& p, const TileDeviceOut& out, uint32_t front = 0);
int session_run_levels(swz_ctx* c, TileSession& t, int last_level, int first_mode);
void session_stats(const TileSession& t, swz_tile_stats* stats);

__device__ __forceinline__ bool recon_candidate(const int8_t* level, const uint32_t* dup, uint32_t i, int start_node_level,
                                                uint32_t child_bit) {
  return child_bit ? (dup[i] & child_bit) != 0 : level[i] == (int8_t)start_node_level;
}
int session_recon_ranks(swz_ctx* c, TileSession& t, int S, uint32_t child_bit, uint32_t* pos);
int session_fast_reconstruct(swz_ctx* c, TileSession& t, const swz_tile_params& p, int S, int lowest_lv);

}
```

schwarzwald_amd/csrc/swz_session.hip:

```cpp
#include <algorithm>
#include <string>
#include <vector>

#include "swz_md.h"
#include "swz_session.h"

namespace swz {

static int session_gather_positions(swz_ctx* c, TileSession& t) {
  if (t.sp.X) return SWZ_OK;
  double *X = nullptr, *Y = nullptr, *Z = nullptr;
  SWZ_TRY(c->get("sorted_x", (size_t)t.n + t.front, &X));
  SWZ_TRY(c->get("sorted_y", (size_t)t.n + t.front, &Y));
  SWZ_TRY(c->get("sorted_z", (size_t)t.n + t.front, &Z));
  SWZ_STAGE(c, "sort");
  const uint32_t g = t.sp.ghosts;
  if (g) {
    if (t.next_level <= -1) SWZ_TRY(gather_positions(c, t.sp.ghost_xyz, t.perm, g, X, Y, Z));
    SWZ_TRY(gather_positions(c, t.xyz_in, t.perm + g, t.n - g, X + g, Y + g, Z + g));
  } else {
    X += t.front;
    Y += t.front;
    Z += t.front;
    SWZ_TRY(gather_positions(c, t.xyz_in, t.perm, t.n, X, Y, Z));
  }
  SWZ_STAGE(c, "gather");
  t.sp.X = X;
  t.sp.Y = Y;
  t.sp.Z = Z;
  return SWZ_OK;
}
static int session_need_positions(swz_ctx* c, TileSession& t, const LevelPlan& plan) {
  if (t.sp.X || level_decides_on_keys(c, plan, t.sp)) return SWZ_OK;
  return session_gather_positions(c, t);
}

int session_prepare(swz_ctx* c, TileSession& t, double* d_xyz, uint32_t n, const double bmin[3], const double bmax[3],
                    const swz_tile_params& p, const TileDeviceOut& out, uint32_t front) {
  t = TileSession{};
  t.n = n;
  for (int a = 0; a < 3; ++a) {
    t.bmin[a] = bmin[a];
    t.bmax[a] = bmax[a];
  }
  t.params = p;
  t.keys = out.keys;
  t.perm = out.perm;
  t.level = out.level;
  t.dup = out.dup;
  t.xyz_in = d_xyz;
  uint64_t* keys_b = nullptr;
  uint32_t* vals_b = nullptr;
  SWZ_TRY(c->get("sort_keys_b", (size_t)n, &keys_b));
  SWZ_TRY(c->get("sort_vals_b", (size_t)n, &vals_b));
  SWZ_TRY(encode_device(c, d_xyz, n, bmin, bmax, keys_b));
  SWZ_STAGE(c, "encode");
  SWZ_TRY(radix_sort_pairs(c, keys_b, vals_b, out.keys, out.perm, n, true));
  t.sp = SortedPoints{nullptr, nullptr, nullptr, d_xyz, out.perm};
  t.front = front;
  const LevelPlan top = make_plan(-1, p.sampler, p.max_points_per_node, p.spacing_at_root, p.max_depth, bmin, bmax, false, true);
  SWZ_TRY(session_need_positions(c, t, top));
  if (out.dup) SWZ_HIP(c, hipMemsetAsync(out.dup, 0, (size_t)n * 4, c->stream));
  SWZ_HIP(c, hipMemsetAsync(out.level, 0x80, (size_t)n, c->stream));
  SWZ_TRY(alloc_level_buffers(c, n + front, &t.lb));
  t.key_buf[0] = keys_b;
  t.idx_buf[0] = vals_b;
  t.as = ActiveSet{out.keys, nullptr, n};
  return SWZ_OK;
}

int session_run_levels(swz_ctx* c, TileSession& t, int last_level, int first_mode) {
  const uint64_t* pprefix = nullptr;
  uint32_t parents = 0;
  for (int level = t.next_level; t.as.m > 0 && level <= last_level; ++level) {
    if (level > 20) return c->fail(SWZ_ERR_INTERNAL, "level loop ran past level 20");
    if (!t.key_buf[t.which]) {
      SWZ_TRY(c->get("active_keys_2", (size_t)t.as.m, &t.key_buf[t.which]));
      SWZ_TRY(c->get("active_idx_2", (size_t)t.as.m, &t.idx_buf[t.which]));
    }
    LevelPlan plan = make_plan(level, t.params.sampler, t.params.max_points_per_node, t.params.spacing_at_root,
                               t.params.max_depth, t.bmin, t.bmax, false, true);
    plan.md_property = (t.params.flags & SWZ_FLAG_MIN_DISTANCE_PROPERTY) != 0;
    if (first_mode >= 0 && level == t.next_level) plan.md_property = false;
    if (first_mode >= 0 && level == t.next_level && !plan.terminal) {
      if (first_mode == 1) {
        plan.force_sample = true;
      } else {
        plan.max_points = ~0ull;
      }
    }
    SWZ_TRY(session_need_positions(c, t, plan));
    LevelResult r;
    t.as.parent_prefix = pprefix;
    t.as.parents = pprefix ? parents : 0u;
    SWZ_TRY(level_step(c, plan, t.as, t.sp, t.lb, t.level, t.key_buf[t.which], t.idx_buf[t.which], &r));
    t.visited += t.as.m;
    t.nodes += r.num_nodes;
    t.rounds += r.md_rounds;
    t.max_level = level;
    ++t.nlevels;
    t.as = ActiveSet{t.key_buf[t.which], t.idx_buf[t.which], r.remaining};
    pprefix = r.node_prefix;
    parents = r.num_nodes;
    t.which ^= 1;
    t.next_level = level + 1;
  }
  return SWZ_OK;
}

void session_stats(const TileSession& t, swz_tile_stats* stats) {
  if (!stats) return;
  stats->num_nodes = t.nodes;
  stats->points_visited = t.visited;
  stats->max_level = t.max_level;
  stats->fast_start_levels = t.fast_start;
  stats->num_levels = t.nlevels;
  stats->min_distance_rounds = t.rounds;
}

__global__ __launch_bounds__(256) void prefix_bounds_kernel(const uint64_t* __restrict__ keys, uint32_t n,
                                                            uint32_t* __restrict__ starts, uint32_t nbins) {
  const uint32_t b = blockIdx.x * 256 + threadIdx.x;
  if (b > nbins) return;
  if (b == nbins) {
    starts[b] = n;
    return;
  }
  const uint64_t target = (uint64_t)b << 45;
  uint32_t lo = 0, hi = n;
  while (lo < hi) {
    const uint32_t mid = lo + (hi - lo) / 2;
    if (keys[mid] < target) lo = mid + 1; else hi = mid;
  }
  starts[b] = lo;
}

static size_t estimate_start_level_host(const std::vector<uint32_t>& starts6, size_t concurrency) {
  constexpr uint32_t MIN_LEVEL = 3, MAX_LEVEL = 6;
  constexpr float MIN_SCORE = 1.f;
  for (uint32_t level = 0; level < MAX_LEVEL; ++level) {
    const uint32_t digits = level + 1;
    const uint32_t group = 1u << (3 * (6 - digits));
    size_t ranges = 0, large = 0;
    for (uint32_t b = 0; b < (1u << 18); b += group) {
      const uint32_t cnt = starts6[b + group] - starts6[b];
      if (cnt > 0) ++ranges;
      if (cnt >= 100000) ++large;
    }
    float score = 0.f;
    if (!(ranges <= concurrency / 2)) score = static_cast<float>(large) / static_cast<float>(concurrency);
    if (score >= MIN_SCORE) return std::max(level + 1, MIN_LEVEL);
  }
  return MAX_LEVEL;
}

__global__ __launch_bounds__(256) void recon_select_kernel(const int8_t* __restrict__ level,
                                                           const uint32_t* __restrict__ dup, uint32_t n,
                                                           int start_node_level, uint32_t child_bit,
                                                           uint32_t* __restrict__ flags) {
  const uint32_t i = blockIdx.x * 256 + threadIdx.x;
  if (i >= n) return;
  flags[i] = recon_candidate(level, dup, i, start_node_level, child_bit) ? 1u : 0u;
}
__global__ __launch_bounds__(256) void recon_gather_kernel(const uint64_t* __restrict__ keys, uint32_t n,
                                                           const uint32_t* __restrict__ flags_in_scanned,
                                                           const int8_t* __restrict__ level,
                                                           const uint32_t* __restrict__ dup, int start_node_level,
                                                           uint32_t child_bit, uint64_t* __restrict__ okey,
                                                           uint32_t* __restrict__ oidx) {
  const uint32_t i = blockIdx.x * 256 + threadIdx.x;
  if (i >= n) return;
  if (recon_candidate(level, dup, i, start_node_level, child_bit)) {
    const uint32_t o = flags_in_scanned[i];
    okey[o] = keys[i];
    oidx[o] = i;
  }
}
__global__ __launch_bounds__(256) void recon_mark_kernel(const uint32_t* __restrict__ aidx, uint32_t m,
                                                         const uint8_t* __restrict__ taken, uint32_t bit,
                                                         uint32_t* __restrict__ dup) {
  const uint32_t i = blockIdx.x * 256 + threadIdx.x;
  if (i < m && taken[i]) dup[aidx[i]] |= bit;
}

int fast_prefix_counts(swz_ctx* c, const uint64_t* d_keys_sorted, uint32_t n, uint32_t* counts_host) {
  const uint32_t nbins = 1u << 18;
  uint32_t* d_starts = nullptr;
  SWZ_TRY(c->get("fast_starts", (size_t)nbins + 1, &d_starts));
  std::vector<uint32_t> starts(nbins + 1, 0);
  if (n) {
    hipLaunchKernelGGL(prefix_bounds_kernel, dim3(div_up(nbins + 1, 256)), dim3(256), 0, c->stream, d_keys_sorted, n, d_starts, nbins);
    SWZ_LAUNCH_CHECK(c);
    SWZ_HIP(c, hipMemcpyAsync(starts.data(), d_starts, (nbins + 1) * 4, hipMemcpyDeviceToHost, c->stream));
    SWZ_HIP(c, hipStreamSynchronize(c->stream));
  }
  for (uint32_t b = 0; b < nbins; ++b) counts_host[b] = starts[b + 1] - starts[b];
  return SWZ_OK;
}
int fast_start_level_from_counts(const uint64_t* counts, uint32_t concurrency) {
  std::vector<uint32_t> starts((1u << 18) + 1, 0);
  uint64_t run = 0;
  for (uint32_t b = 0; b < (1u << 18); ++b) {
    starts[b] = (uint32_t)std::min<uint64_t>(run, 0xFFFFFFFFull);
    run += counts[b];
  }
  starts[1u << 18] = (uint32_t)std::min<uint64_t>(run, 0xFFFFFFFFull);
  return (int)estimate_start_level_host(starts, concurrency);
}

int fast_start_level(swz_ctx* c, const uint64_t* d_keys_sorted, uint32_t n, uint32_t concurrency, int* start_level) {
  const uint32_t nbins = 1u << 18;
  uint32_t* d_starts = nullptr;
  SWZ_TRY(c->get("fast_starts", (size_t)nbins + 1, &d_starts));
  hipLaunchKernelGGL(prefix_bounds_kernel, dim3(div_up(nbins + 1, 256)), dim3(256), 0, c->stream, d_keys_sorted, n,
                     d_starts, nbins);
  SWZ_LAUNCH_CHECK(c);
  std::vector<uint32_t> starts(nbins + 1);
  SWZ_HIP(c, hipMemcpyAsync(starts.data(), d_starts, (nbins + 1) * 4, hipMemcpyDeviceToHost, c->stream));
  SWZ_HIP(c, hipStreamSynchronize(c->stream));
  *start_level = (int)estimate_start_level_host(starts, concurrency);
  return SWZ_OK;
}

int session_recon_ranks(swz_ctx* c, TileSession& t, int S, uint32_t child_bit, uint32_t* pos) {
  hipLaunchKernelGGL(recon_select_kernel, dim3(div_up(t.n, 256)), dim3(256), 0, c->stream, t.level, t.dup, t.n, S - 1, child_bit, pos);
  SWZ_LAUNCH_CHECK(c);
  SWZ_HIP(c, hipMemsetAsync(t.lb.counters, 0, CTR_COUNT * sizeof(uint32_t), c->stream));
  return scan_exclusive_u32(c, pos, pos, t.n, t.lb.counters + CTR_REMAINING, "rec");
}

int session_fast_reconstruct(swz_ctx* c, TileSession& t, const swz_tile_params& p, int S, int lowest_lv) {
  const uint32_t n = t.n;
  const double* bmin = t.bmin;
  const double* bmax = t.bmax;
  uint64_t* rkey = nullptr;
  uint32_t* ridx = nullptr;
  SWZ_TRY(c->get("recon_keys", (size_t)n, &rkey));
  SWZ_TRY(c->get("recon_idx", (size_t)n, &ridx));
  const uint32_t nb = div_up(n, 256);
  for (int lv = S - 1; lv >= lowest_lv; --lv) {
    const uint32_t child_bit = (lv + 1 == S) ? 0u : (1u << (lv + 1));
    SWZ_TRY(session_recon_ranks(c, t, S, child_bit, t.lb.flags));
    hipLaunchKernelGGL(recon_gather_kernel, dim3(nb), dim3(256), 0, c->stream, t.keys, n, t.lb.flags, t.level, t.dup,
                       S - 1, child_bit, rkey, ridx);
    SWZ_LAUNCH_CHECK(c);
    uint32_t m = 0;
    SWZ_TRY(read_u32(c, t.lb.counters + CTR_REMAINING, &m));
    if (m == 0) continue;
    LevelPlan plan = make_plan(lv - 1, p.sampler, p.max_points_per_node, p.spacing_at_root, p.max_depth, bmin,
                               bmax, true, false);
    plan.md_property = (p.flags & SWZ_FLAG_MIN_DISTANCE_PROPERTY) != 0;
    ActiveSet as{rkey, ridx, m};
    SWZ_TRY(session_need_positions(c, t, plan));
    LevelResult r;
    SWZ_TRY(level_step(c, plan, as, t.sp, t.lb, nullptr, nullptr, nullptr, &r));
    hipLaunchKernelGGL(recon_mark_kernel, dim3(div_up(m, 256)), dim3(256), 0, c->stream, ridx, m, t.lb.taken,
                       1u << lv, t.dup);
    SWZ_LAUNCH_CHECK(c);
    t.nodes += r.num_nodes;
    t.rounds += r.md_rounds;
  }
  return SWZ_OK;
}

int tile_device(swz_ctx* c, double* d_xyz, uint32_t n, const double bmin[3], const double bmax[3],
                const swz_tile_params& p, const TileDeviceOut& out_in, swz_tile_stats* stats) {
  TileDeviceOut out = out_in;
  if (p.strategy == SWZ_FAST && !out.dup) SWZ_TRY(c->get("fast_dup", (size_t)n, &out.dup));
  TileSession t;
  SWZ_TRY(session_prepare(c, t, d_xyz, n, bmin, bmax, p, out));
  if (p.strategy == SWZ_ACCURATE) {
    SWZ_TRY(session_run_levels(c, t, 20, -1));
    session_stats(t, stats);
    return SWZ_OK;
  }
  int S = 0;
  SWZ_TRY(fast_start_level(c, t.keys, n, p.fast_concurrency, &S));
  t.fast_start = S;
  t.next_level = S - 1;
  SWZ_TRY(session_run_levels(c, t, 20, -1));
  SWZ_TRY(session_fast_reconstruct(c, t, p, S, 0));
  session_stats(t, stats);
  return SWZ_OK;
}

__global__ __launch_bounds__(256) void count_taken_kernel(const uint8_t* __restrict__ taken, uint32_t n,
                                                          uint32_t* __restrict__ count) {
  const uint32_t i = blockIdx.x * 256 + threadIdx.x;
  const bool t = (i < n) && taken[i];
  const uint64_t b = __ballot(t);
  if (lane_id() == 0 && b) atomicAdd(count, (uint32_t)__popcll(b));
}

__global__ __launch_bounds__(256) void node_key_check_kernel(const uint64_t* __restrict__ keys, uint32_t n, uint32_t nsh,
                                                             uint64_t prefix, uint32_t* __restrict__ bad) {
  const uint32_t i = blockIdx.x * 256 + threadIdx.x;
  const bool b = i < n && (keys[i] >> nsh) != prefix;
  const uint64_t m = __ballot(b);
  if (lane_id() == 0 && m) atomicAdd(bad, (uint32_t)__popcll(m));
}

int sample_points_device(swz_ctx* c, int sampler, uint64_t max_points, const uint64_t* d_keys, const uint32_t* d_idx,
                         uint32_t n, const double* d_xyz, uint64_t node_key, int32_t node_level,
                         const double rmin[3], const double rmax[3], float spacing, int behaviour, uint8_t* d_taken,
                         uint64_t* num_taken) {
  const bool uses_node_key = greedy_sampler(sampler) || sampler == SWZ_JITTERED;
  if (node_level >= 0 && uses_node_key) {
    uint32_t* d_bad = nullptr;
    SWZ_TRY(c->get("lvl_counters", (size_t)CTR_COUNT, &d_bad));
    SWZ_HIP(c, hipMemsetAsync(d_bad, 0, sizeof(uint32_t), c->stream));
    const uint32_t nsh = level_shift(node_level);
    hipLaunchKernelGGL(node_key_check_kernel, dim3(div_up(n, 256)), dim3(256), 0, c->stream, d_keys, n, nsh,
                       node_key >> nsh, d_bad);
    SWZ_LAUNCH_CHECK(c);
    uint32_t bad = 0;
    SWZ_TRY(read_u32(c, d_bad, &bad));
    if (bad) return c->fail(SWZ_ERR_BAD_ARG, "swz_sample_points: " + std::to_string(bad) + " keys of the range do not lie in node_key's node");
  }
  double *X = nullptr, *Y = nullptr, *Z = nullptr;
  SWZ_TRY(c->get("sorted_x", (size_t)n, &X));
  SWZ_TRY(c->get("sorted_y", (size_t)n, &Y));
  SWZ_TRY(c->get("sorted_z", (size_t)n, &Z));
  SWZ_TRY(gather_positions(c, d_xyz, d_idx, n, X, Y, Z));
  LevelBuffers lb;
  SWZ_TRY(alloc_level_buffers(c, n, &lb));
  LevelPlan plan = make_plan(node_level, sampler, max_points, spacing, 100, rmin, rmax,
                             behaviour == SWZ_ALWAYS_ADHERE_TO_MIN_SPACING, false);
  if (!uses_node_key) plan.node_shift = 63;
  ActiveSet as{d_keys, nullptr, n};
  SortedPoints sp{X, Y, Z, d_xyz, d_idx};
  LevelResult r;
  SWZ_TRY(level_step(c, plan, as, sp, lb, nullptr, nullptr, nullptr, &r));
  SWZ_HIP(c, hipMemcpyAsync(d_taken, lb.taken, n, hipMemcpyDeviceToDevice, c->stream));
  if (num_taken) {
    SWZ_HIP(c, hipMemsetAsync(lb.counters, 0, sizeof(uint32_t), c->stream));
    hipLaunchKernelGGL(count_taken_kernel, dim3(div_up(n, 256)), dim3(256), 0, c->stream, lb.taken, n, lb.counters);
    SWZ_LAUNCH_CHECK(c);
    uint32_t cnt = 0;
    SWZ_TRY(read_u32(c, lb.counters, &cnt));
    *num_taken = cnt;
  }
  return SWZ_OK;
}

}
```

Before: 2603.

## Defer per-level compaction across min-distance levels using gone masks

When a min-distance level removes only a small fraction of points, the compaction of active keys and indices is skipped. The next level runs on the same arrays, with a per-point 'gone' code in the taken buffer, tile-prefix live counts, and qpos reused from the previous level. A chain flush compacts everything when a later level cannot handle shared arrays. This targets the per-level scan and scatter bandwidth, at the cost of extra live-count scans, a commit kernel, and wasted work on dead points.

```diff
diff --git a/schwarzwald_amd/csrc/swz_api.hip b/schwarzwald_amd/csrc/swz_api.hip
--- a/schwarzwald_amd/csrc/swz_api.hip
+++ b/schwarzwald_amd/csrc/swz_api.hip
@@ -86,6 +86,7 @@
 
 void swz_ctx::free_buf(swz::DevBuf& b) {
   if (b.ptr && b.ptr == sbi_clean_ptr) sbi_clean_ptr = nullptr;
+  if (b.ptr && b.ptr == mq_qpos_buf) mq_qpos_buf = nullptr;
   if (b.ptr) (void)(b.host ? hipHostFree(b.ptr) : hipFree(b.ptr));
   b.ptr = nullptr;
   b.cap = 0;
diff --git a/schwarzwald_amd/csrc/swz_internal.h b/schwarzwald_amd/csrc/swz_internal.h
--- a/schwarzwald_amd/csrc/swz_internal.h
+++ b/schwarzwald_amd/csrc/swz_internal.h
@@ -80,6 +80,9 @@
   bool md_shard_root_published = false;
   const void* sbi_clean_ptr = nullptr;
   size_t sbi_clean_bytes = 0;
+  const void* mq_qpos_buf = nullptr;
+  const void* mq_qpos_keys = nullptr;
+  uint32_t mq_qpos_m = 0;
   bool tiler_active = false;
   swz_tiler* nodes_tiler = nullptr;
   bool tiler_scratch_dead = false;
diff --git a/schwarzwald_amd/csrc/swz_level.h b/schwarzwald_amd/csrc/swz_level.h
--- a/schwarzwald_amd/csrc/swz_level.h
+++ b/schwarzwald_amd/csrc/swz_level.h
@@ -16,6 +16,7 @@
   CTR_REMAINING = 4,
   CTR_NUM_CELLS = 5,
   CTR_DONE_CELLS = 6,
+  CTR_LIVE_NODES = 7,
   CTR_Q0 = 8,
   CTR_DBG_TIME = 20,
   CTR_DBG_TMAX = 21,
@@ -36,6 +37,13 @@
   uint32_t child_nn = 0;
   const uint64_t* parent_prefix = nullptr;
   uint32_t parents = 0;
+  const uint8_t* gone = nullptr;
+  const uint32_t* gone_tiles = nullptr;
+  uint32_t live = 0;
+};
+struct LevelChain {
+  bool may_defer = false;
+  double max_gone = 0.125;
 };
 
 struct SortedPoints {
@@ -78,6 +86,7 @@
   double spacing_node = 0.0;
   uint32_t jitter_start = 0;
   double sq_spacing = 0.0;
+  uint8_t take_code = 1;
   int cell_levels_geo = 0;
 };
 
@@ -94,6 +103,11 @@
   uint32_t remaining = 0;
   uint32_t num_nodes = 0;
   uint32_t md_rounds = 0;
+  uint32_t table_nodes = 0;
+  bool md_keys_direct = false;
+  bool deferred = false;
+  const uint32_t* gone_tiles = nullptr;
+  bool needs_flush = false;
   const uint64_t* node_prefix = nullptr;
 };
 
@@ -102,7 +116,9 @@
 int alloc_level_buffers(swz_ctx* c, uint32_t m, LevelBuffers* lb);
 int required_depth_host(int sampler, int node_level, double root_extent_x, float root_max_spacing);
 int level_step(swz_ctx* c, const LevelPlan& plan, const ActiveSet& as, const SortedPoints& sp, const LevelBuffers& lb,
-               int8_t* level_out, uint64_t* okey, uint32_t* oidx, LevelResult* res);
+               int8_t* level_out, uint64_t* okey, uint32_t* oidx, LevelResult* res, const LevelChain* chain = nullptr);
+int level_flush_chain(swz_ctx* c, const ActiveSet& as, const LevelBuffers& lb, int8_t* level_out, uint64_t* okey, uint32_t* oidx,
+                      uint32_t* remaining);
 const char* level_error_message(int code);
 int fast_start_level(swz_ctx* c, const uint64_t* d_keys_sorted, uint32_t n, uint32_t concurrency, int* start_level);
 int fast_prefix_counts(swz_ctx* c, const uint64_t* d_keys_sorted, uint32_t n, uint32_t* counts_host);
@@ -113,7 +129,7 @@
 bool grid_level_uses_keys(const swz_ctx* c, const LevelPlan& plan, const SortedPoints& sp);
 int min_distance_level(swz_ctx* c, const LevelPlan& plan, const ActiveSet& as, const SortedPoints& sp,
                        const LevelBuffers& lb, uint32_t num_nodes, uint32_t sample_nodes,
-                       uint32_t sample_points, uint32_t* rounds_out);
+                       uint32_t sample_points, uint32_t* rounds_out, bool* keys_direct = nullptr, bool* needs_flush = nullptr);
 int min_distance_fast_level(swz_ctx* c, const LevelPlan& plan, const ActiveSet& as, const SortedPoints& sp, const LevelBuffers& lb,
                             uint32_t stride, uint32_t num_nodes, uint32_t sample_nodes, uint32_t* rounds_out);
 
diff --git a/schwarzwald_amd/csrc/swz_level.hip b/schwarzwald_amd/csrc/swz_level.hip
--- a/schwarzwald_amd/csrc/swz_level.hip
+++ b/schwarzwald_amd/csrc/swz_level.hip
@@ -164,14 +164,64 @@
   if (i == m - 1) nstart[id + 1] = m;
 }
 
+__device__ __forceinline__ uint32_t live_before(const uint8_t* __restrict__ gone, const uint32_t* __restrict__ tiles, uint32_t i) {
+  uint32_t off = i & ~(uint32_t)(FS_TILE - 1);
+  uint32_t cnt = tiles[i / (uint32_t)FS_TILE];
+  for (; off + 16u <= i; off += 16u) {
+    const uint4 v = *reinterpret_cast<const uint4*>(gone + off);
+    cnt += fs_zero_bytes(v.x) + fs_zero_bytes(v.y) + fs_zero_bytes(v.z) + fs_zero_bytes(v.w);
+  }
+  for (; off < i; ++off) cnt += gone[off] == 0 ? 1u : 0u;
+  return cnt;
+}
+static int level_live_counts(swz_ctx* c, const uint8_t* gone, uint32_t m, const uint32_t** tiles_out, uint32_t* live) {
+  ProfScope ps(c, "level_live_count", (uint64_t)m, 1);
+  const uint32_t nb = div_up(m, FS_TILE);
+  uint32_t* tiles = nullptr;
+  SWZ_TRY(c->get("lvl_gone_tiles", (size_t)nb + 1, &tiles));
+  hipLaunchKernelGGL(fscan_partial_zero_bytes_kernel, dim3(div_up(nb, (uint32_t)(FS_THREADS / 32))), dim3(FS_THREADS), 0, c->stream, gone,
+                     m, nb, tiles);
+  SWZ_LAUNCH_CHECK(c);
+  SWZ_TRY(scan_exclusive_u32(c, tiles, tiles, nb, tiles + nb, "gone"));
+  SWZ_TRY(read_u32(c, tiles + nb, live));
+  *tiles_out = tiles;
+  return SWZ_OK;
+}
+struct CompactCodedG {
+  const uint64_t* akey;
+  const uint32_t* aidx;
+  const uint8_t* gone;
+  int8_t* level_out;
+  uint64_t* okey;
+  uint32_t* oidx;
+  __device__ void operator()(uint32_t i, uint32_t excl, uint32_t keep) const {
+    const uint32_t p = aidx ? aidx[i] : i;
+    if (keep) {
+      okey[excl] = akey[i];
+      oidx[excl] = p;
+    } else {
+      level_out[p] = (int8_t)((int)gone[i] - 2);
+    }
+  }
+};
+
 __global__ __launch_bounds__(256) void node_mode_kernel(const uint32_t* __restrict__ nstart,
                                                         uint8_t* __restrict__ nmode, uint32_t* __restrict__ counters,
                                                         uint64_t max_points, int force_sample, int terminal,
                                                         int reroot, const uint64_t* __restrict__ akey, uint32_t nsh,
-                                                        const uint64_t* __restrict__ ckey, uint32_t nc) {
+                                                        const uint64_t* __restrict__ ckey, uint32_t nc,
+                                                        const uint8_t* __restrict__ gone, const uint32_t* __restrict__ gone_tiles) {
   const uint32_t nnodes = counters[CTR_NUM_NODES];
   for (uint32_t j = blockIdx.x * 256 + threadIdx.x; j < nnodes; j += gridDim.x * 256u) {
-    const uint32_t cnt = nstart[j + 1] - nstart[j];
+    uint32_t cnt = nstart[j + 1] - nstart[j];
+    if (gone) {
+      cnt = live_before(gone, gone_tiles, nstart[j + 1]) - live_before(gone, gone_tiles, nstart[j]);
+      if (cnt == 0u) {
+        nmode[j] = MODE_TAKE_ALL;
+        continue;
+      }
+      atomicAdd(&counters[CTR_LIVE_NODES], 1u);
+    }
     bool cached = false;
     if (nc) {
       const uint64_t prefix = akey[nstart[j]] >> nsh;
@@ -194,10 +244,10 @@
 
 __global__ __launch_bounds__(256) void take_all_kernel(uint32_t m, const uint32_t* __restrict__ nid,
                                                        const uint8_t* __restrict__ nmode,
-                                                       uint8_t* __restrict__ taken) {
+                                                       uint8_t* __restrict__ taken, uint8_t code, int open_only) {
   const uint32_t i = blockIdx.x * 256 + threadIdx.x;
   if (i >= m) return;
-  if (nmode[nid[i]] == MODE_TAKE_ALL) taken[i] = 1;
+  if (nmode[nid[i]] == MODE_TAKE_ALL && !(open_only && taken[i])) taken[i] = code;
 }
 
 static int candidate_level_host(double root_extent_x, float spacing_at_root, int node_level) {
@@ -300,9 +350,15 @@
 
 int level_step(swz_ctx* c, const LevelPlan& plan, const ActiveSet& as, const SortedPoints& sp,
                       const LevelBuffers& lb, int8_t* level_out, uint64_t* okey, uint32_t* oidx,
-                      LevelResult* res) {
+                      LevelResult* res, const LevelChain* chain) {
   const uint32_t m = as.m;
   const uint32_t nb = div_up(m, 256);
+  const bool shared = as.gone != nullptr;
+  if (shared && !(as.gone == lb.taken && as.gone_tiles && as.parent_prefix && as.parents && m > 0 && plan.node_shift < 63u &&
+                  plan.sampler == SWZ_MIN_DISTANCE && !plan.md_property && !as.ckey && okey && !c->opt("SWZ_LEVEL_NODES_SCAN"))) {
+    res->needs_flush = true;
+    return SWZ_OK;
+  }
   SWZ_HIP(c, hipMemsetAsync(lb.counters, 0, CTR_COUNT * sizeof(uint32_t), c->stream));
   {
     ProfScope ps(c, "level_nodes", (uint64_t)m * 8ull, 3);
@@ -328,7 +384,7 @@
     }
     hipLaunchKernelGGL(node_mode_kernel, dim3(std::min(nb, 2048u)), dim3(256), 0, c->stream, lb.nstart, lb.nmode, lb.counters,
                        plan.max_points, plan.force_sample ? 1 : 0, plan.terminal ? 1 : 0, plan.reroot ? 1 : 0, as.akey,
-                       plan.node_shift, as.ckey, as.nc);
+                       plan.node_shift, as.ckey, as.nc, as.gone, as.gone_tiles);
     SWZ_LAUNCH_CHECK(c);
     if (fill_after_modes) {
       hipLaunchKernelGGL(node_fill_kernel, dim3(div_up(m, NF_TILE)), dim3(256), 0, c->stream, lb.nstart, lb.counters, m, lb.nid,
@@ -344,13 +400,14 @@
   } else if (plan.sampler == SWZ_MIN_DISTANCE_FAST && plan.cand < 0) {
     SWZ_TRY(random_grid_level(c, plan, as, lb));
   } else {
-    SWZ_HIP(c, hipMemsetAsync(lb.taken, 0, m, c->stream));
+    if (!shared) SWZ_HIP(c, hipMemsetAsync(lb.taken, 0, m, c->stream));
     uint32_t h[CTR_COUNT];
     SWZ_HIP(c, hipMemcpyAsync(h, lb.counters, sizeof(h), hipMemcpyDeviceToHost, c->stream));
     SWZ_HIP(c, hipStreamSynchronize(c->stream));
     if (h[CTR_ERROR]) return c->fail((int)h[CTR_ERROR], level_error_message((int)h[CTR_ERROR]));
-    if (h[CTR_SAMPLE_NODES] < h[CTR_NUM_NODES]) {
-      hipLaunchKernelGGL(take_all_kernel, dim3(nb), dim3(256), 0, c->stream, m, lb.nid, lb.nmode, lb.taken);
+    const bool take_all = h[CTR_SAMPLE_NODES] < (shared ? h[CTR_LIVE_NODES] : h[CTR_NUM_NODES]);
+    if (take_all && !shared) {
+      hipLaunchKernelGGL(take_all_kernel, dim3(nb), dim3(256), 0, c->stream, m, lb.nid, lb.nmode, lb.taken, plan.take_code, 0);
       SWZ_LAUNCH_CHECK(c);
     }
     const uint32_t stride = plan.sampler == SWZ_MIN_DISTANCE_FAST ? (uint32_t)swz_min_distance_fast_stride(plan.level) : 1u;
@@ -358,14 +415,31 @@
       SWZ_TRY(min_distance_fast_level(c, plan, as, sp, lb, stride, h[CTR_NUM_NODES], h[CTR_SAMPLE_NODES], &res->md_rounds));
     } else if (h[CTR_SAMPLE_NODES] > 0) {
       SWZ_TRY(min_distance_level(c, plan, as, sp, lb, h[CTR_NUM_NODES], h[CTR_SAMPLE_NODES], h[CTR_SAMPLE_POINTS],
-                                 &res->md_rounds));
-    }
-  }
-
-  if (okey) {
+                                 &res->md_rounds, &res->md_keys_direct, &res->needs_flush));
+      if (res->needs_flush) {
+        c->prof_collect();
+        return SWZ_OK;
+      }
+    }
+    if (take_all && shared) {
+      hipLaunchKernelGGL(take_all_kernel, dim3(nb), dim3(256), 0, c->stream, m, lb.nid, lb.nmode, lb.taken, plan.take_code, 1);
+      SWZ_LAUNCH_CHECK(c);
+    }
+  }
+
+  uint32_t live = 0;
+  if (okey && chain && chain->may_defer && res->md_keys_direct) {
+    SWZ_TRY(level_live_counts(c, lb.taken, m, &res->gone_tiles, &live));
+    res->deferred = live > 0u && (double)(m - live) < chain->max_gone * (double)m;
+  }
+  if (okey && !res->deferred) {
     ProfScope ps(c, "level_compact", (uint64_t)m * 14ull, 2);
-    SWZ_TRY(fused_scan(c, KeepF{lb.taken}, CompactG{as.akey, as.aidx, (int8_t)plan.level, level_out, okey, oidx}, m,
-                       lb.counters + CTR_REMAINING, "lvl"));
+    if (shared)
+      SWZ_TRY(fused_scan(c, KeepF{lb.taken}, CompactCodedG{as.akey, as.aidx, lb.taken, level_out, okey, oidx}, m,
+                         lb.counters + CTR_REMAINING, "lvl"));
+    else
+      SWZ_TRY(fused_scan(c, KeepF{lb.taken}, CompactG{as.akey, as.aidx, (int8_t)plan.level, level_out, okey, oidx}, m,
+                         lb.counters + CTR_REMAINING, "lvl"));
   }
   uint32_t h[CTR_COUNT];
   SWZ_HIP(c, hipMemcpyAsync(h, lb.counters, sizeof(h), hipMemcpyDeviceToHost, c->stream));
@@ -375,18 +449,27 @@
     const int code = (int)h[CTR_ERROR];
     return c->fail(code, level_error_message(code));
   }
-  res->remaining = h[CTR_REMAINING];
-  res->num_nodes = h[CTR_NUM_NODES];
+  res->remaining = res->deferred ? live : h[CTR_REMAINING];
+  res->num_nodes = shared ? h[CTR_LIVE_NODES] : h[CTR_NUM_NODES];
+  res->table_nodes = h[CTR_NUM_NODES];
   res->node_prefix = nullptr;
-  if (okey && res->remaining && res->num_nodes) {
+  if (okey && res->remaining && res->table_nodes) {
     uint64_t* np = nullptr;
-    SWZ_TRY(c->get((plan.level & 1) ? "lvl_node_prefix_1" : "lvl_node_prefix_0", (size_t)res->num_nodes, &np));
-    hipLaunchKernelGGL(node_prefix_kernel, dim3(div_up(res->num_nodes, 256)), dim3(256), 0, c->stream, lb.nstart, as.akey,
-                       plan.node_shift, res->num_nodes, np);
+    SWZ_TRY(c->get((plan.level & 1) ? "lvl_node_prefix_1" : "lvl_node_prefix_0", (size_t)res->table_nodes, &np));
+    hipLaunchKernelGGL(node_prefix_kernel, dim3(div_up(res->table_nodes, 256)), dim3(256), 0, c->stream, lb.nstart, as.akey,
+                       plan.node_shift, res->table_nodes, np);
     SWZ_LAUNCH_CHECK(c);
     res->node_prefix = np;
   }
   return SWZ_OK;
+}
+
+int level_flush_chain(swz_ctx* c, const ActiveSet& as, const LevelBuffers& lb, int8_t* level_out, uint64_t* okey, uint32_t* oidx,
+                      uint32_t* remaining) {
+  ProfScope ps(c, "level_compact", (uint64_t)as.m * 14ull, 2);
+  SWZ_TRY(fused_scan(c, KeepF{as.gone}, CompactCodedG{as.akey, as.aidx, as.gone, level_out, okey, oidx}, as.m, lb.counters + CTR_REMAINING,
+                     "lvl"));
+  return read_u32(c, lb.counters + CTR_REMAINING, remaining);
 }
 
 int alloc_level_buffers(swz_ctx* c, uint32_t m, LevelBuffers* lb) {
diff --git a/schwarzwald_amd/csrc/swz_md.h b/schwarzwald_amd/csrc/swz_md.h
--- a/schwarzwald_amd/csrc/swz_md.h
+++ b/schwarzwald_amd/csrc/swz_md.h
@@ -54,7 +54,7 @@
 int md_active_positions(swz_ctx* c, const MdLevel& L, size_t per_point, const double** X, const double** Y, const double** Z);
 
 int min_distance_keys_level(swz_ctx* c, const MdLevel& L, int cl, uint32_t* rounds_out, bool* used,
-                            const MdShardRoot* shard_root = nullptr);
+                            const MdShardRoot* shard_root = nullptr, bool* direct = nullptr);
 int min_distance_block_level(swz_ctx* c, const MdLevel& L, bool* done);
 int min_distance_sparse_level(swz_ctx* c, const MdLevel& L, int cl, uint32_t* rounds_out, bool* used);
 int min_distance_rounds_level(swz_ctx* c, const MdLevel& L, uint32_t* rounds_out, bool* used);
diff --git a/schwarzwald_amd/csrc/swz_md.hip b/schwarzwald_amd/csrc/swz_md.hip
--- a/schwarzwald_amd/csrc/swz_md.hip
+++ b/schwarzwald_amd/csrc/swz_md.hip
@@ -195,7 +195,13 @@
 }
 
 int min_distance_level(swz_ctx* c, const LevelPlan& plan, const ActiveSet& as, const SortedPoints& sp, const LevelBuffers& lb,
-                       uint32_t num_nodes, uint32_t sample_nodes, uint32_t sample_points, uint32_t* rounds_out) {
+                       uint32_t num_nodes, uint32_t sample_nodes, uint32_t sample_points, uint32_t* rounds_out, bool* keys_direct,
+                       bool* needs_flush) {
+  bool direct = false;
+  if (keys_direct) *keys_direct = false;
+  if (needs_flush) *needs_flush = false;
+  const bool shared = as.gone != nullptr;
+  if (shared && !needs_flush) return c->fail(SWZ_ERR_INTERNAL, "MIN_DISTANCE: a level on shared arrays needs a caller that can compact them");
   c->next_scratch_epoch();
   MdLevel L{plan, as, sp, lb, num_nodes, sample_nodes, sample_points, sample_nodes == num_nodes};
   SWZ_TRY(survey(c, L));
@@ -209,6 +215,10 @@
 
   const int cl_sparse = md_clamp_cell_levels(sample_nodes, plan.cell_levels_geo);
   const bool sparse = (double)sample_points / (double)std::max(1u, L.occupied[cl_sparse]) < c->opt_num("SWZ_MD_SPARSE_LIMIT", 2.0);
+  if (sparse && shared) {
+    *needs_flush = true;
+    return SWZ_OK;
+  }
   if (sparse && !(sp.ghosts && plan.level == -1 && !sp.X)) {
     SWZ_TRY(min_distance_block_level(c, L, &used));
     if (used) {
@@ -232,8 +242,15 @@
   if (!plan.md_property || !sp.X) {
     SWZ_TRY(md_populations(c, L));
     cl = sweep_cell_levels(c, L);
-    SWZ_TRY(min_distance_keys_level(c, L, cl, rounds_out, &used));
-    if (used) return SWZ_OK;
+    SWZ_TRY(min_distance_keys_level(c, L, cl, rounds_out, &used, nullptr, &direct));
+    if (used) {
+      if (keys_direct) *keys_direct = direct;
+      return SWZ_OK;
+    }
+  }
+  if (shared) {
+    *needs_flush = true;
+    return SWZ_OK;
   }
 
   if (!sp.X) return c->fail(SWZ_ERR_INTERNAL, "MIN_DISTANCE: this level needs the positions in Morton order and they were not gathered");
diff --git a/schwarzwald_amd/csrc/swz_mdkeys.hip b/schwarzwald_amd/csrc/swz_mdkeys.hip
--- a/schwarzwald_amd/csrc/swz_mdkeys.hip
+++ b/schwarzwald_amd/csrc/swz_mdkeys.hip
@@ -145,6 +145,8 @@
   const uint32_t* dlist;
   uint32_t* round_word;
   MqPeers peers;
+  const uint8_t* gone;
+  uint32_t keep_qpos;
 };
 
 __device__ __forceinline__ uint32_t uni(uint32_t v) { return (uint32_t)__builtin_amdgcn_readfirstlane((int)v); }
@@ -286,18 +288,29 @@
   }
   key[0] = i0 ? a.akey[i0 - 1u] : 0ull;
   key[5] = i0 + 4u < a.m ? a.akey[i0 + 4u] : 0ull;
-#pragma unroll
-  for (int j = 0; j < 4; ++j) q[j] = mq_pack(key[1 + j]);
+  if (!a.keep_qpos) {
+#pragma unroll
+    for (int j = 0; j < 4; ++j) q[j] = mq_pack(key[1 + j]);
+  }
   if (n == 4u) {
-    ulonglong2 w0, w1;
-    w0.x = q[0], w0.y = q[1], w1.x = q[2], w1.y = q[3];
-    *reinterpret_cast<ulonglong2*>(a.qpos + i0) = w0;
-    *reinterpret_cast<ulonglong2*>(a.qpos + i0 + 2) = w1;
-    *reinterpret_cast<uint32_t*>(a.state + i0) = 0x01010101u * (uint32_t)QS_OPEN;
+    if (!a.keep_qpos) {
+      ulonglong2 w0, w1;
+      w0.x = q[0], w0.y = q[1], w1.x = q[2], w1.y = q[3];
+      *reinterpret_cast<ulonglong2*>(a.qpos + i0) = w0;
+      *reinterpret_cast<ulonglong2*>(a.qpos + i0 + 2) = w1;
+    }
+    uint32_t sw = 0x01010101u * (uint32_t)QS_OPEN;
+    if (a.gone) {
+      const uint32_t g = *reinterpret_cast<const uint32_t*>(a.gone + i0);
+#pragma unroll
+      for (int j = 0; j < 4; ++j)
+        if ((g >> (8 * j)) & 0xFFu) sw = (sw & ~(0xFFu << (8 * j))) | ((uint32_t)QS_DEAD << (8 * j));
+    }
+    *reinterpret_cast<uint32_t*>(a.state + i0) = sw;
   } else {
     for (uint32_t j = 0; j < n; ++j) {
-      a.qpos[i0 + j] = q[j];
-      a.state[i0 + j] = QS_OPEN;
+      if (!a.keep_qpos) a.qpos[i0 + j] = q[j];
+      a.state[i0 + j] = (a.gone && a.gone[i0 + j]) ? (uint8_t)QS_DEAD : (uint8_t)QS_OPEN;
     }
   }
 #pragma unroll
@@ -1152,6 +1165,24 @@
   __hip_atomic_store(word, value, __ATOMIC_RELAXED, __HIP_MEMORY_SCOPE_SYSTEM);
 }
 
+__global__ __launch_bounds__(256) void mq_commit_kernel(const uint8_t* __restrict__ state, uint32_t m, uint8_t code, uint8_t* __restrict__ taken) {
+  const uint64_t i0 = ((uint64_t)blockIdx.x * 256u + threadIdx.x) * 4u;
+  if (i0 >= m) return;
+  if (m - i0 >= 4u) {
+    const uint32_t sw = *reinterpret_cast<const uint32_t*>(state + i0);
+    uint32_t hit = 0;
+#pragma unroll
+    for (int j = 0; j < 4; ++j)
+      if (((sw >> (8 * j)) & 0xFFu) == (uint32_t)QS_TAKEN) hit |= 0xFFu << (8 * j);
+    if (!hit) return;
+    uint32_t* w = reinterpret_cast<uint32_t*>(taken + i0);
+    *w = (*w & ~hit) | ((0x01010101u * (uint32_t)code) & hit);
+  } else {
+    for (uint32_t j = 0; i0 + j < m; ++j)
+      if (state[i0 + j] == QS_TAKEN) taken[i0 + j] = code;
+  }
+}
+
 __global__ __launch_bounds__(256) void mq_verify_kernel(MqArgs a, uint32_t ncells, uint32_t* __restrict__ open_cells) {
   const uint32_t c = blockIdx.x * 256 + threadIdx.x;
   bool open = false;
@@ -1169,8 +1200,10 @@
   return key_metric(c, plan, sp).ok;
 }
 
-int min_distance_keys_level(swz_ctx* c, const MdLevel& L, int cl, uint32_t* rounds_out, bool* used, const MdShardRoot* shard_root) {
+int min_distance_keys_level(swz_ctx* c, const MdLevel& L, int cl, uint32_t* rounds_out, bool* used, const MdShardRoot* shard_root,
+                            bool* direct_out) {
   *used = false;
+  if (direct_out) *direct_out = false;
   const LevelPlan& plan = L.plan;
   const ActiveSet& as = L.as;
   const SortedPoints& sp = L.sp;
@@ -1236,6 +1269,8 @@
     if (const char* f = c->opt("SWZ_MD_DIRECT")) direct = atoi(f) != 0;
     a.direct = (direct && !sharded && grid_entries <= max_cells) ? 1u : 0u;
   }
+  if (as.gone && !a.direct) return SWZ_OK;
+  if (direct_out) *direct_out = a.direct != 0u;
   *used = true;
   uint32_t ncells = 0;
   uint32_t* d_cell_sums = nullptr;
@@ -1256,6 +1291,13 @@
 
   SWZ_TRY(c->get(("md_qpos" + sfx).c_str(), (size_t)m, &a.qpos));
   SWZ_TRY(c->get(("md_qstate" + sfx).c_str(), (size_t)m, &a.state));
+  const bool coded = as.gone != nullptr || plan.take_code != 1;
+  if (coded) a.taken = a.state;
+  a.gone = as.gone;
+  a.keep_qpos = (as.gone && c->mq_qpos_buf == a.qpos && c->mq_qpos_keys == as.akey && c->mq_qpos_m == m) ? 1u : 0u;
+  c->mq_qpos_buf = sharded ? nullptr : a.qpos;
+  c->mq_qpos_keys = as.akey;
+  c->mq_qpos_m = m;
   SWZ_TRY(c->get(("md_qovf" + sfx).c_str(), (size_t)m, &a.ovf));
   SWZ_TRY(c->get(("md_qcinfo" + sfx).c_str(), (size_t)ncells, &a.cinfo));
   if (!a.direct) {
@@ -1533,6 +1575,10 @@
       return c->fail(SWZ_ERR_INTERNAL, msg);
     }
   }
+  if (coded) {
+    hipLaunchKernelGGL(mq_commit_kernel, dim3(div_up(m, 1024)), dim3(256), 0, c->stream, a.state, m, plan.take_code, lb.taken);
+    SWZ_LAUNCH_CHECK(c);
+  }
   if (rounds_out) *rounds_out += round - MQ_FIRST_ROUND;
   if (dbg) {
     float ms = 0.f;
diff --git a/schwarzwald_amd/csrc/swz_session.h b/schwarzwald_amd/csrc/swz_session.h
--- a/schwarzwald_amd/csrc/swz_session.h
+++ b/schwarzwald_amd/csrc/swz_session.h
@@ -29,7 +29,7 @@
 
 int session_prepare(swz_ctx* c, TileSession& t, double* d_xyz, uint32_t n, const double bmin[3], const double bmax[3],
                     const swz_tile_params& p, const TileDeviceOut& out, uint32_t front = 0);
-int session_run_levels(swz_ctx* c, TileSession& t, int last_level, int first_mode);
+int session_run_levels(swz_ctx* c, TileSession& t, int last_level, int first_mode, bool chains = false);
 void session_stats(const TileSession& t, swz_tile_stats* stats);
 
 __device__ __forceinline__ bool recon_candidate(const int8_t* level, const uint32_t* dup, uint32_t i, int start_node_level,
diff --git a/schwarzwald_amd/csrc/swz_session.hip b/schwarzwald_amd/csrc/swz_session.hip
--- a/schwarzwald_amd/csrc/swz_session.hip
+++ b/schwarzwald_amd/csrc/swz_session.hip
@@ -69,10 +69,15 @@
   return SWZ_OK;
 }
 
-int session_run_levels(swz_ctx* c, TileSession& t, int last_level, int first_mode) {
+int session_run_levels(swz_ctx* c, TileSession& t, int last_level, int first_mode, bool chains) {
   const uint64_t* pprefix = nullptr;
   uint32_t parents = 0;
-  for (int level = t.next_level; t.as.m > 0 && level <= last_level; ++level) {
+  const bool chain_static = chains && first_mode < 0 && t.params.sampler == SWZ_MIN_DISTANCE &&
+                            !(t.params.flags & SWZ_FLAG_MIN_DISTANCE_PROPERTY) && !t.sp.ghosts && !t.front && !c->shard &&
+                            !c->md_shard_root && c->opt_on("SWZ_MD_DEFER", true);
+  LevelChain chain;
+  chain.max_gone = c->opt_num("SWZ_MD_DEFER_MAX_GONE", 0.125);
+  for (int level = t.next_level; (t.as.gone ? t.as.live : t.as.m) > 0 && level <= last_level; ++level) {
     if (level > 20) return c->fail(SWZ_ERR_INTERNAL, "level loop ran past level 20");
     if (!t.key_buf[t.which]) {
       SWZ_TRY(c->get("active_keys_2", (size_t)t.as.m, &t.key_buf[t.which]));
@@ -81,6 +86,13 @@
     LevelPlan plan = make_plan(level, t.params.sampler, t.params.max_points_per_node, t.params.spacing_at_root,
                                t.params.max_depth, t.bmin, t.bmax, false, true);
     plan.md_property = (t.params.flags & SWZ_FLAG_MIN_DISTANCE_PROPERTY) != 0;
+    chain.may_defer = false;
+    if (chain_static && level < 20) {
+      const LevelPlan next = make_plan(level + 1, t.params.sampler, t.params.max_points_per_node, t.params.spacing_at_root,
+                                       t.params.max_depth, t.bmin, t.bmax, false, true);
+      chain.may_defer = !plan.terminal && !plan.reroot && !next.terminal && !next.reroot;
+    }
+    if (chain.may_defer || t.as.gone) plan.take_code = (uint8_t)(level + 2);
     if (first_mode >= 0 && level == t.next_level) plan.md_property = false;
     if (first_mode >= 0 && level == t.next_level && !plan.terminal) {
       if (first_mode == 1) {
@@ -93,16 +105,31 @@
     LevelResult r;
     t.as.parent_prefix = pprefix;
     t.as.parents = pprefix ? parents : 0u;
-    SWZ_TRY(level_step(c, plan, t.as, t.sp, t.lb, t.level, t.key_buf[t.which], t.idx_buf[t.which], &r));
-    t.visited += t.as.m;
+    SWZ_TRY(level_step(c, plan, t.as, t.sp, t.lb, t.level, t.key_buf[t.which], t.idx_buf[t.which], &r, &chain));
+    if (r.needs_flush) {
+      if (!t.as.gone) return c->fail(SWZ_ERR_INTERNAL, "a level outside a chain asked for the chain's compaction");
+      uint32_t remaining = 0;
+      SWZ_TRY(level_flush_chain(c, t.as, t.lb, t.level, t.key_buf[t.which], t.idx_buf[t.which], &remaining));
+      t.as = ActiveSet{t.key_buf[t.which], t.idx_buf[t.which], remaining};
+      t.which ^= 1;
+      --level;
+      continue;
+    }
+    t.visited += t.as.gone ? t.as.live : t.as.m;
     t.nodes += r.num_nodes;
     t.rounds += r.md_rounds;
     t.max_level = level;
     ++t.nlevels;
-    t.as = ActiveSet{t.key_buf[t.which], t.idx_buf[t.which], r.remaining};
+    if (r.deferred) {
+      t.as.gone = t.lb.taken;
+      t.as.gone_tiles = r.gone_tiles;
+      t.as.live = r.remaining;
+    } else {
+      t.as = ActiveSet{t.key_buf[t.which], t.idx_buf[t.which], r.remaining};
+      t.which ^= 1;
+    }
     pprefix = r.node_prefix;
-    parents = r.num_nodes;
-    t.which ^= 1;
+    parents = r.table_nodes;
     t.next_level = level + 1;
   }
   return SWZ_OK;
@@ -270,7 +297,7 @@
   TileSession t;
   SWZ_TRY(session_prepare(c, t, d_xyz, n, bmin, bmax, p, out));
   if (p.strategy == SWZ_ACCURATE) {
-    SWZ_TRY(session_run_levels(c, t, 20, -1));
+    SWZ_TRY(session_run_levels(c, t, 20, -1, true));
     session_stats(t, stats);
     return SWZ_OK;
   }
```

Measured after the change: 2696, median of 6. 1.04x the previous value.
